# SYSTRAN/faster-whisper

Measured on AMD Instinct MI355X. Metric: audio-sec/sec (RTF) large-v3 fp16 beam=5 batch=16, higher is better.
Workload: dtype f16

## Files before the change

### faster_whisper_amd/_lib.py

```python
import ctypes as C
import os

import numpy as np

_HERE = os.path.dirname(os.path.abspath(__file__))
LIB_PATH = os.environ.get("FWAMD_LIB") or os.path.join(_HERE, "libfwamd.so")

FW_OK = 0
FW_EINVAL = -1
FW_ENODEV = -2
FW_ENOMEM = -3
FW_ERUNTIME = -4
FW_ENOSPC = -5

COMPUTE_FLOAT16 = 0
COMPUTE_INT8_FLOAT16 = 1
FW_DT_F32 = 0
FW_DT_F16 = 1
FW_MAX_ALIGN_HEADS = 64
FW_MAX_ALTERNATIVES = 8


class FwConfig(C.Structure):
    _fields_ = [
        ("n_mels", C.c_int32), ("n_audio_ctx", C.c_int32), ("d_model", C.c_int32), ("n_heads", C.c_int32),
        ("n_enc_layers", C.c_int32), ("n_dec_layers", C.c_int32), ("n_vocab", C.c_int32),
        ("n_text_ctx", C.c_int32), ("is_multilingual", C.c_int32),
        ("tok_eot", C.c_int32), ("tok_sot", C.c_int32), ("tok_lang_begin", C.c_int32), ("n_langs", C.c_int32),
        ("tok_translate", C.c_int32), ("tok_transcribe", C.c_int32), ("tok_sot_lm", C.c_int32),
        ("tok_sot_prev", C.c_int32), ("tok_no_speech", C.c_int32), ("tok_no_timestamps", C.c_int32),
        ("tok_timestamp_begin", C.c_int32),
        ("n_suppress_begin", C.c_int32), ("suppress_begin", C.c_int32 * 8),
        ("n_align_heads", C.c_int32), ("align_heads", C.c_int32 * (2 * FW_MAX_ALIGN_HEADS)),
    ]


class FwWeight(C.Structure):
    _fields_ = [("name", C.c_char_p), ("data", C.c_void_p), ("dtype", C.c_int32), ("ndim", C.c_int32),
                ("dims", C.c_int64 * 4)]


class FwGenOpts(C.Structure):
    _fields_ = [
        ("beam_size", C.c_int32), ("patience", C.c_float), ("num_hypotheses", C.c_int32),
        ("length_penalty", C.c_float), ("repetition_penalty", C.c_float), ("no_repeat_ngram_size", C.c_int32),
        ("max_length", C.c_int32), ("return_scores", C.c_int32), ("return_no_speech_prob", C.c_int32),
        ("max_initial_timestamp_index", C.c_int32), ("suppress_blank", C.c_int32),
        ("suppress_tokens", C.POINTER(C.c_int32)), ("n_suppress_tokens", C.c_int32),
        ("sampling_topk", C.c_int32), ("sampling_temperature", C.c_float), ("seed", C.c_uint64),
        ("min_new_tokens", C.c_int32),
    ]


class FwVadWeights(C.Structure):
    _fields_ = [
        ("stft_basis", C.c_void_p), ("conv_w", C.c_void_p * 4), ("conv_b", C.c_void_p * 4),
        ("lstm_w", C.c_void_p), ("lstm_r", C.c_void_p), ("lstm_b", C.c_void_p), ("dec_w", C.c_void_p),
        ("dec_b", C.c_float),
    ]


SYMBOLS = [
    "fw_last_error", "fw_abi_version", "fw_device_count",
    "fw_model_create", "fw_model_free", "fw_model_info", "fw_model_blob", "fw_model_create_from_blob_dev",
    "fw_model_set_decode_batch", "fw_model_decode_batch", "fw_model_join_decoder", "fw_model_decode_stats",
    "fw_model_set_merge_wait", "fw_model_set_decode_lanes", "fw_model_run_capacity", "fw_dec_big_min_rows", "fw_dec_big_min_rows_of", "fw_test_knob",
    "fw_test_idle_lead_chunks", "fw_test_run_capacity", "fw_test_dec_linear_plan", "fw_test_self_attn_form",
    "fw_test_gemm_plan",
    "fw_pack_blob_size", "fw_pack_blob_copy", "fw_pack_blob_free",
    "fw_logmel", "fw_logmel_full",
    "fw_encode", "fw_encode_pcm", "fw_encode_pcm_dev", "fw_tensor_shape", "fw_tensor_to_host",
    "fw_tensor_from_host", "fw_tensor_free",
    "fw_generate", "fw_generate_lp", "fw_generate_alt", "fw_detect_language", "fw_align", "fw_score",
    "fw_prof_enable", "fw_prof_reset", "fw_prof_count", "fw_prof_name", "fw_prof_get", "fw_synchronize",
    "fw_dev_alloc", "fw_dev_free", "fw_dev_upload",
    "fw_test_gemm", "fw_test_layernorm", "fw_test_attention", "fw_test_dec_linear", "fw_test_dec_logits", "fw_test_logits_rules",
    "fw_test_dec_self_attn", "fw_test_dec_cross_attn", "fw_test_dec_cross_probs", "fw_test_dec_softmax_pick", "fw_bench_gemm", "fw_bench_dec_linear", "fw_bench_attention",
    "fw_bench_gemm_epi", "fw_bench_dec_linear_epi",
    "fw_test_gemm_ex", "fw_test_cross_kv_frag_index", "fw_test_quant_rows", "fw_test_layernorm_frag",
    "fw_test_dec_beam_update", "fw_test_dec_embed", "fw_test_align_post",
    "fw_test_logits_rules_lp", "fw_test_dec_beam_update_lp",
    "fw_test_logits_rules_alt", "fw_test_dec_beam_update_alt", "fw_test_alt_gather",
    "fw_test_logits_rules_smp_tab", "fw_test_logits_rules_ex", "fw_test_score_rows", "fw_test_graph_captures", "fw_test_blob_check",
    "fw_vad_create", "fw_vad_forward", "fw_vad_free", "fw_vad_forward_dev", "fw_vad_forward_audio_dev",
    "fw_vad_forward_audio_batch_dev",
    "fw_flac_info", "fw_flac_decode",
    "fw_resample_filter", "fw_resample_dev", "fw_bench_resample",
]

_lib = None


class FwError(RuntimeError):
    pass


def load():
    global _lib
    if _lib is not None:
        return _lib
    if not os.path.exists(LIB_PATH):
        raise FwError(
            f"{LIB_PATH} not found: build it with `python -c 'import __graft_entry__ as g; g.build()'` "
            "(hipcc --offload-arch=gfx950). faster_whisper_amd has no CPU fallback.")
    lib = C.CDLL(LIB_PATH)
    vp, i32, i64, f32p = C.c_void_p, C.c_int32, C.c_int64, C.POINTER(C.c_float)
    i32p, i64p = C.POINTER(C.c_int32), C.POINTER(C.c_int64)
    lib.fw_last_error.restype = C.c_char_p
    lib.fw_abi_version.restype = i32
    lib.fw_device_count.restype = i32
    lib.fw_model_create.argtypes = [C.POINTER(FwConfig), C.POINTER(FwWeight), i32, i32, i32, i32, i32, C.POINTER(vp)]
    lib.fw_model_free.argtypes = [vp]
    lib.fw_model_free.restype = None
    lib.fw_model_info.argtypes = [vp, C.POINTER(FwConfig), i32p, i32p, i32p, i32p]
    lib.fw_model_blob.argtypes = [vp, C.POINTER(vp), i64p]
    lib.fw_model_create_from_blob_dev.argtypes = [C.POINTER(FwConfig), vp, i64, i32, i32, i32, i32, C.POINTER(vp)]
    lib.fw_model_set_decode_batch.argtypes = [vp, i32]
    lib.fw_model_decode_batch.argtypes = [vp]
    lib.fw_model_decode_batch.restype = i32
    lib.fw_model_run_capacity.argtypes = [vp]
    lib.fw_model_run_capacity.restype = i32
    lib.fw_dec_big_min_rows.restype = i32
    if hasattr(lib, "fw_dec_big_min_rows_of"):
        lib.fw_dec_big_min_rows_of.restype = i32
        lib.fw_dec_big_min_rows_of.argtypes = [i32, i32]
    if hasattr(lib, "fw_flac_info"):
        lib.fw_flac_info.argtypes = [vp, i64, i32p, i32p, i32p, i64p]
        lib.fw_flac_decode.argtypes = [vp, i64, vp, i64, i64p, i32p]
    if hasattr(lib, "fw_test_knob"):
        lib.fw_test_knob.argtypes = [i32, i32]
    if hasattr(lib, "fw_test_idle_lead_chunks"):
        lib.fw_test_idle_lead_chunks.argtypes = [i64, i32, i32, i64, i32]
        lib.fw_test_idle_lead_chunks.restype = i64
    if hasattr(lib, "fw_test_run_capacity"):
        lib.fw_test_run_capacity.argtypes = [i32, i32, i32, i64, i32, i32, i32, i32, i32, i64p, i64p, i64p]
        lib.fw_test_run_capacity.restype = i32
    if hasattr(lib, "fw_test_dec_linear_plan"):
        lib.fw_test_dec_linear_plan.argtypes = [i32, i32, i32, i32, i32, i32, i32, i32p]
        lib.fw_test_self_attn_form.argtypes = [i32] * 8
        lib.fw_test_self_attn_form.restype = i32
    if hasattr(lib, "fw_test_gemm_plan"):
        lib.fw_test_gemm_plan.argtypes = [i32, i32, i32, i32, i64, i64, i64, i64, i64, i32, i32, i32, i32, i32, i32p]
    lib.fw_model_join_decoder.argtypes = [vp, vp]
    lib.fw_model_set_merge_wait.argtypes = [vp, i32, i32]
    lib.fw_model_set_decode_lanes.argtypes = [vp, i32]
    lib.fw_model_decode_stats.argtypes = [vp, i64p, i64p, i64p, i32p]
    lib.fw_pack_blob_size.argtypes = [C.POINTER(FwConfig), C.POINTER(FwWeight), i32, i32, i64p, C.POINTER(vp)]
    lib.fw_pack_blob_copy.argtypes = [vp, vp, i64]
    lib.fw_pack_blob_free.argtypes = [vp]
    lib.fw_pack_blob_free.restype = None
    lib.fw_logmel.argtypes = [vp, vp, i64p, i32, vp, i32p]
    lib.fw_logmel_full.argtypes = [vp, vp, i64, vp, i64]
    lib.fw_encode.argtypes = [vp, vp, i32, C.POINTER(vp)]
    lib.fw_encode_pcm.argtypes = [vp, vp, i64p, i32, C.POINTER(vp)]
    lib.fw_encode_pcm_dev.argtypes = [vp, vp, i64p, i32, C.POINTER(vp)]
    lib.fw_tensor_shape.argtypes = [vp, i32p, i32p, i32p]
    lib.fw_tensor_to_host.argtypes = [vp, vp, vp]
    lib.fw_tensor_from_host.argtypes = [vp, vp, i32, C.POINTER(vp)]
    lib.fw_tensor_free.argtypes = [vp]
    lib.fw_tensor_free.restype = None
    lib.fw_generate.argtypes = [vp, vp, i32p, i32p, i32, C.POINTER(FwGenOpts), i32p, i32p, f32p, f32p]
    if hasattr(lib, "fw_generate_lp"):
        lib.fw_generate_lp.argtypes = [vp, vp, i32p, i32p, i32, C.POINTER(FwGenOpts), i32p, i32p, f32p, f32p, f32p, f32p]
    if hasattr(lib, "fw_generate_alt"):
        f32 = C.c_float
        lib.fw_generate_alt.argtypes = [vp, vp, i32p, i32p, i32, C.POINTER(FwGenOpts), i32, i32p, i32p, f32p, f32p, f32p,
                                        f32p, i32p, f32p, i32p, f32p]
        lib.fw_test_logits_rules_alt.argtypes = [vp, vp, i32, vp, i32, vp, C.POINTER(FwGenOpts), i32, vp, vp, vp, vp, vp,
                                                 vp, vp, i32, vp, vp]
        lib.fw_test_dec_beam_update_alt.argtypes = [vp, i32, i32, i32, i32, i32, i32, i32, i32, f32, i32, vp, vp, vp, vp,
                                                    vp, vp, vp, i32, f32, vp, vp, vp, vp, vp, vp, vp, vp, vp, vp, vp, vp,
                                                    vp, vp, vp]
        lib.fw_test_alt_gather.argtypes = [vp, vp, vp, i32, i32, i32, i32, i32, vp, i32, vp, vp, vp, vp, i32, vp, vp]
    lib.fw_detect_language.argtypes = [vp, vp, i32, i32p, f32p]
    lib.fw_align.argtypes = [vp, vp, i32p, i32, i32p, i32p, i32p, i32, i32, i32, i32p, i32p, f32p]
    lib.fw_prof_enable.argtypes = [vp, i32]
    lib.fw_prof_enable.restype = None
    lib.fw_prof_reset.argtypes = [vp]
    lib.fw_prof_reset.restype = None
    lib.fw_prof_count.restype = i32
    lib.fw_prof_name.argtypes = [i32]
    lib.fw_prof_name.restype = C.c_char_p
    lib.fw_prof_get.argtypes = [vp, i32, C.POINTER(C.c_double), i64p, C.POINTER(C.c_double), C.POINTER(C.c_double)]
    lib.fw_synchronize.argtypes = [vp]
    lib.fw_dev_alloc.argtypes = [vp, i64, C.POINTER(vp)]
    lib.fw_dev_free.argtypes = [vp, vp]
    lib.fw_dev_upload.argtypes = [vp, vp, vp, i64]
    lib.fw_test_gemm.argtypes = [vp, vp, vp, vp, vp, i32, i32, i32, i32, i32, vp]
    lib.fw_test_dec_linear.argtypes = [vp, vp, vp, vp, vp, vp, vp, i32, i32, i32, i32, i32, vp, vp]
    lib.fw_test_dec_logits.argtypes = [vp, vp, i32, vp]
    lib.fw_test_logits_rules.argtypes = [vp, vp, i32, vp, i32, vp, C.POINTER(FwGenOpts), i32, vp, vp]
    if hasattr(lib, "fw_test_dec_self_attn"):
        lib.fw_test_dec_self_attn.argtypes = [vp, vp, vp, vp, vp, i32, i32, i32, i32, i32, i32, i32, i32, i32, i32, i32, vp]
        lib.fw_test_dec_cross_attn.argtypes = [vp, vp, vp, vp, i32, i32, i32, i32, i32, i32, vp, vp, i32, C.c_float, vp]
        lib.fw_test_dec_cross_probs.argtypes = [vp, vp, vp, i32, i32, i32, vp, i32, i32, i32, i32, vp]
        lib.fw_test_dec_softmax_pick.argtypes = [vp, vp, i32, i32, i32, vp, i32, vp]
    lib.fw_bench_attention.argtypes = [vp, i32, i32, i32, i32, i32, f32p]
    lib.fw_bench_gemm.argtypes = [vp, i32, i32, i32, i32, i32, i32, i32, i32, f32p]
    lib.fw_bench_dec_linear.argtypes = [vp, i32, i32, i32, i32, i32, i32, f32p]
    if hasattr(lib, "fw_bench_gemm_epi"):
        lib.fw_bench_gemm_epi.argtypes = [vp, i32, i32, i32, i32, i32, i32, i32, i32, i32, i32, i32, f32p]
        lib.fw_bench_dec_linear_epi.argtypes = [vp, i32, i32, i32, i32, i32, i32, i32, i32, i32, f32p]
    lib.fw_test_layernorm.argtypes = [vp, vp, vp, vp, i32, i32, vp]
    lib.fw_test_attention.argtypes = [vp, vp, vp, vp, i32, i32, i32, vp]
    if hasattr(lib, "fw_test_gemm_ex"):
        lib.fw_test_gemm_ex.argtypes = [vp, vp, i64, i64, i64, vp, vp, vp, i64, i64, i64, vp, i64, i64, i64, i64, i64,
                                        i32, i32, i32, i32, i32, i32, i32, i32, i32, vp, vp]
        lib.fw_test_cross_kv_frag_index.argtypes = [i32, i32, i32, vp]
        lib.fw_test_quant_rows.argtypes = [vp, vp, i32, i32, i64, vp, vp, i32, vp, vp]
        lib.fw_test_layernorm_frag.argtypes = [vp, vp, vp, vp, i32, i32, i32, vp]
    if hasattr(lib, "fw_test_dec_beam_update"):
        f32 = C.c_float
        lib.fw_test_dec_beam_update.argtypes = [vp, i32, i32, i32, i32, i32, i32, i32, i32, f32, i32, vp, vp, vp, vp, vp,
                                                i32, f32, vp, vp, vp, vp, vp, vp, vp, vp, vp, vp, vp]
        lib.fw_test_dec_embed.argtypes = [vp, vp, i32, vp, i32, vp, i32, i32, i32, i32, i32, i32, f32, vp, vp]
        lib.fw_test_align_post.argtypes = [vp, vp, i32, i32, i32, i32, vp, vp, i32, vp]
    if hasattr(lib, "fw_test_dec_beam_update_lp"):
        f32 = C.c_float
        lib.fw_test_logits_rules_lp.argtypes = [vp, vp, i32, vp, i32, vp, C.POINTER(FwGenOpts), i32, vp, vp, vp]
        lib.fw_test_dec_beam_update_lp.argtypes = [vp, i32, i32, i32, i32, i32, i32, i32, i32, f32, i32, vp, vp, vp, vp, vp,
                                                   vp, vp, i32, f32, vp, vp, vp, vp, vp, vp, vp, vp, vp, vp, vp, vp, vp]
    if hasattr(lib, "fw_test_graph_captures"):
        lib.fw_test_logits_rules_smp_tab.argtypes = [vp, vp, i32, vp, i32, vp, C.POINTER(FwGenOpts), i32, vp, vp, vp, vp, vp, vp]
        lib.fw_test_graph_captures.argtypes = [vp, i64p]
    if hasattr(lib, "fw_test_logits_rules_ex"):
        lib.fw_test_logits_rules_ex.argtypes = [vp, vp, i32, vp, i32, vp, C.POINTER(FwGenOpts), i32, vp, vp, vp, vp, vp, vp, vp]
    if hasattr(lib, "fw_score"):
        lib.fw_score.argtypes = [vp, vp, i32p, i32p, i32p, i32p, i32, i32, C.POINTER(FwGenOpts), f32p, i32p, f32p]
        lib.fw_test_score_rows.argtypes = [vp, vp, i32, vp, vp, vp, C.POINTER(FwGenOpts), i32, vp, vp, vp]
    if hasattr(lib, "fw_test_blob_check"):
        lib.fw_test_blob_check.argtypes = [vp, i64]
    lib.fw_vad_create.argtypes = [C.POINTER(FwVadWeights), C.POINTER(vp)]
    lib.fw_vad_forward.argtypes = [vp, vp, i64, i32, vp, vp, vp]
    lib.fw_vad_free.argtypes = [vp]
    lib.fw_vad_forward_dev.argtypes = [vp, i32, vp, i64, vp, vp, vp]
    if hasattr(lib, "fw_vad_forward_audio_dev"):
        lib.fw_vad_forward_audio_dev.argtypes = [vp, i32, vp, i64, vp, vp, vp]
    if hasattr(lib, "fw_vad_forward_audio_batch_dev"):
        lib.fw_vad_forward_audio_batch_dev.argtypes = [vp, i32, vp, vp, i32, vp, vp, vp]
    lib.fw_vad_free.restype = None
    if hasattr(lib, "fw_resample_dev"):
        f64 = C.c_double
        lib.fw_resample_filter.argtypes = [i32, i32, i32, f64, vp, i64p, i32p, i32p]
        lib.fw_resample_dev.argtypes = [i32, vp, i64, i32, i32, i32, f64, i32, vp, i64]
        lib.fw_bench_resample.argtypes = [i32, vp, i64, i32, i32, i32, f64, i32, i32, f32p]
    _lib = lib
    return lib


def check(rc: int):
    if rc == FW_OK:
        return
    msg = load().fw_last_error().decode("utf-8", "replace")
    if rc in (FW_EINVAL, FW_ENOSPC):
        raise ValueError(msg)
    raise RuntimeError(f"libfwamd error {rc}: {msg}")


def ptr(a: np.ndarray):
    return a.ctypes.data_as(C.c_void_p)


def as_i32p(a: np.ndarray):
    return a.ctypes.data_as(C.POINTER(C.c_int32))


def as_i64p(a: np.ndarray):
    return a.ctypes.data_as(C.POINTER(C.c_int64))


def as_f32p(a: np.ndarray):
    return a.ctypes.data_as(C.POINTER(C.c_float))
```

### faster_whisper_amd/csrc/decoder.hip

```cpp
#include "engine.h"

#include <math.h>
#include <stdlib.h>
#include <string.h>

#include <algorithm>
#include <atomic>
#include <chrono>
#include <numeric>

#include "dec_kernels.h"
#include "kernels.h"

namespace fw {

using fwd::FIN_CAP;
using fwd::GenDev;

#define DEC_RUN_MAX_ROWS 1600

struct CrossPool {
  DevBufs bufs;
  half_t *ck = nullptr, *cvt = nullptr;
  int n_blocks = 0, EB = 0, kvp = 0;
// ... 40 lines not shown
  GrowBuf<int> alt_out_tok;
  GrowBuf<float> alt_out_lp;
  GrowBuf<fwd::AltHyp> alt_hyps;
  int *done = nullptr, *n_done = nullptr, *n_fin = nullptr, *fin_tok = nullptr, *fin_len = nullptr;
  float *fin_score = nullptr, *fin_cum = nullptr;
  int* d_step = nullptr;
  float* no_speech = nullptr;
  unsigned long long* sup_bits = nullptr;
  int* zero_done = nullptr;
  int *ptab = nullptr, *sot_tab = nullptr;
  half_t *nsp_x = nullptr, *nsp_xf = nullptr;
  fwd::SmpRow* smp_tab = nullptr;
  half_t *x_frag = nullptr, *att_frag = nullptr, *ffn_frag = nullptr;
  half_t* xn_frag = nullptr;
  int8_t* xq = nullptr;
  float* xs = nullptr;
  QuantRows ekq;
  std::vector<GraphSlot> graphs;
  uint64_t graph_clock = 0;
  bool graphs_enabled = true;
  ~GenWorkspace() {
    for (GraphSlot& s : graphs)
      if (s.exec) (void)hipGraphExecDestroy(s.exec);
  }
};

static std::atomic<uint64_t> g_tensor_id{1};
uint64_t next_tensor_id() { return g_tensor_id.fetch_add(1); }

static bool env_knob_on(std::atomic<int>& v, const char* env) {
  int x = v.load(std::memory_order_relaxed);
  if (x < 0) {
    const char* e = getenv(env);
    x = (e && atoi(e) == 0) ? 0 : 1;
    v.store(x);
  }
  return x != 0;
}

static int self_positions(const Model* m, int decode_batch, int nts) {
  const int NT = m->cfg.n_text_ctx;
  const int need = (int)(((int64_t)NT * m->max_batch + decode_batch - 1) / decode_batch);
  return std::min(NT, std::max(std::max(nts, need), 8));
}

int64_t gen_workspace_bytes(const Model* m, int lane_chunks, int nts) {
  const fw_config& c = m->cfg;
  const int64_t B = lane_chunks, R = B * m->max_beam, d = c.d_model, L = c.n_dec_layers, NT = c.n_text_ctx;
  const int64_t NTs = self_positions(m, lane_chunks, nts > 0 ? nts : (int)NT);
  int64_t n = 2 * (L * R * NTs * d) * 2;
  n += R * (int64_t)c.n_vocab * 4 + R * 12 * d * 2 * 2;
  n += R * FIN_CAP * NT * 4 + 3 * R * NT * 4;
  n += R * FIN_CAP * (NT + 1) * 4 + 2 * R * NT * 4 + R * 32 * 4;
  return n + (64 << 20);
}

int64_t cross_pool_bytes(const Model* m, int pool_chunks) {
  const fw_config& c = m->cfg;
  const int64_t kvp = ((c.n_audio_ctx + 31) / 32) * 32;
  return 2 * ((int64_t)c.n_dec_layers * pool_chunks * c.d_model * kvp) * 2;
}

static int pool_block_count(int pool_chunks, int max_batch) {
  return std::max(1, std::max(pool_chunks, max_batch) / max_batch);
}

int cross_pool_ensure(Model* m, int pool_chunks) {
  if (m->xpool) return FW_OK;
  const fw_config& c = m->cfg;
  std::unique_ptr<CrossPool> p(new CrossPool());
  p->EB = m->max_batch;
  p->n_blocks = pool_block_count(pool_chunks, m->max_batch);
  p->kvp = ((c.n_audio_ctx + 31) / 32) * 32;
  p->blocks.assign(p->n_blocks, CrossPool::Block());
  const size_t n = (size_t)c.n_dec_layers * p->n_slots() * c.d_model * p->kvp;
  int rc;
  if ((rc = p->bufs.alloc(&p->ck, n)) || (rc = p->bufs.alloc(&p->cvt, n))) return rc;
  const HipFail fail{FW_ENODEV, "cross-attention pool setup"};
  FW_HIP_AS(fail, hipMemset(p->ck, 0, n * sizeof(half_t)));
  FW_HIP_AS(fail, hipMemset(p->cvt, 0, n * sizeof(half_t)));
  FW_HIP_AS(fail, hipDeviceSynchronize());
  m->xpool = p.release();
  return FW_OK;
}

void cross_pool_free(Model* m) {
  delete m->xpool;
  m->xpool = nullptr;
}

static void pool_acquire(CrossPool* p, const std::vector<uint64_t>& ids, const std::vector<int>& ns, std::vector<int>& blk,
                         std::vector<char>& hit) {
  std::unique_lock<std::mutex> lk(p->mu);
  const int n = (int)ids.size();
  blk.assign(n, -1);
  hit.assign(n, 0);
  for (;;) {
    int n_free = 0;
    for (const CrossPool::Block& b : p->blocks) n_free += b.busy ? 0 : 1;
    if (n_free >= n) break;
    p->cv.wait(lk);
  }
  for (int i = 0; i < n; ++i)
    for (int k = 0; k < p->n_blocks; ++k) {
      CrossPool::Block& b = p->blocks[k];
      if (!b.busy && b.enc_id == ids[i] && b.n == ns[i] && ids[i] != 0) { b.busy = true; blk[i] = k; hit[i] = 1; break; }
    }
  for (int i = 0; i < n; ++i) {
    if (blk[i] >= 0) continue;
    int best = -1;
    for (int k = 0; k < p->n_blocks; ++k)
      if (!p->blocks[k].busy && (best < 0 || p->blocks[k].stamp < p->blocks[best].stamp)) best = k;
    CrossPool::Block& b = p->blocks[best];
    b.busy = true; b.enc_id = 0; b.n = 0;
    blk[i] = best;
  }
  for (int i = 0; i < n; ++i) p->blocks[blk[i]].stamp = ++p->clock;
}

static void pool_release(CrossPool* p, const std::vector<int>& blk) {
  {
    std::lock_guard<std::mutex> lk(p->mu);
    for (int k : blk)
      if (k >= 0) p->blocks[k].busy = false;
  }
  p->cv.notify_all();
}

struct PoolHold {
  CrossPool* p;
  std::vector<int> blk;
  hipStream_t st = nullptr;
  ~PoolHold() {
    if (!p) return;
    if (st && !blk.empty()) (void)hipStreamSynchronize(st);
    pool_release(p, blk);
  }
};

int gen_workspace_build(const Model* m, DecodeLane* lane, int lane_chunks, int self_ctx) {
  const fw_config& c = m->cfg;
  std::unique_ptr<GenWorkspace> ws(new GenWorkspace());
  GenWorkspace* g = ws.get();
  g->B = lane_chunks;
  g->EB = m->max_batch;
  g->K = m->max_beam;
  g->R = g->B * g->K;
  g->NT = c.n_text_ctx;
  g->NTs = self_positions(m, g->B, self_ctx > 0 ? self_ctx : c.n_text_ctx);
  g->self_cap = (int64_t)g->R * g->NTs;
  const size_t R = g->R, d = c.d_model, L = c.n_dec_layers, NT = g->NT;
  FW_CHECK_ARG(R <= 2048, "decode_batch * max_beam must be <= 2048 (got %zu)", R);
  FW_HIP(hipSetDevice(m->device));
  if (!lane->stream) FW_HIP(create_stream(&lane->stream, "DEC"));
  int rc;
#define A(p, n) do { if ((rc = g->bufs.alloc(&(p), (n)))) return rc; } while (0)
#define Z(p, n) do { if ((rc = g->bufs.zalloc(&(p), (n)))) return rc; } while (0)
  Z(g->slot_map, R);
  A(g->sk, L * (size_t)g->self_cap * d);
  A(g->sv, L * (size_t)g->self_cap * d);
  A(g->x, R * d); A(g->qkv, R * 3 * d); A(g->att, R * d); A(g->qc, R * d);
  A(g->ffn, R * 4 * d);
  A(g->logits, R * c.n_vocab);
  A(g->prompt_dev, NT * R); A(g->prompt_blk, NT * R);
  A(g->cur_tok, R);
  A(g->hist2, 2 * R * NT);
  A(g->cum2, 2 * R);
  A(g->kvidx2, 2 * R * NT);
  A(g->cand_val, R * 32);
  A(g->cand_tok, R * 32);
  A(g->cand_lp, R * 32);
  A(g->lphist2, 2 * R * NT);
  A(g->done, R); A(g->n_done, 1); A(g->n_fin, R);
  A(g->fin_tok, R * FIN_CAP * NT); A(g->fin_len, R * FIN_CAP);
  A(g->fin_score, R * FIN_CAP); A(g->fin_cum, R * FIN_CAP);
  A(g->fin_lp, R * FIN_CAP * (NT + 1));
  Z(g->d_step, 1);
  A(g->no_speech, R);
  A(g->sup_bits, (size_t)LP_SUP_WORDS);
  Z(g->zero_done, R);
  const size_t R16 = (R + 15) / 16 * 16;
  Z(g->ptab, R); Z(g->sot_tab, R);
  Z(g->nsp_x, R16 * d); Z(g->nsp_xf, R16 * d);
  Z(g->smp_tab, R);
  if (m->compute_type == FW_COMPUTE_INT8_FLOAT16) {
    Z(g->xq, R16 * 4 * d);
    Z(g->xs, R16);
    g->ekq.cap_rows = (int64_t)g->EB * c.n_audio_ctx;
    g->ekq.cap_elems = g->ekq.cap_rows * d;
    A(g->ekq.q, (size_t)g->ekq.cap_elems);
    A(g->ekq.scale, (size_t)g->ekq.cap_rows);
  } else {
    Z(g->x_frag, R16 * d); Z(g->att_frag, R16 * d); Z(g->ffn_frag, R16 * 4 * d); Z(g->xn_frag, R16 * d);
  }
#undef A
#undef Z
  FW_HIP(hipDeviceSynchronize());
  const char* ng = getenv("FWAMD_NO_GRAPH");
  g->graphs_enabled = !(ng && ng[0] == '1');
  lane->gen = ws.release();
  return FW_OK;
}

int gen_workspace_ensure(Model* m, DecodeLane* lane) {
  if (int rc = cross_pool_ensure(m, m->decode_batch)) return rc;
  if (lane->gen) return FW_OK;
  return gen_workspace_build(m, lane, lane_chunks_of(m), m->decode_self_ctx);
}

void gen_workspace_free(DecodeLane* lane) {
  delete lane->gen;
  lane->gen = nullptr;
}

DecodeLane::~DecodeLane() {
  if (stream) (void)hipStreamSynchronize(stream);
  gen_workspace_free(this);
  if (stream) (void)hipStreamDestroy(stream);
  if (spare) (void)hipStreamDestroy(spare);
}

static std::atomic<int> g_cross_kv_layered{-1};
void set_cross_kv_layered(int on) { g_cross_kv_layered.store(on ? 1 : 0); }
static bool cross_kv_strides(const Model* m, int64_t* ws, int64_t* bs) {
  const int L = m->cfg.n_dec_layers;
  if (L < 2) return false;
  const int64_t w1 = m->dec[1].ck.w - m->dec[0].ck.w, b1 = m->dec[1].ck.b - m->dec[0].ck.b;
  for (int l = 1; l < L; ++l) {
    if (m->dec[l].ck.w - m->dec[0].ck.w != l * w1 || m->dec[l].cv.w - m->dec[0].cv.w != l * w1) return false;
    if (m->dec[l].ck.b - m->dec[0].ck.b != l * b1 || m->dec[l].cv.b - m->dec[0].cv.b != l * b1) return false;
  }
  *ws = w1; *bs = b1;
  return w1 > 0;
}

static int ensure_cross_kv(Model* m, DecodeLane* lane, const Tensor* enc, int blk, bool hit) {
  if (hit) return FW_OK;
  GenWorkspace* g = lane->gen;
  CrossPool* pool = m->xpool;
  const int B = enc->B;
  const int b0 = blk * pool->EB;
  const fw_config& c = m->cfg;
  const int d = c.d_model, T = c.n_audio_ctx;
  const int64_t xs = (int64_t)T * d;
  hipStream_t st = lane->stream;
  int rc;
  ProfScope ps(lane->prof, PF_CROSS_KV_GEMM, 2.0 * c.n_dec_layers * B * (double)T * d * (2.0 * d), 0, st);
  const bool i8 = m->compute_type == FW_COMPUTE_INT8_FLOAT16;
  const int kvp = pool->kvp;
  const int64_t kvs = (int64_t)d * kvp;
  const int64_t cls = (int64_t)pool->n_slots() * kvs;
  LinCall k{.in = {enc->data, d, xs}, .C = pool->ck + (size_t)b0 * kvs, .ldc = d, .c_bs = kvs, .M = T, .batch = B,
            .head_rows = kvp, .st = st};
  LinCall v{.in = k.in, .C = pool->cvt + (size_t)b0 * kvs, .ldc = kvp, .c_bs = kvs, .M = T, .batch = B, .trans = true,
            .head_rows = kvp, .st = st};
  if (i8) {
    if ((rc = quantise_rows(m, enc->data, nullptr, (int64_t)B * T, d, st, g->ekq))) return rc;
    k.in = v.in = {.xq = &g->ekq};
  }
  int64_t ws = 0, bs = 0;
  if (!i8 && env_knob_on(g_cross_kv_layered, "FWAMD_CROSS_KV_LAYERED") && cross_kv_strides(m, &ws, &bs)) {
    k.n_layers = v.n_layers = c.n_dec_layers;
    k.w_ls = v.w_ls = ws; k.b_ls = v.b_ls = bs; k.c_ls = v.c_ls = cls;
    if ((rc = run_linear(m, m->dec[0].ck, k)) || (rc = run_linear(m, m->dec[0].cv, v))) return rc;
  } else for (int l = 0; l < c.n_dec_layers; ++l) {
    if (l) { k.C += cls; v.C += cls; }
    if ((rc = run_linear(m, m->dec[l].ck, k)) || (rc = run_linear(m, m->dec[l].cv, v))) return rc;
  }
  std::lock_guard<std::mutex> lk(pool->mu);
  pool->blocks[blk].enc_id = enc->id;
  pool->blocks[blk].n = B;
  return FW_OK;
}

struct StepCfg {
  int rows, kmul;
  int B;
  int pos_fixed;
  int P;
  const int* ptab = nullptr;
  const int* tok;
  bool need_logits;
  int nospeech_rowmul;
  bool beam_tail;
  const int* done;
  int kv_slot0 = 0;
  int blk_n = 0;
  int nospeech_off = 0;
  const int* sel_heads_dev = nullptr;
  const int* sel_layer_off = nullptr;
  float* probs = nullptr; int n_sel_total = 0, n_tok = 0, tok_idx = 0;
};

#define DG(call)                                                        \
  do {                                                                  \
    if ((call) != 0) {                                                  \
      set_error("decoder gemm: unsupported shape (%s)", #call);        \
      return FW_ERUNTIME;                                               \
    }                                                                   \
  } while (0)

static std::atomic<int> g_pos_blocks{-1};
void set_pos_blocks(int on) { g_pos_blocks.store(on ? 1 : 0); }
static int pos_block_size(const Model* m, const GenWorkspace* g, const GenDev& gp, int chunks) {
  if (!env_knob_on(g_pos_blocks, "FWAMD_POS_BLOCKS") || chunks < 1) return 1;
  if (!fwd::self_attn_block_ok(g->NT, gp.ctx, m->cfg.d_model, gp.R)) return 1;
  return std::max(1, std::min(16, g->R / chunks));
}

static int project_logits(Model* m, DecodeLane* lane, const half_t* x, const half_t* x_frag, int rows) {
  GenWorkspace* g = lane->gen;
  const fw_config& c = m->cfg;
  const int d = c.d_model;
  hipStream_t st = lane->stream;
  ProfScope ps(lane->prof, PF_DEC_LOGITS, 2.0 * rows * (double)c.n_vocab * d, 2.0 * c.n_vocab * d, st);
  if (m->compute_type == FW_COMPUTE_INT8_FLOAT16) {
    fwk::launch_quant_rows(st, x, d, m->dec_ln.g, m->dec_ln.b, g->xq, g->xs, rows, d, 1);
    DG(fwd::launch_dec_logits(st, true, g->xq, g->xs, m->logits.wq, m->logits.wscale, nullptr, nullptr, g->logits,
                              c.n_vocab, rows, c.n_vocab, d));
  } else if (m->ln_unfold >= 1) {
    fwk::launch_layernorm(st, x, m->dec_ln.g, m->dec_ln.b, g->xn_frag, rows, d, 1);
    DG(fwd::launch_dec_logits(st, false, g->xn_frag, nullptr, m->logits_p.w, nullptr, nullptr, nullptr, g->logits,
                              c.n_vocab, rows, c.n_vocab, d));
  } else {
    DG(fwd::launch_dec_logits(st, false, x_frag, nullptr, m->logits.w, nullptr, m->logits.s1, m->logits.cf, g->logits,
                              c.n_vocab, rows, c.n_vocab, d));
  }
  return FW_OK;
}

static int run_step(Model* m, DecodeLane* lane, const GenDev& gp, const StepCfg& s) {
  GenWorkspace* g = lane->gen;
  const fw_config& c = m->cfg;
  const int d = c.d_model, H = c.n_heads, T = c.n_audio_ctx, NT = g->NT;
  CrossPool* pool = m->xpool;
  const int kvp = pool->kvp;
  hipStream_t st = lane->stream;
  const int rows = s.rows;
  const bool i8 = m->compute_type == FW_COMPUTE_INT8_FLOAT16;
  {
    ProfScope ps(lane->prof, PF_DEC_MISC, 0, 0, st);
    fwd::launch_embed(st, s.tok, m->tok_emb, m->dec_pos, g->x, i8 ? nullptr : g->x_frag, rows, d, g->d_step,
                      s.pos_fixed, s.P, s.blk_n, s.ptab, s.kmul, gp.reach);
  }
  auto lin_q = [&](const half_t* xin, const LNW* ln, const LinearW& L, const half_t* res, half_t* outp, int act) -> int {
    fwk::launch_quant_rows(st, xin, L.K, ln ? ln->g : nullptr, ln ? ln->b : nullptr, g->xq, g->xs, rows, L.K, 1);
    return fwd::launch_dec_gemm_frag_i8(st, g->xq, g->xs, L.wq, L.wscale, L.b, res, L.N, outp, L.N, rows, L.N, L.K, act);
  };
  auto lin_f = [&](const half_t* xin_frag, const LinearW& L, const half_t* res, half_t* outp, half_t* outp_frag,
                   int act) -> int {
    return fwd::launch_dec_linear(st, fwd::DecLin{xin_frag, L.w, L.b, L.s1, L.cf, res, L.N, outp, L.N, outp_frag, rows,
                                                  L.N, L.K, act});
  };
  const int frag = i8 ? 0 : 1;
  const bool unf = !i8 && m->ln_unfold >= 2;
  auto lin_u = [&](const LNW& ln, const LinearW& L, half_t* outp, half_t* outp_frag, int act) -> int {
    fwk::launch_layernorm(st, g->x, ln.g, ln.b, g->xn_frag, rows, d, 1);
    return fwd::launch_dec_linear(st, fwd::DecLin{g->xn_frag, L.w, L.b, nullptr, nullptr, nullptr, L.N, outp, L.N,
                                                  outp_frag, rows, L.N, L.K, act});
  };
  for (int l = 0; l < c.n_dec_layers; ++l) {
    const DecLayerW& L = m->dec[l];
    half_t* kc = g->sk + (size_t)l * gp.cache_rows * gp.ctx * d;
    half_t* vc = g->sv + (size_t)l * gp.cache_rows * gp.ctx * d;
    const half_t* ck = pool->ck + (size_t)l * pool->n_slots() * d * kvp;
    const half_t* cvt = pool->cvt + (size_t)l * pool->n_slots() * d * kvp;
    {
      ProfScope ps(lane->prof, PF_DEC_GEMM_QKV, 2.0 * rows * 3.0 * d * d, 2.0 * 3.0 * d * d, st);
      if (i8) DG(lin_q(g->x, &L.ln1, L.qkv, nullptr, g->qkv, 0));
      else if (unf) DG(lin_u(L.ln1, L.qkv_p, g->qkv, nullptr, 0));
      else DG(lin_f(g->x_frag, L.qkv, nullptr, g->qkv, nullptr, 0));
    }
// ... 1217 lines not shown
```

### faster_whisper_amd/csrc/engine.h

```cpp
#pragma once
#include <hip/hip_runtime.h>
#include <math.h>
#include <stdint.h>
#include <string.h>
#include <algorithm>
#include <atomic>
#include <chrono>
#include <condition_variable>
#include <deque>
#include <memory>
#include <mutex>
#include <string>
#include <vector>

#include "../../include/fwamd.h"
#include "common.h"
#include "kernels.h"

namespace fw {

void set_error(const char* fmt, ...);
#define FW_HIP(call)                                                                   \
  do {                                                                                 \
    hipError_t e_ = (call);                                                            \
// ... 23 lines not shown
  half_t h = (half_t)f;
  uint16_t u;
  memcpy(&u, &h, 2);
  return u;
}
inline float f16_bits_to_f32(uint16_t u) {
  half_t h;
  memcpy(&h, &u, 2);
  return (float)h;
}

template <typename At>
inline float quant_row_i8(const float* row, int K, int8_t* q, At&& at) {
  float amax = 0.f;
  for (int k = 0; k < K; ++k) amax = std::max(amax, fabsf(row[k]));
  const float sc = amax > 0.f ? 127.0f / amax : 0.f;
  for (int k = 0; k < K; ++k) q[at(k)] = (int8_t)lrintf(row[k] * sc);
  return amax > 0.f ? amax / 127.0f : 1.0f;
}

inline size_t frag_pos(int64_t row, int64_t k, int64_t K, int KE) {
  const int OCT = KE / 4;
  return (size_t)((((row >> 4) * (K / KE) + k / KE) * 64 + ((k / OCT) & 3) * 16 + (row & 15)) * OCT + (k % OCT));
}

#define FW_BLOB_MAGIC "FWAMDBL1"
constexpr int kBlobGeneration = 6;
struct BlobHeader {
  char magic[8];
  int32_t version;
  int32_t n_tensors;
  int64_t total_bytes;
  int32_t compute_type;
  int32_t reserved;
  fw_config cfg;
};
struct BlobEntry {
  char name[64];
  int32_t dtype;
  int32_t ndim;
  int64_t dims[4];
  int64_t offset;
  int64_t nbytes;
};

struct LinearW {
  const half_t* w = nullptr;
  const half_t* b = nullptr;
  const int8_t* wq = nullptr;
  const float* wscale = nullptr;
  const float* s1 = nullptr;
  const float* cf = nullptr;
  int N = 0, K = 0;
};
struct LNW { const half_t* g = nullptr; const half_t* b = nullptr; };

struct EncLayerW { LNW ln1, ln2; LinearW qk, v, out, ffn1, ffn2; };
struct DecLayerW { LNW ln1, ln2, ln3; LinearW qkv, out, cq, ck, cv, cout, ffn1, ffn2; LinearW qkv_p, cq_p, ffn1_p; };

enum ProfFamily {
  PF_LOGMEL = 0, PF_ENC_GEMM, PF_ENC_ATTN, PF_ENC_LN, PF_CROSS_KV_GEMM,
  PF_DEC_GEMM_QKV, PF_DEC_GEMM_DXD, PF_DEC_GEMM_FFN1, PF_DEC_GEMM_FFN2,
  PF_DEC_SELF_ATTN, PF_DEC_CROSS_ATTN, PF_DEC_LOGITS, PF_DEC_SAMPLE, PF_DEC_MISC, PF_COUNT
};

struct ProfAcc {
  double ms = 0; int64_t launches = 0; double flops = 0; double bytes = 0;
};

struct Prof {
  std::mutex mu;
  bool on = false;
  ProfAcc acc[PF_COUNT];
  struct PendingEv { hipEvent_t a, b; int fam; };
  std::vector<PendingEv> pending;
  std::vector<hipEvent_t> ev_pool;
  ~Prof();
};

int dev_alloc(void** p, size_t bytes);
template <typename T>
inline int dev_alloc_t(T** p, size_t n) { return dev_alloc(reinterpret_cast<void**>(p), n * sizeof(T)); }
struct DevBufs {
  std::vector<void*> ptrs;
  DevBufs() = default;
  DevBufs(const DevBufs&) = delete;
  DevBufs& operator=(const DevBufs&) = delete;
  ~DevBufs() {
    for (void* p : ptrs) (void)hipFree(p);
  }
  template <typename T>
  int alloc(T** p, size_t n) {
    if (int rc = dev_alloc_t(p, n)) return rc;
    ptrs.push_back(*p);
    return FW_OK;
  }
  template <typename T>
  int zalloc(T** p, size_t n) {
    if (int rc = alloc(p, n)) return rc;
    FW_HIP(hipMemset(*p, 0, n * sizeof(T)));
    return FW_OK;
  }
};
template <typename T>
struct GrowBuf {
  T* p = nullptr;
  int64_t cap = 0;
  GrowBuf() = default;
  GrowBuf(const GrowBuf&) = delete;
  GrowBuf& operator=(const GrowBuf&) = delete;
  ~GrowBuf() { if (p) (void)hipFree(p); }
  int ensure(int64_t n) {
    if (n <= cap) return FW_OK;
    if (p) (void)hipFree(p);
    p = nullptr;
    cap = 0;
    if (int rc = dev_alloc_t(&p, (size_t)n)) return rc;
    cap = n;
    return FW_OK;
  }
};

struct QuantRows {
  int8_t* q = nullptr;
  float* scale = nullptr;
  int64_t cap_rows = 0, cap_elems = 0;
  int64_t rows = 0, ld = 0;
  bool fits(int64_t r, int64_t K) const { return r >= 0 && K >= 0 && r <= cap_rows && r * K <= cap_elems; }
};

struct Model;
struct EncPool {
  std::mutex mu;
  std::vector<half_t*> free;
  const size_t elems;
  bool closed = false;
  std::atomic<Model*> model;
  EncPool(Model* m, size_t elems_) : elems(elems_), model(m) {}
  int take(half_t** p);
  void give(half_t* p);
  void close();
};
struct Tensor {
  std::shared_ptr<EncPool> pool;
  half_t* data = nullptr;
  int B = 0, T = 0, D = 0;
  uint64_t id = 0;
};

struct GenWorkspace;
struct GenRequest;
struct CrossPool;

constexpr int kMaxDecodeLanes = 4;
struct DecodeLane {
  GenWorkspace* gen = nullptr;
  hipStream_t stream = nullptr;
  hipStream_t spare = nullptr;
  std::mutex mu;
  Prof prof;
  bool busy = false;
  ~DecodeLane();
};

struct DecodeGroup {
  std::mutex mu;
  std::condition_variable cv;
  std::deque<GenRequest*> queue;
  bool gathering = false;
  bool resizing = false;
  int active_runs = 0;
  std::atomic<int> lanes_enabled{kMaxDecodeLanes};
  std::atomic<int> encoding{0};
  std::chrono::steady_clock::time_point last_arrival{};
  std::mutex enc_mu;
  std::atomic<int> enc_pass_us{0};
  std::atomic<int> merge_wait_ms{-1};
  std::atomic<int> merge_fill_pct{90};
  std::atomic<int64_t> n_runs{0}, n_requests{0}, n_chunks{0};
  std::atomic<int> max_run_chunks{0};
  std::atomic<int64_t> graph_captures{0};
};

struct Weights {
  int c_pad = 0;
  LinearW conv1, conv2;
  const half_t* enc_pos = nullptr;
  std::vector<EncLayerW> enc;
  LNW enc_ln_post;
  const half_t* tok_emb = nullptr;
  const half_t* dec_pos = nullptr;
  std::vector<DecLayerW> dec;
  LinearW logits;
  LinearW logits_p;
  LNW dec_ln;
};
int check_blob_header(const BlobHeader& h, int64_t blob_bytes);
int bind_weights(const BlobHeader& h, const BlobEntry* entries, void* blob, Weights& W, bool* has_plain);

struct Model : Weights {
  fw_config cfg{};
  int compute_type = 0;
  int device = 0;
  int max_batch = 0, max_beam = 0;
  hipStream_t stream = nullptr;
  std::mutex mu;

  void* blob = nullptr;
  bool blob_owned = true;
  int64_t blob_bytes = 0;
  int ln_unfold = 0;
  bool has_plain = false;

  float* lm_consts = nullptr;
  float* lm_filtT = nullptr;
  int lm_mel_pad = 0;

  DevBufs bufs;
  GrowBuf<float> ws_pcm;
  int64_t* ws_offsets = nullptr;
  GrowBuf<float> ws_raw;
  int* ws_chunk_max = nullptr;
  int* ws_nframes = nullptr;
  float* ws_feat32 = nullptr;
  half_t* ws_mel_cl = nullptr;
  half_t* ws_conv1 = nullptr;
  half_t *ws_x = nullptr, *ws_x2 = nullptr, *ws_xn = nullptr;
  half_t* ws_qk = nullptr;
  half_t* ws_vt = nullptr;
  half_t* ws_att = nullptr;
  half_t* ws_ffn = nullptr;
  QuantRows ws_xq;
  int t_pad = 0;

  std::vector<std::unique_ptr<DecodeLane>> lanes;
  Model* decoder = nullptr;
  CrossPool* xpool = nullptr;
  int decode_batch = 0;
  int lane_batch = 0;
  int decode_self_ctx = 0;
  int dependents = 0;
  bool free_deferred = false;
  void* self = nullptr;
  Model* blob_owner = nullptr;
  DecodeGroup grp;

  std::shared_ptr<EncPool> enc_pool;

  Prof prof;
};

struct ProfScope {
  Prof* p; int fam; hipStream_t st; hipEvent_t a = nullptr, b = nullptr;
  ProfScope(Prof& p_, int fam_, double flops, double bytes, hipStream_t st_);
  ProfScope(Model* m, int fam_, double flops, double bytes) : ProfScope(m->prof, fam_, flops, bytes, m->stream) {}
  ~ProfScope();
};
void prof_collect(Prof& p);

hipError_t create_stream(hipStream_t* st, const char* role);
int64_t idle_lead_chunks(int64_t queued, int n_queued, int encoding, int64_t want, int max_batch, int lanes = 2);
struct RunCapacity {
  int64_t rows_per_chunk;
  int64_t rows, row_cap, self_cap;
  int ctx;
  bool rows_fit, cache_fits;
  int64_t want;
  int64_t run_cap;
  RunCapacity(int lane_chunks, int max_batch, int max_beam, int64_t self_cap, int B, bool sampling, int beam_size,
              int num_hypotheses, int ctx);
};

struct LinIn {
  const half_t* A = nullptr; int64_t lda = 0, a_bs = 0;
  const QuantRows* xq = nullptr;
};
struct LinCall {
  LinIn in;
  half_t* C = nullptr; int64_t ldc = 0, c_bs = 0;
  const half_t* res = nullptr; int64_t ldr = 0, r_bs = 0;
  int M = 0, batch = 1;
  int act = 0;
  bool trans = false;
  int head_rows = 0;
  int n_layers = 1; int64_t w_ls = 0, b_ls = 0, c_ls = 0;
  hipStream_t st = nullptr;
};
fwk::GemmParams gemm_params(const LinearW& L, const LinCall& c, int64_t ldw);
int run_linear(Model* m, const LinearW& L, const LinCall& c);
int quantise_rows(Model* m, const half_t* A, const LNW* ln, int64_t rows, int K, hipStream_t st, QuantRows& qr);
void set_cross_kv_layered(int on);
int run_encoder(Model* m, int B, half_t* out);

void set_pos_blocks(int on);
uint64_t next_tensor_id();
int gen_workspace_ensure(Model* dm, DecodeLane* lane);
int cross_pool_ensure(Model* dm, int pool_chunks);
int gen_workspace_build(const Model* dm, DecodeLane* lane, int lane_chunks, int self_ctx);
void gen_workspace_free(DecodeLane* lane);
int64_t gen_workspace_bytes(const Model* m, int lane_chunks, int self_ctx);
int64_t cross_pool_bytes(const Model* m, int pool_chunks);
void cross_pool_free(Model* m);
void launch_align_post(hipStream_t st, const float* probs, float* stats, int n_sel, int n_tok_cap, int T, int B,
                       const int* n_tok, const int* nfr, int width, float* mat);
inline Model* decoder_of(Model* m) { return m->decoder ? m->decoder : m; }
inline const Model* decoder_of(const Model* m) { return m->decoder ? m->decoder : m; }
inline Model* decoder_of(const Tensor& t) {
  Model* m = t.pool ? t.pool->model.load() : nullptr;
  return m ? decoder_of(m) : nullptr;
}
inline int lane_chunks_of(const Model* m) {
  const int b = m->lane_batch > 0 ? m->lane_batch : m->decode_batch;
  return b > m->max_batch ? b : m->max_batch;
}

}

struct fw_model { fw::Model impl; };
struct fw_tensor { fw::Tensor impl; };
```

### faster_whisper_amd/csrc/engine.hip

```cpp
#include "engine.h"

#include <math.h>
#include <stdarg.h>
#include <stdio.h>
#include <stdlib.h>
#include <string.h>

#include <algorithm>
#include <map>
#include <optional>
#include <type_traits>

#include "dec_kernels.h"
#include "kernels.h"

namespace fw {

static thread_local char g_err[1024] = "";
void set_error(const char* fmt, ...) {
  va_list ap;
  va_start(ap, fmt);
  vsnprintf(g_err, sizeof(g_err), fmt, ap);
  va_end(ap);
}
// ... 435 lines not shown
  template <typename T>
  int get(const std::string& name, int dtype, std::initializer_list<int64_t> dims, const T** out) const {
    auto it = by_name.find(name);
    FW_CHECK_ARG(it != by_name.end(), "weight blob lacks tensor '%s'", name.c_str());
    const BlobEntry& e = *it->second;
    const char* nm = name.c_str();
    FW_CHECK_ARG(e.dtype == dtype, "weight blob tensor '%s': dtype %d, expected %d", nm, e.dtype, dtype);
    FW_CHECK_ARG(e.ndim == (int)dims.size(), "weight blob tensor '%s': %d dims, expected %zu", nm, e.ndim, dims.size());
    int64_t bytes = dtype == 1 ? 2 : dtype == 2 ? 1 : 4;
    int i = 0;
    for (int64_t x : dims) {
      FW_CHECK_ARG(e.dims[i] == x, "weight blob tensor '%s': dim %d is %lld, expected %lld", nm, i, (long long)e.dims[i],
                   (long long)x);
      bytes *= x;
      ++i;
    }
    FW_CHECK_ARG(e.nbytes == bytes, "weight blob tensor '%s': %lld bytes, its shape has %lld", nm, (long long)e.nbytes,
                 (long long)bytes);
    FW_CHECK_ARG(e.offset >= 0 && e.offset % 256 == 0 && e.offset <= h.total_bytes - bytes,
                 "weight blob tensor '%s': offset %lld (%lld bytes) misaligned or outside the blob's %lld bytes", nm,
                 (long long)e.offset, (long long)bytes, (long long)h.total_bytes);
    *out = reinterpret_cast<const T*>(blob + e.offset);
    return FW_OK;
  }
  int plain(const std::string& name, std::initializer_list<int64_t> dims, const half_t** dst, WForm form = W_ROWS,
            const char* = nullptr) const {
    if (dims.size() != 2) return get(name, 1, dims, dst);
    return get(name, 1, {stored_rows(dims.begin()[0], form), dims.begin()[1]}, dst);
  }
  int conv(const std::string& base, int cout, int, int cin_pad, LinearW& L) const {
    if (int rc = get(base + ".wg", 1, {cout, 3 * cin_pad}, &L.w)) return rc;
    return get(base + ".b", 1, {cout}, &L.b);
  }
  int folded(const std::string& out, const std::string&, const std::string&, const std::string&, int N, int K,
             WForm form, LinearW& L) const {
    int rc;
    if ((rc = get(out + ".wf", 1, {stored_rows(N, form), K}, &L.w)) || (rc = get(out + ".s1", 0, {N}, &L.s1))) return rc;
    return get(out + ".cf", 0, {N}, &L.cf);
  }
  int quant(const std::string& out, const std::string&, int N, int K, WForm form, LinearW& L) const {
    if (int rc = get(out + ".wq", 2, {stored_rows(N, form), K}, &L.wq)) return rc;
    return get(out + ".ws", 0, {N}, &L.wscale);
  }
};

int bind_weights(const BlobHeader& h, const BlobEntry* entries, void* blob, Weights& W, bool* has_plain) {
  Binder b{h, reinterpret_cast<char*>(blob), {}};
  for (int i = 0; i < h.n_tensors; ++i)
    b.by_name[std::string(entries[i].name, strnlen(entries[i].name, sizeof(entries[i].name)))] = &entries[i];
  const bool i8 = h.compute_type == FW_COMPUTE_INT8_FLOAT16;
  *has_plain = !i8 && b.by_name.count("dec.logits.wp") != 0;
  return walk_weights(h.cfg, i8, *has_plain, W, b);
}

static void compute_mel_filters(int n_mels, std::vector<float>& filt ) {
  const int n_fft = 400, nb = 201;
  const double sr = 16000.0;
  std::vector<double> fftfreqs(nb);
  const double val = 1.0 / (n_fft * (1.0 / sr));
  for (int k = 0; k < nb; ++k) fftfreqs[k] = k * val;
  const double max_mel = 45.245640471924965;
  const int n = n_mels + 2;
  std::vector<double> mels(n), freqs(n);
  const double step = (max_mel - 0.0) / (n - 1);
  for (int i = 0; i < n; ++i) mels[i] = i * step + 0.0;
  mels[n - 1] = max_mel;
  const double f_sp = 200.0 / 3;
  const double min_log_hz = 1000.0, min_log_mel = (min_log_hz - 0.0) / f_sp;
  const double logstep = log(6.4) / 27.0;
  for (int i = 0; i < n; ++i) {
    freqs[i] = 0.0 + f_sp * mels[i];
    if (mels[i] >= min_log_mel) freqs[i] = min_log_hz * exp(logstep * (mels[i] - min_log_mel));
  }
  filt.assign((size_t)n_mels * nb, 0.f);
  for (int i = 0; i < n_mels; ++i) {
    const double fd0 = freqs[i + 1] - freqs[i], fd1 = freqs[i + 2] - freqs[i + 1];
    const double enorm = 2.0 / (freqs[i + 2] - freqs[i]);
    for (int k = 0; k < nb; ++k) {
      const double lower = -(freqs[i] - fftfreqs[k]) / fd0;
      const double upper = (freqs[i + 2] - fftfreqs[k]) / fd1;
      double wv = std::max(0.0, std::min(lower, upper));
      wv *= enorm;
      filt[(size_t)i * nb + k] = (float)wv;
    }
  }
}

static int setup_logmel_consts(Model* m) {
  std::vector<float> consts(800);
  for (int j = 0; j < 400; ++j) consts[j] = (float)cos(2.0 * M_PI * (double)j / 400.0);
  for (int n = 0; n < 400; ++n) consts[400 + n] = (float)(0.5 - 0.5 * cos(2.0 * M_PI * (double)n / 400.0));
  std::vector<float> filt;
  compute_mel_filters(m->cfg.n_mels, filt);
  m->lm_mel_pad = ((m->cfg.n_mels + 31) / 32) * 32;
  std::vector<float> filtT((size_t)224 * m->lm_mel_pad, 0.f);
  for (int i = 0; i < m->cfg.n_mels; ++i)
    for (int k = 0; k < 201; ++k) filtT[(size_t)k * m->lm_mel_pad + i] = filt[(size_t)i * 201 + k];
  int rc;
  if ((rc = m->bufs.alloc(&m->lm_consts, 800)) || (rc = m->bufs.alloc(&m->lm_filtT, filtT.size()))) return rc;
  FW_HIP(hipMemcpy(m->lm_consts, consts.data(), 800 * sizeof(float), hipMemcpyHostToDevice));
  FW_HIP(hipMemcpy(m->lm_filtT, filtT.data(), filtT.size() * sizeof(float), hipMemcpyHostToDevice));
  return FW_OK;
}

static std::mutex g_models_mu;
static std::vector<Model*> g_live_models;

static int alloc_workspaces(Model* m) {
  const fw_config& c = m->cfg;
  const size_t B = m->max_batch, d = c.d_model, T = c.n_audio_ctx;
  m->t_pad = ((c.n_audio_ctx + 63) / 64) * 64;
  DevBufs& db = m->bufs;
  const bool i8 = m->compute_type == FW_COMPUTE_INT8_FLOAT16;
  int rc;
  if ((rc = db.alloc(&m->ws_offsets, B + 1)) || (rc = db.alloc(&m->ws_chunk_max, B)) || (rc = db.alloc(&m->ws_nframes, B)) ||
      (rc = m->ws_raw.ensure((int64_t)B * c.n_mels * 3008)) || (rc = db.alloc(&m->ws_feat32, B * c.n_mels * 3000)) ||
      (rc = db.zalloc(&m->ws_mel_cl, B * 3002 * m->c_pad)) || (rc = db.zalloc(&m->ws_conv1, B * 3002 * d)) ||
      (rc = db.alloc(&m->ws_x, B * T * d)) || (rc = db.alloc(&m->ws_x2, B * T * d)) || (rc = db.alloc(&m->ws_xn, B * T * d)) ||
      (rc = db.alloc(&m->ws_qk, B * T * 2 * d)) || (rc = db.zalloc(&m->ws_vt, B * d * m->t_pad)) ||
      (rc = db.alloc(&m->ws_att, B * T * d)) || (rc = db.alloc(&m->ws_ffn, B * T * 4 * d)) ||
      (i8 && ((rc = db.alloc(&m->ws_xq.q, B * T * 4 * d)) || (rc = db.alloc(&m->ws_xq.scale, B * T)))))
    return rc;
  if (i8) { m->ws_xq.cap_rows = B * T; m->ws_xq.cap_elems = B * T * 4 * d; }
  return FW_OK;
}

static int model_from_blob(const void* blob_dev, int64_t blob_bytes, bool owned, int device, int max_batch,
                           int max_beam, fw_model** out) {
  FW_CHECK_ARG(max_batch >= 1 && max_batch <= 256, "max_batch must be in [1,256], got %d", max_batch);
  FW_CHECK_ARG(max_beam >= 1 && max_beam <= 16, "max_beam must be in [1,16], got %d", max_beam);
  FW_CHECK_ARG(max_batch * max_beam <= 2048, "max_batch * max_beam must be <= 2048 decoder rows, got %d", max_batch * max_beam);
  FW_CHECK_ARG(blob_bytes >= (int64_t)sizeof(BlobHeader), "weight blob too small");
  BlobHeader h;
  FW_HIP(hipMemcpy(&h, blob_dev, sizeof(h), hipMemcpyDeviceToHost));
  int rc = check_blob_header(h, blob_bytes);
  if (rc) return rc;
  std::vector<BlobEntry> entries(h.n_tensors);
  FW_HIP(hipMemcpy(entries.data(), reinterpret_cast<const char*>(blob_dev) + sizeof(h),
                   entries.size() * sizeof(BlobEntry), hipMemcpyDeviceToHost));
  fw_model* fm = new fw_model();
  Model* m = &fm->impl;
  m->lanes.reserve(kMaxDecodeLanes);
  m->lanes.emplace_back(new DecodeLane());
  m->cfg = h.cfg;
  m->compute_type = h.compute_type;
  m->device = device;
  m->max_batch = max_batch;
  m->max_beam = max_beam;
  m->blob = const_cast<void*>(blob_dev);
  m->blob_owned = owned;
  m->blob_bytes = blob_bytes;
  m->enc_pool = std::make_shared<EncPool>(m, (size_t)max_batch * h.cfg.n_audio_ctx * h.cfg.d_model);
  auto fail = [&](int code) { fw_model_free(fm); return code; };
  hipError_t he = create_stream(&m->stream, "ENC");
  if (he != hipSuccess) {
    set_error("hipStreamCreate failed: %s", hipGetErrorString(he));
    return fail(FW_ENODEV);
  }
  if ((rc = bind_weights(h, entries.data(), m->blob, *m, &m->has_plain))) return fail(rc);
  m->ln_unfold = env_ln_unfold();
  if (m->ln_unfold && m->compute_type != FW_COMPUTE_INT8_FLOAT16 && !m->has_plain) {
    set_error("FWAMD_LN_UNFOLD=%d needs a weight blob packed with FWAMD_LN_UNFOLD set (this one carries the folded forms only)",
              m->ln_unfold);
    return fail(FW_EINVAL);
  }
  if ((rc = setup_logmel_consts(m))) return fail(rc);
  if ((rc = alloc_workspaces(m))) return fail(rc);
  m->decode_batch = max_batch;
  he = hipDeviceSynchronize();
  if (he != hipSuccess) {
    set_error("device sync after model setup failed: %s", hipGetErrorString(he));
    return fail(FW_ENODEV);
  }
  {
    std::lock_guard<std::mutex> lk(g_models_mu);
    if (!owned)
      for (Model* o : g_live_models)
        if (o->blob == m->blob && o->blob_owned) { m->blob_owner = o; o->dependents += 1; break; }
    g_live_models.push_back(m);
  }
  m->self = fm;
  *out = fm;
  return FW_OK;
}

static void balanced_cu_mask(int n_cus, bool invert, uint32_t mask[8]) {
  const int k = n_cus / 32;
  for (int w = 0; w < 8; ++w) mask[w] = 0;
  for (int i = 0; i < 256; ++i) {
    const bool in = ((i % 8) + (i / 8)) % 8 < k;
    if (in != invert) mask[i >> 5] |= 1u << (i & 31);
  }
}

hipError_t create_stream(hipStream_t* st, const char* role) {
  char name[64];
  snprintf(name, sizeof(name), "FWAMD_%s_CUS", role);
  if (const char* c = getenv(name)) {
    const int v = atoi(c), n = v < 0 ? -v : v;
    if (n >= 32 && n <= 224 && n % 32 == 0) {
      uint32_t mask[8];
      balanced_cu_mask(n, v < 0, mask);
      return hipExtStreamCreateWithCUMask(st, 8, mask);
    }
  }
  snprintf(name, sizeof(name), "FWAMD_%s_STREAM_PRIO", role);
  const char* e = getenv(name);
  if (e && (!strcmp(e, "high") || !strcmp(e, "low"))) {
    int least = 0, greatest = 0;
    if (hipDeviceGetStreamPriorityRange(&least, &greatest) == hipSuccess && least != greatest)
      return hipStreamCreateWithPriority(st, hipStreamNonBlocking, e[0] == 'h' ? greatest : least);
  }
  return hipStreamCreateWithFlags(st, hipStreamNonBlocking);
}

fwk::GemmParams gemm_params(const LinearW& L, const LinCall& c, int64_t ldw) {
  fwk::GemmParams p{};
  if (const QuantRows* xq = c.in.xq) {
    p.A = reinterpret_cast<const half_t*>(xq->q); p.lda = xq->ld; p.a_bstride = c.M * xq->ld;
    p.W = reinterpret_cast<const half_t*>(L.wq);
    p.a_scale = xq->scale; p.as_bstride = c.M; p.w_scale = L.wscale;
  } else {
    p.A = c.in.A; p.lda = c.in.lda; p.a_bstride = c.in.a_bs;
    p.W = L.w;
  }
  p.ldw = ldw;
  p.bias = L.b;
  p.res = c.res; p.ldr = c.ldr; p.r_bstride = c.r_bs;
  p.C = c.C; p.ldc = c.ldc; p.c_bstride = c.c_bs;
  p.M = c.M; p.N = L.N; p.K = L.K;
  p.act = c.act;
  p.head_rows = c.head_rows;
  p.n_layers = c.n_layers; p.w_lstride = c.w_ls; p.bias_lstride = c.b_ls; p.c_lstride = c.c_ls;
  return p;
}

int run_linear(Model* m, const LinearW& L, const LinCall& c) {
  if (const QuantRows* xq = c.in.xq)
    FW_CHECK_ARG(xq->scale && xq->rows == (int64_t)c.batch * c.M && xq->ld == L.K,
                 "int8 gemm: the quantised input holds %lld rows of %lld, the call reads %lld rows of %d", (long long)xq->rows,
                 (long long)xq->ld, (long long)c.batch * c.M, L.K);
  if (fwk::launch_gemm(c.st ? c.st : m->stream, gemm_params(L, c, L.K), c.batch, c.trans) != 0) {
    set_error("%sgemm: unsupported shape M=%d N=%d K=%d lda=%lld layers=%d", c.in.xq ? "int8 " : "", c.M, L.N, L.K,
              (long long)c.in.lda, c.n_layers);
    return FW_ERUNTIME;
  }
  return FW_OK;
}

int quantise_rows(Model* m, const half_t* A, const LNW* ln, int64_t rows, int K, hipStream_t st, QuantRows& qr) {
  FW_CHECK_ARG(qr.fits(rows, K), "quantise_rows: %lld rows x %d = %lld elements, the buffer holds %lld rows, %lld elements",
               (long long)rows, K, (long long)(rows * K), (long long)qr.cap_rows, (long long)qr.cap_elems);
  fwk::launch_quant_rows(st ? st : m->stream, A, K, ln ? ln->g : nullptr, ln ? ln->b : nullptr, qr.q, qr.scale, (int)rows, K);
  qr.rows = rows; qr.ld = K;
  return FW_OK;
}

int run_encoder(Model* m, int B, half_t* out) {
  const fw_config& c = m->cfg;
  const int d = c.d_model, T = c.n_audio_ctx, H = c.n_heads;
  const int64_t xs = (int64_t)T * d, vts = (int64_t)d * m->t_pad;
  const bool i8 = m->compute_type == FW_COMPUTE_INT8_FLOAT16;
  auto gemm_flops = [&](double rows, double k) { return 2.0 * B * rows * d * k; };
  int rc;
  {
    ProfScope ps(m, PF_ENC_GEMM, gemm_flops(3000.0, 3.0 * c.n_mels), 0);
    if ((rc = run_linear(m, m->conv1, {.in = {m->ws_mel_cl, m->c_pad, (int64_t)3002 * m->c_pad}, .C = m->ws_conv1 + d,
                                       .ldc = d, .c_bs = (int64_t)3002 * d, .M = 3000, .batch = B, .act = 1})))
      return rc;
  }
  {
    ProfScope ps(m, PF_ENC_GEMM, gemm_flops(T, 3.0 * d), 0);
    if ((rc = run_linear(m, m->conv2, {.in = {m->ws_conv1, 2 * d, (int64_t)3002 * d}, .C = m->ws_x, .ldc = d, .c_bs = xs,
                                       .res = m->enc_pos, .ldr = d, .r_bs = 0, .M = T, .batch = B, .act = 1})))
      return rc;
  }
  half_t* x = m->ws_x;
  half_t* x2 = m->ws_x2;
  auto normed = [&](const half_t* a, const LNW& ln) -> const half_t* {
    if (i8) return a;
    ProfScope ps(m, PF_ENC_LN, 0, 4.0 * B * T * d);
    fwk::launch_layernorm(m->stream, a, ln.g, ln.b, m->ws_xn, B * T, d);
    return m->ws_xn;
  };
  auto input = [&](const half_t* a, int K, const LNW* ln, LinIn& in) -> int {
    if (!i8) { in = {a, K, (int64_t)T * K}; return FW_OK; }
    in = {.xq = &m->ws_xq};
    return quantise_rows(m, a, ln, (int64_t)B * T, K, m->stream, m->ws_xq);
  };
  for (int l = 0; l < c.n_enc_layers; ++l) {
    const EncLayerW& L = m->enc[l];
    LinIn in;
    const half_t* h = normed(x, L.ln1);
    {
      ProfScope ps(m, PF_ENC_GEMM, gemm_flops(T, 3.0 * d), 0);
      if ((rc = input(h, d, &L.ln1, in)) ||
          (rc = run_linear(m, L.qk, {.in = in, .C = m->ws_qk, .ldc = 2 * d, .c_bs = 2 * xs, .M = T, .batch = B})) ||
          (rc = run_linear(m, L.v, {.in = in, .C = m->ws_vt, .ldc = m->t_pad, .c_bs = vts, .M = T, .batch = B, .trans = true})))
        return rc;
    }
    {
      ProfScope ps(m, PF_ENC_ATTN, 4.0 * B * (double)T * T * d, 0);
      fwk::launch_attn_enc(m->stream, {.q = m->ws_qk, .k = m->ws_qk + d, .ld = 2 * d, .qk_bstride = 2 * xs, .vt = m->ws_vt,
                                       .ldvt = m->t_pad, .vt_bstride = vts, .out = m->ws_att, .ldo = d, .o_bstride = xs,
                                       .B = B, .H = H, .T = T});
    }
    std::optional<ProfScope> ps;
    ps.emplace(m, PF_ENC_GEMM, gemm_flops(T, i8 ? 9.0 * d : d), 0);
    if ((rc = input(m->ws_att, d, nullptr, in)) ||
        (rc = run_linear(m, L.out, {.in = in, .C = x2, .ldc = d, .c_bs = xs, .res = x, .ldr = d, .r_bs = xs, .M = T, .batch = B})))
      return rc;
    if (!i8) ps.reset();
    h = normed(x2, L.ln2);
    if (!i8) ps.emplace(m, PF_ENC_GEMM, gemm_flops(T, 8.0 * d), 0);
    if ((rc = input(h, d, &L.ln2, in)) ||
        (rc = run_linear(m, L.ffn1, {.in = in, .C = m->ws_ffn, .ldc = 4 * d, .c_bs = 4 * xs, .M = T, .batch = B, .act = 1})) ||
        (rc = input(m->ws_ffn, 4 * d, nullptr, in)) ||
        (rc = run_linear(m, L.ffn2, {.in = in, .C = x, .ldc = d, .c_bs = xs, .res = x2, .ldr = d, .r_bs = xs, .M = T, .batch = B})))
      return rc;
  }
  {
    ProfScope ps(m, PF_ENC_LN, 0, 4.0 * B * T * d);
    fwk::launch_layernorm(m->stream, x, m->enc_ln_post.g, m->enc_ln_post.b, out, B * T, d);
  }
  hipError_t he = hipGetLastError();
  if (he != hipSuccess) {
    set_error("encoder launch failed: %s", hipGetErrorString(he));
    return FW_ERUNTIME;
  }
  return FW_OK;
}

int EncPool::take(half_t** p) {
  {
    std::lock_guard<std::mutex> lk(mu);
    if (!free.empty()) {
      *p = free.back();
      free.pop_back();
      return FW_OK;
    }
  }
  return dev_alloc_t(p, elems);
}
void EncPool::give(half_t* p) {
  std::unique_lock<std::mutex> lk(mu);
  if (!closed) { free.push_back(p); return; }
  lk.unlock();
  (void)hipFree(p);
}
void EncPool::close() {
  std::vector<half_t*> rest;
  {
    std::lock_guard<std::mutex> lk(mu);
    closed = true;
    model.store(nullptr);
    rest.swap(free);
  }
  for (half_t* p : rest) (void)hipFree(p);
}

static int new_tensor(Model* m, int B, fw_tensor** out) {
  fw_tensor* t = new fw_tensor();
  t->impl.pool = m->enc_pool;
  t->impl.B = B;
  t->impl.T = m->cfg.n_audio_ctx;
  t->impl.D = m->cfg.d_model;
// ... 8 lines not shown

static int encode_to_tensor(Model* m, int B, const char* what, fw_tensor** out) {
  fw_tensor* t = nullptr;
  int rc = new_tensor(m, B, &t);
  if (rc) return rc;
  if ((rc = run_encoder(m, B, t->impl.data))) {
    fw_tensor_free(t);
    return rc;
  }
  hipError_t he = hipStreamSynchronize(m->stream);
  if (he != hipSuccess) {
    fw_tensor_free(t);
    set_error("%s failed: %s", what, hipGetErrorString(he));
    return FW_ERUNTIME;
  }
  prof_collect(m->prof);
  *out = t;
  return FW_OK;
}

static int check_offsets(const int64_t* offsets, int B, int64_t* total, int* max_frames) {
  FW_CHECK_ARG(offsets && offsets[0] == 0, "offsets[0] must be 0");
  int mf = 0;
  for (int b = 0; b < B; ++b) {
    const int64_t n = offsets[b + 1] - offsets[b];
    FW_CHECK_ARG(n >= 0 && n < (int64_t)1 << 30, "chunk %d has invalid length %lld", b, (long long)n);
    mf = std::max(mf, (int)((n + 160) / 160));
  }
  *total = offsets[B];
  *max_frames = mf;
  return FW_OK;
}

static int logmel_batch(Model* m, const float* pcm_dev, const int64_t* offsets_host, int B, bool want_f32,
                        bool want_cl) {
  int64_t total;
  int max_frames;
  int rc = check_offsets(offsets_host, B, &total, &max_frames);
  if (rc) return rc;
  const int stride = std::max(3008, (max_frames + 7) / 8 * 8);
  if ((rc = m->ws_raw.ensure((int64_t)B * m->cfg.n_mels * stride))) return rc;
  FW_HIP(hipMemcpyAsync(m->ws_offsets, offsets_host, (B + 1) * sizeof(int64_t), hipMemcpyHostToDevice, m->stream));
  {
    ProfScope ps(m, PF_LOGMEL, 0, (double)total * 4 + (double)B * m->cfg.n_mels * 3000 * (want_f32 ? 4 : 2));
    fwk::launch_logmel(m->stream, pcm_dev, m->ws_offsets, B, max_frames, m->lm_consts, m->lm_filtT, m->lm_mel_pad,
                       m->cfg.n_mels, m->ws_raw.p, (int64_t)m->cfg.n_mels * stride, stride, m->ws_chunk_max, 1, 3000,
                       want_f32 ? m->ws_feat32 : nullptr, want_cl ? m->ws_mel_cl : nullptr, m->c_pad, m->ws_nframes);
  }
  hipError_t he = hipGetLastError();
  if (he != hipSuccess) {
    set_error("logmel launch failed: %s", hipGetErrorString(he));
    return FW_ERUNTIME;
  }
  return FW_OK;
}

}

using namespace fw;

extern "C" {

const char* fw_last_error(void) { return g_err; }
int32_t fw_abi_version(void) { return FW_ABI_VERSION; }

int32_t fw_device_count(void) {
  int n = 0;
  if (hipGetDeviceCount(&n) != hipSuccess) return 0;
  return n;
}

int32_t fw_model_create(const fw_config* cfg, const fw_weight* weights, int32_t n_weights, int32_t compute_type,
                        int32_t device_index, int32_t max_batch, int32_t max_beam, fw_model** out) {
  FW_CHECK_ARG(cfg && weights && out, "null argument");
  FW_CHECK_ARG(compute_type == FW_COMPUTE_FLOAT16 || compute_type == FW_COMPUTE_INT8_FLOAT16,
               "unsupported compute_type %d", compute_type);
  int rc = check_config(cfg);
  if (rc) return rc;
  const int ndev = fw_device_count();
  if (ndev <= 0) {
    set_error("no HIP device visible: libfwamd has no CPU fallback");
    return FW_ENODEV;
  }
  FW_CHECK_ARG(device_index >= 0 && device_index < ndev, "device_index %d out of range (%d devices)", device_index,
               ndev);
  FW_HIP(hipSetDevice(device_index));
  std::vector<uint8_t> blob;
  if ((rc = pack_blob(cfg, weights, n_weights, compute_type, blob))) return rc;
  void* dblob = nullptr;
  if ((rc = dev_alloc(&dblob, blob.size()))) return rc;
  hipError_t he = hipMemcpy(dblob, blob.data(), blob.size(), hipMemcpyHostToDevice);
  if (he != hipSuccess) {
    (void)hipFree(dblob);
    set_error("weight upload failed: %s", hipGetErrorString(he));
    return FW_ENODEV;
  }
  rc = model_from_blob(dblob, (int64_t)blob.size(), true, device_index, max_batch, max_beam, out);
  return rc;
}

int32_t fw_pack_blob_size(const fw_config* cfg, const fw_weight* weights, int32_t n_weights, int32_t compute_type,
                          int64_t* size_out, void** handle_out) {
  FW_CHECK_ARG(cfg && weights && size_out && handle_out, "null argument");
  int rc = check_config(cfg);
  if (rc) return rc;
  auto* blob = new std::vector<uint8_t>();
  if ((rc = pack_blob(cfg, weights, n_weights, compute_type, *blob))) {
    delete blob;
    return rc;
  }
  *size_out = (int64_t)blob->size();
  *handle_out = blob;
  return FW_OK;
}
int32_t fw_pack_blob_copy(void* handle, void* dst, int64_t dst_bytes) {
  auto* blob = reinterpret_cast<std::vector<uint8_t>*>(handle);
  FW_CHECK_ARG(blob && dst && dst_bytes >= (int64_t)blob->size(), "bad blob copy arguments");
  memcpy(dst, blob->data(), blob->size());
  return FW_OK;
}
void fw_pack_blob_free(void* handle) { delete reinterpret_cast<std::vector<uint8_t>*>(handle); }

int32_t fw_model_create_from_blob_dev(const fw_config* cfg, const void* blob_dev, int64_t blob_bytes,
                                      int32_t compute_type, int32_t device_index, int32_t max_batch,
                                      int32_t max_beam, fw_model** out) {
  (void)cfg;
  (void)compute_type;
  FW_CHECK_ARG(blob_dev && out, "null argument");
  const int ndev = fw_device_count();
  if (ndev <= 0) {
    set_error("no HIP device visible: libfwamd has no CPU fallback");
    return FW_ENODEV;
  }
  FW_CHECK_ARG(device_index >= 0 && device_index < ndev, "device_index %d out of range", device_index);
  FW_HIP(hipSetDevice(device_index));
  return model_from_blob(blob_dev, blob_bytes, false, device_index, max_batch, max_beam, out);
}

void fw_model_free(fw_model* fm) {
  if (!fm) return;
  Model* m = &fm->impl;
  Model* release[2] = {nullptr, nullptr};
  {
    std::lock_guard<std::mutex> lk(g_models_mu);
    if (m->dependents > 0) {
      m->free_deferred = true;
      return;
    }
    g_live_models.erase(std::remove(g_live_models.begin(), g_live_models.end(), m), g_live_models.end());
    release[0] = m->blob_owner;
    release[1] = m->decoder;
  }
  (void)hipSetDevice(m->device);
  if (m->stream) (void)hipStreamSynchronize(m->stream);
  m->lanes.clear();
  cross_pool_free(m);
  m->enc_pool->close();
  if (m->blob && m->blob_owned) (void)hipFree(m->blob);
  if (m->stream) (void)hipStreamDestroy(m->stream);
  delete fm;
  for (Model* t : release) {
    if (!t) continue;
    bool free_now = false;
    {
      std::lock_guard<std::mutex> lk(g_models_mu);
      t->dependents -= 1;
      free_now = t->free_deferred && t->dependents == 0;
    }
    if (free_now) fw_model_free(static_cast<fw_model*>(t->self));
  }
}

int32_t fw_model_blob(const fw_model* fm, void** blob_dev, int64_t* blob_bytes) {
  FW_CHECK_ARG(fm && blob_dev && blob_bytes, "null argument");
  *blob_dev = fm->impl.blob;
  *blob_bytes = fm->impl.blob_bytes;
  return FW_OK;
}

int32_t fw_model_info(const fw_model* fm, fw_config* cfg_out, int32_t* compute_type, int32_t* device_index,
                      int32_t* max_batch, int32_t* max_beam) {
  FW_CHECK_ARG(fm, "null model");
  const Model* m = &fm->impl;
  if (cfg_out) *cfg_out = m->cfg;
  if (compute_type) *compute_type = m->compute_type;
  if (device_index) *device_index = m->device;
  if (max_batch) *max_batch = m->max_batch;
  if (max_beam) *max_beam = m->max_beam;
  return FW_OK;
}

#define DEC_GROUP_RUN_ROWS 1600
static int env_decode_lanes() {
  const char* e = getenv("FWAMD_DECODE_LANES");
  return e ? std::min(kMaxDecodeLanes, std::max(1, atoi(e))) : 2;
}

int32_t fw_model_set_decode_batch(fw_model* fm, int32_t decode_batch) {
  FW_CHECK_ARG(fm, "null model");
  Model* m = &fm->impl;
  FW_CHECK_ARG(!m->decoder, "this model has joined another model's decoder");
  FW_CHECK_ARG(decode_batch >= 1, "decode_batch must be positive");
  {
    std::lock_guard<std::mutex> gl(m->grp.mu);
    FW_CHECK_ARG(m->grp.active_runs == 0 && !m->grp.gathering && m->grp.queue.empty() && !m->grp.resizing,
                 "decode runs are queued or in flight: set the decode batch before the first generate call or after the last one returned");
    m->grp.resizing = true;
  }
  struct Done {
    DecodeGroup& g;
    ~Done() {
      { std::lock_guard<std::mutex> gl(g.mu); g.resizing = false; }
      g.cv.notify_all();
    }
  } done{m->grp};
  DecodeLane* lane0 = m->lanes[0].get();
  std::lock_guard<std::mutex> lk(lane0->mu);
  FW_HIP(hipSetDevice(m->device));
  int want = std::max(decode_batch, m->max_batch) / m->max_batch * m->max_batch;
  const int n_lanes = want >= 4 * m->max_batch ? env_decode_lanes() : 1;
  const int max_rows = n_lanes >= 2 ? DEC_GROUP_RUN_ROWS : 2048;
  auto lane_of = [&](int pool_chunks) {
    int lc = pool_chunks;
    while (lc > m->max_batch && (int64_t)lc * m->max_beam > max_rows) lc -= m->max_batch;
    return lc;
  };
  size_t free_b = 0, total_b = 0;
  FW_HIP(hipMemGetInfo(&free_b, &total_b));
  for (const auto& l : m->lanes)
    if (l->gen) free_b += (size_t)gen_workspace_bytes(m, lane_chunks_of(m), m->decode_self_ctx);
  if (m->xpool) free_b += (size_t)cross_pool_bytes(m, std::max(m->decode_batch, m->max_batch));
  const int64_t budget = (int64_t)(0.7 * (double)free_b);
  const int NT = m->cfg.n_text_ctx;
  const int ctx_steps[] = {NT, 320, 224, 160};
  int self_ctx = NT;
  for (;;) {
    bool fits = false;
    for (int cs : ctx_steps) {
      if (cs > NT) continue;
      if (cross_pool_bytes(m, want) + n_lanes * gen_workspace_bytes(m, lane_of(want), cs) <= budget) { self_ctx = cs; fits = true; break; }
    }
    if (fits || want <= m->max_batch) break;
    want -= m->max_batch;
  }
  const int lane_batch = lane_of(want);
  const bool lanes_ok = n_lanes == (int)m->lanes.size();
  if (lane0->gen && m->xpool && lanes_ok && want == m->decode_batch && lane_batch == lane_chunks_of(m) &&
      self_ctx == m->decode_self_ctx)
    return FW_OK;
  if (lane0->stream) FW_HIP(hipStreamSynchronize(lane0->stream));
  auto reset = [&] {
    m->lanes.resize(1);
    gen_workspace_free(lane0);
    cross_pool_free(m);
    m->decode_batch = m->max_batch; m->lane_batch = 0; m->decode_self_ctx = 0;
  };
  reset();
  std::vector<std::unique_ptr<DecodeLane>> further;
  int rc = cross_pool_ensure(m, want);
  if (!rc) rc = gen_workspace_build(m, lane0, lane_batch, self_ctx);
  for (int k = 1; !rc && k < n_lanes; ++k) {
    further.emplace_back(new DecodeLane());
    further.back()->prof.on = m->prof.on;
    const hipError_t he = create_stream(&further.back()->spare, "DEC");
    if (he != hipSuccess) set_error("hipStreamCreate failed: %s", hipGetErrorString(he));
    rc = he != hipSuccess ? FW_ENODEV : gen_workspace_build(m, further.back().get(), lane_batch, self_ctx);
  }
  if (rc) { reset(); return rc; }
  m->decode_batch = want; m->lane_batch = lane_batch; m->decode_self_ctx = self_ctx;
  for (auto& l : further) m->lanes.push_back(std::move(l));
  return FW_OK;
}

int32_t fw_model_set_decode_lanes(fw_model* fm, int32_t lanes) {
  FW_CHECK_ARG(fm, "null model");
  Model* dm = decoder_of(&fm->impl);
  int have;
  {
    std::lock_guard<std::mutex> gl(dm->grp.mu);
    have = std::max({2, env_decode_lanes(), (int)dm->lanes.size()});
  }
  FW_CHECK_ARG(lanes >= 1 && lanes <= have, "decode lanes: 1 .. %d", have);
  dm->grp.lanes_enabled.store(lanes);
  return FW_OK;
}

int32_t fw_model_set_merge_wait(fw_model* fm, int32_t wait_ms, int32_t fill_percent) {
  FW_CHECK_ARG(fm, "null model");
  FW_CHECK_ARG(wait_ms >= -1 && wait_ms <= 10000, "merge wait: -1 (one encoder pass), 0 (never) or milliseconds <= 10000");
  FW_CHECK_ARG(fill_percent >= 1 && fill_percent <= 100, "merge fill: 1 .. 100 percent of a run's chunk capacity");
  DecodeGroup& g = decoder_of(&fm->impl)->grp;
  g.merge_wait_ms.store(wait_ms);
  g.merge_fill_pct.store(fill_percent);
  return FW_OK;
}

int32_t fw_model_decode_batch(const fw_model* fm) {
  if (!fm) return 0;
  const Model* m = decoder_of(&fm->impl);
  return std::max(m->decode_batch, m->max_batch);
}

int32_t fw_model_run_capacity(const fw_model* fm) {
  if (!fm) return 0;
  return lane_chunks_of(decoder_of(&fm->impl));
}

int32_t fw_model_decode_stats(const fw_model* fm, int64_t* runs, int64_t* requests, int64_t* chunks,
                              int32_t* max_run_chunks) {
  FW_CHECK_ARG(fm, "null model");
  const Model* m = decoder_of(&fm->impl);
  if (runs) *runs = m->grp.n_runs.load();
  if (requests) *requests = m->grp.n_requests.load();
  if (chunks) *chunks = m->grp.n_chunks.load();
  if (max_run_chunks) *max_run_chunks = m->grp.max_run_chunks.load();
  return FW_OK;
}

int32_t fw_model_join_decoder(fw_model* fm, fw_model* decoder) {
  FW_CHECK_ARG(fm && decoder && fm != decoder, "need two distinct models");
  Model* m = &fm->impl;
  Model* d = &decoder->impl;
  FW_CHECK_ARG(!d->decoder, "the decoder model has itself joined another decoder");
  FW_CHECK_ARG(m->device == d->device && m->blob == d->blob && m->max_batch == d->max_batch && m->max_beam == d->max_beam,
               "models that share a decoder must share device, weight blob, max_batch and max_beam");
  FW_CHECK_ARG(!m->decoder, "this model has already joined a decoder");
  DecodeLane* lane = m->lanes[0].get();
  std::lock_guard<std::mutex> lk(lane->mu);
  FW_HIP(hipSetDevice(m->device));
  if (lane->stream) FW_HIP(hipStreamSynchronize(lane->stream));
  gen_workspace_free(lane);
  cross_pool_free(m);
  {
    std::lock_guard<std::mutex> lk2(g_models_mu);
    d->dependents += 1;
  }
  m->decoder = d;
  return FW_OK;
}

int32_t fw_logmel(fw_model* fm, const float* pcm, const int64_t* offsets, int32_t B, float* out,
                  int32_t* n_frames_out) {
  FW_CHECK_ARG(fm && offsets && out, "null argument");
  Model* m = &fm->impl;
  FW_CHECK_ARG(B >= 1 && B <= m->max_batch, "batch %d exceeds max_batch %d", B, m->max_batch);
  std::lock_guard<std::mutex> lk(m->mu);
  FW_HIP(hipSetDevice(m->device));
  int64_t total; int mf;
  int rc = check_offsets(offsets, B, &total, &mf);
  if (rc) return rc;
  FW_CHECK_ARG(total == 0 || pcm, "null pcm");
  if ((rc = m->ws_pcm.ensure(std::max<int64_t>(total, 1)))) return rc;
  if (total) FW_HIP(hipMemcpyAsync(m->ws_pcm.p, pcm, total * sizeof(float), hipMemcpyHostToDevice, m->stream));
  if ((rc = logmel_batch(m, m->ws_pcm.p, offsets, B, true, false))) return rc;
  FW_HIP(hipMemcpyAsync(out, m->ws_feat32, (size_t)B * m->cfg.n_mels * 3000 * sizeof(float), hipMemcpyDeviceToHost,
                        m->stream));
  if (n_frames_out)
    FW_HIP(hipMemcpyAsync(n_frames_out, m->ws_nframes, B * sizeof(int32_t), hipMemcpyDeviceToHost, m->stream));
  FW_HIP(hipStreamSynchronize(m->stream));
  return FW_OK;
}

int32_t fw_logmel_full(fw_model* fm, const float* pcm, int64_t n_samples, float* out, int64_t out_frames) {
  FW_CHECK_ARG(fm && out, "null argument");
  Model* m = &fm->impl;
  FW_CHECK_ARG(n_samples >= 0 && n_samples < (int64_t)1 << 30, "invalid n_samples");
  const int64_t nf = (n_samples + 160) / 160;
  FW_CHECK_ARG(out_frames == nf, "out_frames must be n_samples/160 + 1 = %lld, got %lld", (long long)nf,
               (long long)out_frames);
  std::lock_guard<std::mutex> lk(m->mu);
  FW_HIP(hipSetDevice(m->device));
  int rc;
  if ((rc = m->ws_pcm.ensure(std::max<int64_t>(n_samples, 1)))) return rc;
  if (n_samples) FW_HIP(hipMemcpyAsync(m->ws_pcm.p, pcm, n_samples * sizeof(float), hipMemcpyHostToDevice, m->stream));
  const int stride = (int)((nf + 7) / 8 * 8);
  if ((rc = m->ws_raw.ensure((int64_t)m->cfg.n_mels * std::max(stride, 3008)))) return rc;
  const int rstride = std::max(stride, 3008);
  int64_t offs[2] = {0, n_samples};
  FW_HIP(hipMemcpyAsync(m->ws_offsets, offs, 2 * sizeof(int64_t), hipMemcpyHostToDevice, m->stream));
  float* dout = nullptr;
  if ((rc = dev_alloc_t(&dout, (size_t)m->cfg.n_mels * nf))) return rc;
  {
    ProfScope ps(m, PF_LOGMEL, 0, (double)n_samples * 4 + (double)m->cfg.n_mels * nf * 4);
    fwk::launch_logmel(m->stream, m->ws_pcm.p, m->ws_offsets, 1, (int)nf, m->lm_consts, m->lm_filtT, m->lm_mel_pad,
                       m->cfg.n_mels, m->ws_raw.p, (int64_t)m->cfg.n_mels * rstride, rstride, m->ws_chunk_max, 0,
                       (int)nf, dout, nullptr, m->c_pad, nullptr);
  }
  hipError_t he = hipMemcpyAsync(out, dout, (size_t)m->cfg.n_mels * nf * sizeof(float), hipMemcpyDeviceToHost,
                                 m->stream);
  if (he == hipSuccess) he = hipStreamSynchronize(m->stream);
  (void)hipFree(dout);
  if (he != hipSuccess) {
    set_error("logmel_full failed: %s", hipGetErrorString(he));
    return FW_ERUNTIME;
  }
  return FW_OK;
}

namespace {
struct EncodingMark {
  fw::DecodeGroup& g;
  std::chrono::steady_clock::time_point t0;
  explicit EncodingMark(fw::Model* m) : g(fw::decoder_of(m)->grp) {
    g.encoding.fetch_add(1);
    g.enc_mu.lock();
    t0 = std::chrono::steady_clock::now();
  }
  ~EncodingMark() {
    const int us = (int)std::chrono::duration_cast<std::chrono::microseconds>(std::chrono::steady_clock::now() - t0).count();
    const int old = g.enc_pass_us.load();
    g.enc_pass_us.store(old ? (3 * old + us) / 4 : us);
    g.enc_mu.unlock();
    g.encoding.fetch_sub(1);
    g.cv.notify_all();
  }
};
}

int32_t fw_encode(fw_model* fm, const float* features, int32_t B, fw_tensor** out) {
  FW_CHECK_ARG(fm && features && out, "null argument");
  Model* m = &fm->impl;
  FW_CHECK_ARG(B >= 1 && B <= m->max_batch, "batch %d exceeds max_batch %d", B, m->max_batch);
  EncodingMark mark(m);
  std::lock_guard<std::mutex> lk(m->mu);
  FW_HIP(hipSetDevice(m->device));
  FW_HIP(hipMemcpyAsync(m->ws_feat32, features, (size_t)B * m->cfg.n_mels * 3000 * sizeof(float),
                        hipMemcpyHostToDevice, m->stream));
  fwk::launch_features_to_cl(m->stream, m->ws_feat32, B, m->cfg.n_mels, 3000, m->ws_mel_cl, m->c_pad);
  return encode_to_tensor(m, B, "encode", out);
}

static int encode_pcm_common(Model* m, const float* pcm_dev, const int64_t* offsets, int B, fw_tensor** out) {
  if (int rc = logmel_batch(m, pcm_dev, offsets, B, false, true)) return rc;
  return encode_to_tensor(m, B, "encode_pcm", out);
}

int32_t fw_encode_pcm(fw_model* fm, const float* pcm, const int64_t* offsets, int32_t B, fw_tensor** out) {
  FW_CHECK_ARG(fm && offsets && out, "null argument");
  Model* m = &fm->impl;
  FW_CHECK_ARG(B >= 1 && B <= m->max_batch, "batch %d exceeds max_batch %d", B, m->max_batch);
  EncodingMark mark(m);
  std::lock_guard<std::mutex> lk(m->mu);
  FW_HIP(hipSetDevice(m->device));
  int64_t total; int mf;
  int rc = check_offsets(offsets, B, &total, &mf);
  if (rc) return rc;
  FW_CHECK_ARG(total == 0 || pcm, "null pcm");
  if ((rc = m->ws_pcm.ensure(std::max<int64_t>(total, 1)))) return rc;
  if (total) FW_HIP(hipMemcpyAsync(m->ws_pcm.p, pcm, total * sizeof(float), hipMemcpyHostToDevice, m->stream));
  return encode_pcm_common(m, m->ws_pcm.p, offsets, B, out);
}

int32_t fw_encode_pcm_dev(fw_model* fm, const float* pcm_dev, const int64_t* offsets, int32_t B, fw_tensor** out) {
  FW_CHECK_ARG(fm && pcm_dev && offsets && out, "null argument");
  Model* m = &fm->impl;
  FW_CHECK_ARG(B >= 1 && B <= m->max_batch, "batch %d exceeds max_batch %d", B, m->max_batch);
  EncodingMark mark(m);
  std::lock_guard<std::mutex> lk(m->mu);
  FW_HIP(hipSetDevice(m->device));
  return encode_pcm_common(m, pcm_dev, offsets, B, out);
}

int32_t fw_tensor_shape(const fw_tensor* t, int32_t* B, int32_t* T, int32_t* D) {
  FW_CHECK_ARG(t, "null tensor");
  if (B) *B = t->impl.B;
  if (T) *T = t->impl.T;
  if (D) *D = t->impl.D;
  return FW_OK;
}

int32_t fw_tensor_to_host(fw_model* fm, const fw_tensor* t, float* out) {
  FW_CHECK_ARG(fm && t && out, "null argument");
  Model* m = &fm->impl;
  std::lock_guard<std::mutex> lk(m->mu);
  FW_HIP(hipSetDevice(m->device));
  const size_t n = (size_t)t->impl.B * t->impl.T * t->impl.D;
  DevBufs db;
  float* tmp = nullptr;
  if (int rc = db.alloc(&tmp, n)) return rc;
  fwk::launch_f16_to_f32(m->stream, t->impl.data, tmp, (int64_t)n);
  hipError_t he = hipMemcpyAsync(out, tmp, n * sizeof(float), hipMemcpyDeviceToHost, m->stream);
  if (he == hipSuccess) he = hipStreamSynchronize(m->stream);
  if (he != hipSuccess) {
    set_error("tensor_to_host failed: %s", hipGetErrorString(he));
    return FW_ERUNTIME;
  }
  return FW_OK;
}

int32_t fw_tensor_from_host(fw_model* fm, const float* data, int32_t B, fw_tensor** out) {
  FW_CHECK_ARG(fm && data && out, "null argument");
  Model* m = &fm->impl;
  FW_CHECK_ARG(B >= 1 && B <= m->max_batch, "batch %d exceeds max_batch %d", B, m->max_batch);
  std::lock_guard<std::mutex> lk(m->mu);
  FW_HIP(hipSetDevice(m->device));
  fw_tensor* t = nullptr;
  int rc = new_tensor(m, B, &t);
  if (rc) return rc;
  const size_t n = (size_t)B * t->impl.T * t->impl.D;
  DevBufs db;
  float* tmp = nullptr;
  if ((rc = db.alloc(&tmp, n))) { fw_tensor_free(t); return rc; }
  hipError_t he = hipMemcpyAsync(tmp, data, n * sizeof(float), hipMemcpyHostToDevice, m->stream);
  fwk::launch_f32_to_f16(m->stream, tmp, t->impl.data, (int64_t)n);
  if (he == hipSuccess) he = hipStreamSynchronize(m->stream);
  if (he != hipSuccess) {
    fw_tensor_free(t);
    set_error("tensor_from_host failed: %s", hipGetErrorString(he));
    return FW_ERUNTIME;
  }
  *out = t;
  return FW_OK;
}

void fw_tensor_free(fw_tensor* t) {
  if (!t) return;
  if (t->impl.data) t->impl.pool->give(t->impl.data);
  delete t;
}

void fw_prof_enable(fw_model* fm, int32_t on) {
  if (!fm) return;
  for_each_prof(&fm->impl, [&](Prof& p) { p.on = on != 0; });
}
void fw_prof_reset(fw_model* fm) {
  if (!fm) return;
  for_each_prof(&fm->impl, [](Prof& p) {
    prof_collect(p);
    std::lock_guard<std::mutex> lk(p.mu);
    for (auto& a : p.acc) a = ProfAcc();
  });
}
int32_t fw_prof_count(void) { return PF_COUNT; }
const char* fw_prof_name(int32_t i) { return (i >= 0 && i < PF_COUNT) ? kProfNames[i] : ""; }
int32_t fw_prof_get(fw_model* fm, int32_t i, double* ms, int64_t* launches, double* flops, double* bytes) {
  FW_CHECK_ARG(fm && i >= 0 && i < PF_COUNT, "bad profile index");
  ProfAcc p;
  for_each_prof(&fm->impl, [&](Prof& r) {
    prof_collect(r);
    std::lock_guard<std::mutex> lk(r.mu);
    const ProfAcc& a = r.acc[i];
    p.ms += a.ms; p.launches += a.launches; p.flops += a.flops; p.bytes += a.bytes;
  });
  if (ms) *ms = p.ms;
  if (launches) *launches = p.launches;
  if (flops) *flops = p.flops;
  if (bytes) *bytes = p.bytes;
  return FW_OK;
}
int32_t fw_synchronize(fw_model* fm) {
  FW_CHECK_ARG(fm, "null model");
  FW_HIP(hipSetDevice(fm->impl.device));
  FW_HIP(hipStreamSynchronize(fm->impl.stream));
  for (const auto& l : fm->impl.lanes)
    if (l->stream) FW_HIP(hipStreamSynchronize(l->stream));
  return FW_OK;
}
int32_t fw_dev_alloc(fw_model* fm, int64_t bytes, void** out_dev) {
  FW_CHECK_ARG(fm && out_dev && bytes >= 0, "bad argument");
  FW_HIP(hipSetDevice(fm->impl.device));
  return dev_alloc(out_dev, (size_t)bytes);
}
int32_t fw_dev_free(fw_model* fm, void* dev) {
  FW_CHECK_ARG(fm, "null model");
  FW_HIP(hipSetDevice(fm->impl.device));
  if (dev) FW_HIP(hipFree(dev));
  return FW_OK;
}
int32_t fw_dev_upload(fw_model* fm, void* dst_dev, const void* src_host, int64_t bytes) {
  FW_CHECK_ARG(fm && dst_dev && src_host && bytes >= 0, "bad argument");
  FW_HIP(hipSetDevice(fm->impl.device));
  FW_HIP(hipMemcpy(dst_dev, src_host, (size_t)bytes, hipMemcpyHostToDevice));
  return FW_OK;
}

}
```

### faster_whisper_amd/csrc/hooks.hip

```cpp
#include "engine.h"

#include <math.h>
#include <string.h>

#include <algorithm>

#include "dec_kernels.h"
#include "kernels.h"

using namespace fw;
using fwd::FIN_CAP;
using fwd::GenDev;

namespace {

struct HookBufs : DevBufs {
  template <typename T>
  int upload(T** dst, const T* src, size_t n) {
    int rc = alloc(dst, n);
    if (rc) return rc;
    FW_HIP(hipMemcpy(*dst, src, n * sizeof(T), hipMemcpyHostToDevice));
    return FW_OK;
  }
  int upload_f16(half_t** dst, const float* src, size_t n) {
    std::vector<half_t> tmp(n);
    for (size_t i = 0; i < n; ++i) tmp[i] = (half_t)src[i];
    return upload(dst, tmp.data(), n);
  }
  int zero(void* ptr, size_t bytes, hipStream_t st) {
    FW_HIP(hipMemsetAsync(ptr, 0, bytes, st));
    return FW_OK;
  }
};

template <typename T>
int download(T* dst, const T* src, size_t n) {
  FW_HIP(hipMemcpy(dst, src, n * sizeof(T), hipMemcpyDeviceToHost));
  return FW_OK;
}
int download_f16(hipStream_t st, float* dst, const half_t* src, size_t n) {
  std::vector<half_t> tmp(n);
  FW_HIP(hipStreamSynchronize(st));
  FW_HIP(hipMemcpy(tmp.data(), src, n * 2, hipMemcpyDeviceToHost));
  for (size_t i = 0; i < n; ++i) dst[i] = (float)tmp[i];
  return FW_OK;
}

int download_f16_frag(hipStream_t st, float* dst, const half_t* src, int rows, int d) {
  std::vector<float> f((size_t)((rows + 15) / 16 * 16) * d);
  int rc = download_f16(st, f.data(), src, f.size());
  if (rc) return rc;
  for (int r = 0; r < rows; ++r)
    for (int k = 0; k < d; ++k) dst[(size_t)r * d + k] = f[frag_pos(r, k, d, 32)];
  return FW_OK;
}

inline size_t cross_kv_frag_pos(bool vt, int kvp, int mm, int n) {
  const int c = n & 63, r = mm & 31;
  const size_t head = (size_t)(n >> 6) * kvp * 64;
  return vt ? head + ((size_t)((mm >> 5) * 4 + (c >> 4)) * 64 + ((mm >> 3) & 3) * 16 + (c & 15)) * 8 + (mm & 7)
            : head + ((size_t)((mm >> 5) * 4 + 2 * ((r >> 2) & 1) + (c >> 5)) * 64 + ((c >> 3) & 3) * 16 + (((r >> 3) << 2) | (r & 3))) * 8 + (c & 7);
}

template <typename At>
int upload_quant_w(HookBufs& db, const float* W, int N, int K, At&& at, int8_t** d_wq, float** d_ws) {
  std::vector<int8_t> wq((size_t)N * K);
  std::vector<float> ws(N), row(K);
  for (int n = 0; n < N; ++n) {
    for (int k = 0; k < K; ++k) row[k] = f16_bits_to_f32(f32_to_f16_bits(W[(size_t)n * K + k]));
    ws[n] = quant_row_i8(row.data(), K, wq.data(), [&](int k) { return at(n, k); });
  }
  int rc = db.upload(d_wq, wq.data(), wq.size());
  return rc ? rc : db.upload(d_ws, ws.data(), ws.size());
}

int fill_lcg(half_t* dst, size_t n, std::vector<uint16_t>& stage, uint32_t seed, float scale) {
  if (stage.size() < n) stage.resize(n);
  for (size_t i = 0; i < n; ++i) {
    seed = seed * 1664525u + 1013904223u;
    stage[i] = f32_to_f16_bits(((int)(seed >> 16) % 2001 - 1000) * scale);
  }
  FW_HIP(hipMemcpy(dst, stage.data(), n * 2, hipMemcpyHostToDevice));
  return FW_OK;
}

constexpr int LAUNCH_REFUSED = 1;
template <typename F>
int time_launches(hipStream_t st, int warmup, int iters, F&& launch, float* ms_total) {
  struct Events {
    hipEvent_t a = nullptr, b = nullptr;
    ~Events() {
      if (a) (void)hipEventDestroy(a);
      if (b) (void)hipEventDestroy(b);
    }
  } ev;
  FW_HIP(hipEventCreate(&ev.a));
  FW_HIP(hipEventCreate(&ev.b));
  int lr = 0;
  for (int i = 0; i < warmup && lr == 0; ++i) lr = launch(i);
  FW_HIP(hipEventRecord(ev.a, st));
  for (int i = 0; i < iters && lr == 0; ++i) lr = launch(i);
  FW_HIP(hipEventRecord(ev.b, st));
  FW_HIP(hipEventSynchronize(ev.b));
  if (lr != 0) return LAUNCH_REFUSED;
  FW_HIP(hipEventElapsedTime(ms_total, ev.a, ev.b));
  return FW_OK;
}

int test_layernorm_impl(fw_model* fm, const float* x, const float* g, const float* b, int32_t rows, int32_t d, int32_t frag,
                        float* out) {
  FW_CHECK_ARG(fm && x && g && b && out && rows >= 1, "null argument");
  FW_CHECK_ARG(d % 128 == 0 && d >= 128 && d <= 1536, "d must be a multiple of 128 and <= 1536");
  Model* m = &fm->impl;
  std::lock_guard<std::mutex> lk(m->mu);
  FW_HIP(hipSetDevice(m->device));
  HookBufs db;
  half_t *dx, *dg, *dlb, *dy;
  const size_t ny = (size_t)(frag ? (rows + 15) / 16 * 16 : rows) * d;
  int rc;
  if ((rc = db.upload_f16(&dx, x, (size_t)rows * d)) || (rc = db.upload_f16(&dg, g, d)) || (rc = db.upload_f16(&dlb, b, d)) ||
      (rc = db.alloc(&dy, ny)) || (rc = db.zero(dy, ny * sizeof(half_t), m->stream)))
    return rc;
  fwk::launch_layernorm(m->stream, dx, dg, dlb, dy, rows, d, frag ? 1 : 0);
  return frag ? download_f16_frag(m->stream, out, dy, rows, d) : download_f16(m->stream, out, dy, (size_t)rows * d);
}

}

extern "C" {

int32_t fw_test_gemm(fw_model* fm, const float* A, const float* W, const float* bias, const float* residual,
                     int32_t M, int32_t N, int32_t K, int32_t act_gelu, int32_t use_int8, float* out) {
  FW_CHECK_ARG(fm && A && W && out, "null argument");
  Model* m = &fm->impl;
  std::lock_guard<std::mutex> lk(m->mu);
  FW_HIP(hipSetDevice(m->device));
  const bool frag_kv = !use_int8 && (act_gelu == 8 || act_gelu == 9);
  FW_CHECK_ARG(!use_int8 || m->compute_type == FW_COMPUTE_INT8_FLOAT16, "int8 gemm test needs an int8_float16 model");
  if (frag_kv && (N % 64 || residual)) { set_error("fragment-major gemm test: N %% 64 == 0, no residual"); return FW_EINVAL; }
  HookBufs db;
  half_t *dA, *dW, *dB = nullptr, *dR = nullptr, *dC;
  int rc;
  if ((rc = db.upload_f16(&dA, A, (size_t)M * K)) || (rc = db.upload_f16(&dW, W, (size_t)N * K)) ||
      (bias && (rc = db.upload_f16(&dB, bias, N))) || (residual && (rc = db.upload_f16(&dR, residual, (size_t)M * N))) ||
      (rc = db.alloc(&dC, (size_t)M * N)))
    return rc;
  LinearW L{dW, dB, nullptr, nullptr, nullptr, nullptr, N, K};
  LinIn in{dA, K, 0};
  if (use_int8) {
    int8_t* dWq;
    float* dWs;
    if ((rc = upload_quant_w(db, W, N, K, [&](int n, int k) { return (size_t)n * K + k; }, &dWq, &dWs)) ||
        (rc = quantise_rows(m, dA, nullptr, M, K, nullptr, m->ws_xq)))
      return rc;
    L.wq = dWq; L.wscale = dWs;
    in = {.xq = &m->ws_xq};
  }
  if (frag_kv) {
    const bool vt = act_gelu == 9;
    const int kvp = (M + 31) / 32 * 32, H = N / 64;
    std::vector<float> hf((size_t)H * kvp * 64);
    half_t* dF;
    if ((rc = db.alloc(&dF, hf.size())) || (rc = db.zero(dF, hf.size() * sizeof(half_t), m->stream))) return rc;
    if ((rc = run_linear(m, L, {.in = in, .C = dF, .ldc = vt ? kvp : N, .M = M, .trans = vt, .head_rows = kvp})) ||
        (rc = download_f16(m->stream, hf.data(), dF, hf.size())))
      return rc;
    for (int mm = 0; mm < kvp; ++mm)
      for (int n = 0; n < N; ++n) {
        const size_t off = cross_kv_frag_pos(vt, kvp, mm, n);
        if (mm < M) out[(size_t)mm * N + n] = hf[off];
        else if (hf[off] != 0.f) { set_error("fragment-major epilogue wrote the padded key %d", mm); return FW_ERUNTIME; }
      }
    return FW_OK;
  }
  const bool trans = act_gelu >= 2;
  rc = run_linear(m, L, {.in = in, .C = dC, .ldc = trans ? M : N, .res = trans ? nullptr : dR, .ldr = trans ? 0 : N, .M = M,
                         .act = trans ? act_gelu - 2 : act_gelu, .trans = trans});
  return rc ? rc : download_f16(m->stream, out, dC, (size_t)M * N);
}

int32_t fw_test_dec_linear(fw_model* fm, const float* x, const float* W, const float* bias, const float* ln_g,
                           const float* ln_b, const float* res, int32_t R, int32_t N, int32_t K, int32_t act,
                           int32_t form, float* out, float* out_from_frag) {
  FW_CHECK_ARG(fm && x && W && out && out_from_frag, "null argument");
  FW_CHECK_ARG(R >= 1 && N % 32 == 0 && K % 64 == 0, "need R >= 1, N %% 32 == 0, K %% 64 == 0");
  FW_CHECK_ARG((ln_g == nullptr) == (ln_b == nullptr), "ln_g and ln_b go together");
  Model* m = &fm->impl;
  std::lock_guard<std::mutex> lk(m->mu);
  FW_HIP(hipSetDevice(m->device));
  const bool i8 = form == 1;
  if (i8 && (m->compute_type != FW_COMPUTE_INT8_FLOAT16 || ln_g)) {
    set_error("int8 decoder-linear test needs an int8_float16 model and no LayerNorm");
    return FW_EINVAL;
  }
  hipStream_t st = m->stream;
  const int R16 = (R + 15) / 16 * 16;
  auto h = [](float v) { return f16_bits_to_f32(f32_to_f16_bits(v)); };
  HookBufs db;
  half_t *d_res = nullptr, *d_bias = nullptr, *d_out;
  int rc;
  if ((res && (rc = db.upload_f16(&d_res, res, (size_t)R * N))) || (rc = db.alloc(&d_out, (size_t)R * N))) return rc;
  if (i8) {
    int8_t *d_wq, *d_xq;
    float *d_ws, *d_xs;
    half_t* d_x;
    if ((rc = upload_quant_w(db, W, N, K, [&](int n, int k) { return frag_pos(n, k, K, 64); }, &d_wq, &d_ws)) ||
        (rc = db.upload_f16(&d_x, x, (size_t)R * K)) || (bias && (rc = db.upload_f16(&d_bias, bias, N))) ||
        (rc = db.alloc(&d_xq, (size_t)R16 * K)) || (rc = db.alloc(&d_xs, (size_t)R16)) || (rc = db.zero(d_xq, (size_t)R16 * K, st)))
      return rc;
    fwk::launch_quant_rows(st, d_x, K, nullptr, nullptr, d_xq, d_xs, R, K, 1);
    if (fwd::launch_dec_gemm_frag_i8(st, d_xq, d_xs, d_wq, d_ws, d_bias, d_res, N, d_out, N, R, N, K, act) != 0) {
      set_error("int8 decoder linear: unsupported shape R=%d N=%d K=%d", R, N, K);
      return FW_ERUNTIME;
    }
    if ((rc = download_f16(st, out, d_out, (size_t)R * N))) return rc;
    memcpy(out_from_frag, out, (size_t)R * N * sizeof(float));
    return FW_OK;
  }
  std::vector<uint16_t> wf((size_t)N * K), xf((size_t)R16 * K, 0);
  std::vector<float> s1(N, 0.f), cf(N, 0.f);
  for (int n = 0; n < N; ++n) {
    double a1 = 0.0, ac = 0.0;
    for (int k = 0; k < K; ++k) {
      const float wv = h(W[(size_t)n * K + k]);
      const uint16_t wg = ln_g ? f32_to_f16_bits(wv * h(ln_g[k])) : f32_to_f16_bits(wv);
      wf[frag_pos(n, k, K, 32)] = wg;
      a1 += (double)f16_bits_to_f32(wg);
      if (ln_g) ac += (double)wv * (double)h(ln_b[k]);
    }
    if (bias) ac += (double)h(bias[n]);
    s1[n] = (float)a1;
    cf[n] = (float)ac;
  }
  for (int r = 0; r < R; ++r)
    for (int k = 0; k < K; ++k) xf[frag_pos(r, k, K, 32)] = f32_to_f16_bits(x[(size_t)r * K + k]);
  uint16_t *d_wf, *d_xf;
  half_t* d_of;
  float *d_s1 = nullptr, *d_cf = nullptr;
  if ((rc = db.upload(&d_wf, wf.data(), wf.size())) || (rc = db.upload(&d_xf, xf.data(), xf.size())) ||
      (rc = db.alloc(&d_of, (size_t)R16 * N)) || (rc = db.zero(d_of, (size_t)R16 * N * 2, st)))
    return rc;
  if (ln_g) {
    if ((rc = db.upload(&d_s1, s1.data(), (size_t)N)) || (rc = db.upload(&d_cf, cf.data(), (size_t)N))) return rc;
  } else if (bias) {
    if ((rc = db.upload_f16(&d_bias, bias, N))) return rc;
  }
  const fwd::DecLin lin{(const half_t*)d_xf, (const half_t*)d_wf, d_bias, d_s1, d_cf, d_res, N, d_out, N, d_of, R, N, K, act};
  if (fwd::launch_dec_linear(st, lin, form) != 0) {
    set_error("decoder linear: unsupported shape R=%d N=%d K=%d (form %d)", R, N, K, form);
    return FW_ERUNTIME;
  }
  if ((rc = download_f16(st, out, d_out, (size_t)R * N))) return rc;
  return download_f16_frag(st, out_from_frag, d_of, R, N);
}

int32_t fw_dec_big_min_rows(void) { return fwd::dec_big_min_rows(); }
int32_t fw_dec_big_min_rows_of(int32_t role, int32_t compute_type) { return fwd::dec_big_min_rows_of(role, compute_type); }

int32_t fw_test_knob(int32_t id, int32_t value) {
  FW_CHECK_ARG(id == 1 || id == 2 || id == 4 || id == 5 || id == 6 || id == 7, "unknown knob %d", id);
  if (id == 6) { set_cross_kv_layered(value); return FW_OK; }
  if (id == 7) { fwd::set_cross_attn_regs(value); return FW_OK; }
  if (id == 1) fwk::g_gemm_order.store(value);
  else if (id == 5) fwk::g_gemm_vt_stage.store(value);
  else if (id == 2) fwd::set_self_attn_form(value);
  else set_pos_blocks(value);
  return FW_OK;
}

int64_t fw_test_idle_lead_chunks(int64_t queued, int32_t n_queued, int32_t encoding, int64_t want, int32_t max_batch) {
  return idle_lead_chunks(queued, n_queued, encoding, want, max_batch);
}

int32_t fw_test_run_capacity(int32_t lane_chunks, int32_t max_batch, int32_t max_beam, int64_t self_cap, int32_t B,
                             int32_t sampling, int32_t beam_size, int32_t num_hypotheses, int32_t ctx,
                             int64_t* rows_per_chunk, int64_t* want, int64_t* run_cap) {
  const RunCapacity cap(lane_chunks, max_batch, max_beam, self_cap, B, sampling != 0, beam_size, num_hypotheses, ctx);
  *rows_per_chunk = cap.rows_per_chunk;
  *want = cap.want;
  *run_cap = cap.run_cap;
  return cap.rows_fit && cap.cache_fits ? 1 : 0;
}

int32_t fw_test_dec_linear_plan(int32_t R, int32_t N, int32_t K, int32_t ldo, int32_t ldr, int32_t compute_type,
                                int32_t form, int32_t out[6]) {
  const fwd::DecLinPlan p = fwd::dec_linear_plan(R, N, K, ldo, ldr, compute_type, form);
  const int32_t f[6] = {p.family, p.cfg, p.row_tiles, p.col_tiles, p.chunk, p.waves};
  memcpy(out, f, sizeof(f));
  return FW_OK;
}

int32_t fw_test_gemm_plan(int32_t M, int32_t N, int32_t K, int32_t batch, int64_t lda, int64_t ldw, int64_t a_bstride,
                          int64_t ldc, int64_t c_bstride, int32_t trans, int32_t int8, int32_t head_rows, int32_t n_layers,
                          int32_t has_res, int32_t out[9]) {
  static const float some_scale = 1.f;
  static const half_t some_res = 0;
  fwk::GemmParams p{};
  p.lda = lda; p.a_bstride = a_bstride; p.ldw = ldw; p.ldc = ldc; p.c_bstride = c_bstride;
  p.M = M; p.N = N; p.K = K;
  p.head_rows = head_rows; p.n_layers = n_layers;
  p.a_scale = int8 ? &some_scale : nullptr;
  p.w_scale = int8 == 1 ? &some_scale : nullptr;
  p.res = has_res ? &some_res : nullptr;
  const fwk::GemmPlan pl = fwk::gemm_plan(p, batch, trans != 0);
  const int32_t f[9] = {pl.kernel, pl.p.nMt, pl.p.nNt, pl.p.nNt_layer, pl.p.n_mp, pl.p.blk_n, pl.p.blk_m, pl.p.vt_stage, pl.grid};
  memcpy(out, f, sizeof(f));
  return FW_OK;
}

int32_t fw_test_self_attn_form(int32_t n_ctx, int32_t cache_ctx, int32_t d, int32_t R_total, int32_t kmul, int32_t H,
                               int32_t chunks, int32_t knob) {
  return fwd::self_attn_form(n_ctx, cache_ctx, d, R_total, kmul, H, chunks, knob);
}

int32_t fw_test_blob_check(const void* blob_host, int64_t bytes) {
  FW_CHECK_ARG(blob_host && bytes >= (int64_t)sizeof(BlobHeader), "weight blob too small");
  BlobHeader h;
  memcpy(&h, blob_host, sizeof(h));
  if (int rc = check_blob_header(h, bytes)) return rc;
  std::vector<BlobEntry> entries(h.n_tensors);
  memcpy(entries.data(), reinterpret_cast<const char*>(blob_host) + sizeof(h), entries.size() * sizeof(BlobEntry));
  Weights unused;
  bool has_plain;
  return bind_weights(h, entries.data(), const_cast<void*>(blob_host), unused, &has_plain);
}

int32_t fw_test_dec_logits(fw_model* fm, const float* x, int32_t R, float* out) {
  FW_CHECK_ARG(fm && x && out && R >= 1, "bad argument");
  Model* m = &fm->impl;
  std::lock_guard<std::mutex> lk(m->mu);
  FW_HIP(hipSetDevice(m->device));
  hipStream_t st = m->stream;
  const int d = m->cfg.d_model, V = m->cfg.n_vocab, R16 = (R + 15) / 16 * 16;
  const bool i8 = m->compute_type == FW_COMPUTE_INT8_FLOAT16;
  std::vector<half_t> xh((size_t)R16 * d, (half_t)0.f);
  for (int r = 0; r < R; ++r)
    for (int k = 0; k < d; ++k) xh[i8 ? (size_t)r * d + k : frag_pos(r, k, d, 32)] = (half_t)x[(size_t)r * d + k];
  HookBufs db;
  half_t* d_x;
  float* d_out;
  int rc, lr;
  if ((rc = db.upload(&d_x, xh.data(), xh.size())) || (rc = db.alloc(&d_out, (size_t)R * V))) return rc;
  if (i8) {
    int8_t* d_xq;
    float* d_xs;
    if ((rc = db.alloc(&d_xq, (size_t)R16 * d)) || (rc = db.alloc(&d_xs, (size_t)R16)) || (rc = db.zero(d_xq, (size_t)R16 * d, st)))
      return rc;
    fwk::launch_quant_rows(st, d_x, d, m->dec_ln.g, m->dec_ln.b, d_xq, d_xs, R, d, 1);
    lr = fwd::launch_dec_logits(st, true, d_xq, d_xs, m->logits.wq, m->logits.wscale, nullptr, nullptr, d_out, V, R, V, d);
  } else {
    lr = fwd::launch_dec_logits(st, false, d_x, nullptr, m->logits.w, nullptr, m->logits.s1, m->logits.cf, d_out, V, R, V,
                                d);
  }
  FW_HIP(hipStreamSynchronize(st));
  if (lr != 0) {
    set_error("logits projection test failed: unsupported shape");
    return FW_ERUNTIME;
  }
  return download(out, d_out, (size_t)R * V);
}

int32_t fw_bench_dec_linear(fw_model* fm, int32_t R, int32_t N, int32_t K, int32_t lnf, int32_t variant, int32_t iters,
                            float* us_out) {
  FW_CHECK_ARG(fm && us_out && R > 0 && N > 0 && K > 0 && iters > 0, "bad argument");
  Model* m = &fm->impl;
  std::lock_guard<std::mutex> lk(m->mu);
  FW_HIP(hipSetDevice(m->device));
  hipStream_t st = m->stream;
  const size_t wn = (size_t)N * K;
  const int copies = (int)std::max<size_t>(2, ((size_t)640 << 20) / (wn * 2));
  const size_t rp = ((size_t)R + 15) / 16 * 16;
  HookBufs db;
  half_t *dW, *dX, *dO, *dB;
  float *dS, *dC;
  std::vector<uint16_t> stage;
  int rc;
  if ((rc = db.alloc(&dW, wn * copies)) || (rc = db.alloc(&dX, rp * K)) || (rc = db.alloc(&dO, rp * N)) ||
      (rc = db.alloc(&dB, (size_t)N)) || (rc = db.alloc(&dS, (size_t)N)) || (rc = db.alloc(&dC, (size_t)N)) ||
      (rc = fill_lcg(dW, wn, stage, 2463534242u, 1e-3f)) || (rc = fill_lcg(dX, rp * K, stage, 2463534242u, 1e-3f)) ||
      (rc = db.zero(dB, (size_t)N * 2, st)) || (rc = db.zero(dS, (size_t)N * 4, st)) || (rc = db.zero(dC, (size_t)N * 4, st)))
    return rc;
  for (int c = 1; c < copies; ++c) FW_HIP(hipMemcpy(dW + (size_t)c * wn, dW, wn * 2, hipMemcpyDeviceToDevice));
  float ms = 0.f;
  rc = time_launches(st, 4, iters, [&](int i) {
    return fwd::launch_dec_gemm_frag_variant(st, variant, lnf != 0, dX, dW + (size_t)(i % copies) * wn, dB, dS, dC, dO, R, N, K);
  }, &ms);
  if (rc == LAUNCH_REFUSED) { set_error("fw_bench_dec_linear: unsupported shape / variant"); return FW_EINVAL; }
  if (rc) return rc;
  *us_out = ms * 1000.f / (float)iters;
  return FW_OK;
}

int32_t fw_bench_gemm(fw_model* fm, int32_t M, int32_t N, int32_t K, int32_t batch, int32_t a_pad, int32_t w_pad,
                      int32_t trans, int32_t iters, float* ms_out) {
  FW_CHECK_ARG(fm && ms_out && M > 0 && N > 0 && K > 0 && batch > 0 && iters > 0, "bad argument");
  Model* m = &fm->impl;
  std::lock_guard<std::mutex> lk(m->mu);
  FW_HIP(hipSetDevice(m->device));
  const bool i8 = m->compute_type == FW_COMPUTE_INT8_FLOAT16;
  const int64_t lda = K + a_pad, ldw = K + w_pad;
  const int64_t ldct = (M + 63) / 64 * 64;
  const size_t na = (size_t)batch * M * lda, nw = (size_t)N * ldw,
               nc = trans ? (size_t)batch * N * ldct : (size_t)batch * M * N;
  const size_t ha = i8 ? (na + 1) / 2 : na, hw = i8 ? (nw + 1) / 2 : nw;
  HookBufs db;
  half_t *dA, *dW, *dC;
  float *dsa = nullptr, *dsw = nullptr;
  std::vector<uint16_t> stage;
  int rc;
  if ((rc = db.alloc(&dA, ha)) || (rc = db.alloc(&dW, hw)) || (rc = db.alloc(&dC, nc)) ||
      (rc = fill_lcg(dA, ha, stage, 12345u, 1e-3f)) || (rc = fill_lcg(dW, hw, stage, 12345u, 1e-3f)))
    return rc;
  if (i8 && ((rc = db.alloc(&dsa, (size_t)batch * M)) || (rc = db.alloc(&dsw, (size_t)N)) ||
             (rc = db.zero(dsa, (size_t)batch * M * 4, m->stream)) || (rc = db.zero(dsw, (size_t)N * 4, m->stream))))
    return rc;
  QuantRows xq;
  xq.q = reinterpret_cast<int8_t*>(dA); xq.scale = dsa; xq.ld = lda;
  const LinearW L{dW, nullptr, reinterpret_cast<const int8_t*>(dW), dsw, nullptr, nullptr, N, K};
  LinCall call{.C = dC, .ldc = trans ? ldct : N, .c_bs = trans ? (int64_t)N * ldct : (int64_t)M * N, .M = M};
  if (i8) call.in = {.xq = &xq};
  else call.in = {dA, lda, (int64_t)M * lda};
  const fwk::GemmParams p = gemm_params(L, call, ldw);
  float ms = 0.f;
  rc = time_launches(m->stream, 1, iters, [&](int) { return fwk::launch_gemm(m->stream, p, batch, trans != 0); }, &ms);
  if (rc == LAUNCH_REFUSED) { set_error("gemm bench failed: unsupported shape"); return FW_ERUNTIME; }
  if (rc) return rc;
  *ms_out = ms / (float)iters;
  return FW_OK;
}

int32_t fw_bench_gemm_epi(fw_model* fm, int32_t M, int32_t N, int32_t K, int32_t batch, int32_t lda_in, int32_t trans,
                          int32_t bias, int32_t act, int32_t res, int32_t n_layers, int32_t iters, float* ms_out) {
  FW_CHECK_ARG(fm && ms_out && M > 0 && N > 0 && K > 0 && batch > 0 && iters > 0 && n_layers >= 1, "bad argument");
  FW_CHECK_ARG(res >= 0 && res <= 2 && !(res && (trans || n_layers > 1)), "residual: row-major single-layer output only");
  Model* m = &fm->impl;
  FW_CHECK_ARG(m->compute_type != FW_COMPUTE_INT8_FLOAT16, "float16 models only");
  std::lock_guard<std::mutex> lk(m->mu);
  FW_HIP(hipSetDevice(m->device));
  const int64_t lda = lda_in > 0 ? lda_in : K;
  const bool layered = n_layers > 1;
  const int64_t kvp = (M + 31) / 32 * 32;
  const int64_t ldct = layered ? kvp : (M + 63) / 64 * 64;
  const int64_t c_bs = layered ? (int64_t)N * kvp : (trans ? (int64_t)N * ldct : (int64_t)M * N);
  const int64_t c_ls = c_bs * batch;
  const size_t na = (size_t)batch * ((size_t)M * lda + K), nw = (size_t)N * K * n_layers, nc = (size_t)c_ls * n_layers;
  const size_t nr1 = res == 1 ? (size_t)batch * M * N : (size_t)M * N;
  const int copies = res == 1 ? (int)std::max<size_t>(2, ((size_t)640 << 20) / (nr1 * 2)) : 1;
  HookBufs db;
  half_t *dA, *dW, *dC, *dB, *dR = nullptr;
  std::vector<uint16_t> stage;
  int rc;
  if ((rc = db.alloc(&dA, na)) || (rc = db.alloc(&dW, nw)) || (rc = db.alloc(&dC, nc)) || (rc = db.alloc(&dB, (size_t)N * n_layers)) ||
      (res && (rc = db.alloc(&dR, nr1 * copies))) || (rc = fill_lcg(dA, na, stage, 12345u, 1e-3f)) ||
      (rc = fill_lcg(dW, nw, stage, 12345u, 1e-3f)) || (rc = fill_lcg(dB, (size_t)N * n_layers, stage, 777u, 1e-3f)) ||
      (res && (rc = fill_lcg(dR, nr1, stage, 4242u, 1e-3f))) || (rc = db.zero(dC, nc * 2, m->stream)))
    return rc;
  for (int c = 1; res && c < copies; ++c) FW_HIP(hipMemcpy(dR + (size_t)c * nr1, dR, nr1 * 2, hipMemcpyDeviceToDevice));
  const LinearW L{dW, bias ? dB : nullptr, nullptr, nullptr, nullptr, nullptr, N, K};
  LinCall call{.in = {dA, lda, (int64_t)M * lda}, .C = dC, .ldc = trans ? ldct : N, .c_bs = c_bs, .ldr = N,
               .r_bs = res == 1 ? (int64_t)M * N : 0, .M = M, .act = act};
  if (layered) {
    call.head_rows = (int)kvp;
    call.n_layers = n_layers; call.w_ls = (int64_t)N * K; call.b_ls = N; call.c_ls = c_ls;
  }
  float ms = 0.f;
  rc = time_launches(m->stream, 1, iters, [&](int i) {
    call.res = res ? dR + (size_t)(i % copies) * nr1 : nullptr;
    return fwk::launch_gemm(m->stream, gemm_params(L, call, K), batch, trans != 0);
  }, &ms);
  if (rc == LAUNCH_REFUSED) { set_error("gemm epilogue bench failed: unsupported shape"); return FW_ERUNTIME; }
  if (rc) return rc;
  *ms_out = ms / (float)iters;
  return FW_OK;
}

int32_t fw_bench_dec_linear_epi(fw_model* fm, int32_t R, int32_t N, int32_t K, int32_t lnf, int32_t variant, int32_t act,
                                int32_t res, int32_t outs, int32_t iters, float* us_out) {
  FW_CHECK_ARG(fm && us_out && R > 0 && N > 0 && K > 0 && iters > 0, "bad argument");
  FW_CHECK_ARG((outs & 3) != 0 && (!res || (outs & 1)), "needs an output; the residual is the row-major output in place");
  FW_CHECK_ARG(variant == 0 || variant == 5 || (variant >= 10 && variant <= 12), "unknown variant %d", variant);
  Model* m = &fm->impl;
  std::lock_guard<std::mutex> lk(m->mu);
  FW_HIP(hipSetDevice(m->device));
  hipStream_t st = m->stream;
  const size_t wn = (size_t)N * K;
  const int copies = (int)std::max<size_t>(2, ((size_t)640 << 20) / (wn * 2));
  const size_t rp = ((size_t)R + 15) / 16 * 16, on = rp * N;
  const int ocopies = (int)std::max<size_t>(2, ((size_t)640 << 20) / (on * 2));
  HookBufs db;
  half_t *dW, *dX, *dO, *dF, *dB;
  float *dS, *dC;
  std::vector<uint16_t> stage;
  int rc;
  if ((rc = db.alloc(&dW, wn * copies)) || (rc = db.alloc(&dX, rp * K)) || (rc = db.alloc(&dO, on * ocopies)) ||
      (rc = db.alloc(&dF, on)) || (rc = db.alloc(&dB, (size_t)N)) || (rc = db.alloc(&dS, (size_t)N)) || (rc = db.alloc(&dC, (size_t)N)) ||
      (rc = fill_lcg(dW, wn, stage, 2463534242u, 1e-3f)) || (rc = fill_lcg(dX, rp * K, stage, 2463534242u, 1e-3f)) ||
      (rc = db.zero(dO, on * ocopies * 2, st)) || (rc = db.zero(dB, (size_t)N * 2, st)) || (rc = db.zero(dS, (size_t)N * 4, st)) ||
      (rc = db.zero(dC, (size_t)N * 4, st)))
    return rc;
  for (int c = 1; c < copies; ++c) FW_HIP(hipMemcpy(dW + (size_t)c * wn, dW, wn * 2, hipMemcpyDeviceToDevice));
  float ms = 0.f;
  rc = time_launches(st, 4, iters, [&](int i) {
    const half_t* w = dW + (size_t)(i % copies) * wn;
    half_t* o = dO + (size_t)(i % ocopies) * on;
    half_t* op = (outs & 1) ? o : nullptr;
    half_t* of = (outs & 2) ? dF : nullptr;
    const half_t* r = res ? o : nullptr;
    const half_t* b = lnf ? nullptr : dB;
    const float *s1 = lnf ? dS : nullptr, *cf = lnf ? dC : nullptr;
    return fwd::launch_dec_linear(st, fwd::DecLin{dX, w, b, s1, cf, r, N, op, N, of, R, N, K, act}, variant);
  }, &ms);
  if (rc == LAUNCH_REFUSED) { set_error("fw_bench_dec_linear_epi: unsupported shape / variant"); return FW_EINVAL; }
  if (rc) return rc;
  *us_out = ms * 1000.f / (float)iters;
  return FW_OK;
}

int32_t fw_test_layernorm(fw_model* fm, const float* x, const float* g, const float* b, int32_t rows, int32_t d,
                          float* out) {
  return test_layernorm_impl(fm, x, g, b, rows, d, 0, out);
}
int32_t fw_test_layernorm_frag(fw_model* fm, const float* x, const float* g, const float* b, int32_t rows, int32_t d,
                               int32_t frag, float* out) {
  return test_layernorm_impl(fm, x, g, b, rows, d, frag, out);
}

int32_t fw_test_quant_rows(fw_model* fm, const float* x, int32_t rows, int32_t d, int64_t ldx, const float* ln_g,
                           const float* ln_b, int32_t frag, int8_t* xq, float* scale) {
  FW_CHECK_ARG(fm && x && xq && scale && rows >= 1 && rows <= (1 << 20), "bad argument");
  FW_CHECK_ARG((ln_g == nullptr) == (ln_b == nullptr), "ln_g and ln_b go together");
  FW_CHECK_ARG(d >= 64 && d % 64 == 0 && d <= (ln_g ? 1536 : 5120), "d %% 64 == 0, d <= 1536 with LayerNorm, <= 5120 without");
  FW_CHECK_ARG(ldx >= d && ldx % 8 == 0 && ldx <= (1 << 20), "ldx >= d, ldx %% 8 == 0");
  Model* m = &fm->impl;
  std::lock_guard<std::mutex> lk(m->mu);
  FW_HIP(hipSetDevice(m->device));
  const int R16 = (rows + 15) / 16 * 16;
  std::vector<int8_t> hq((size_t)R16 * d);
  HookBufs db;
  half_t *dx, *dg = nullptr, *dlb = nullptr;
  int8_t* dq;
  float* ds;
  int rc;
  if ((rc = db.upload_f16(&dx, x, (size_t)(rows - 1) * ldx + d)) || (ln_g && (rc = db.upload_f16(&dg, ln_g, d))) ||
      (ln_b && (rc = db.upload_f16(&dlb, ln_b, d))) || (rc = db.alloc(&dq, hq.size())) || (rc = db.alloc(&ds, (size_t)R16)) ||
      (rc = db.zero(dq, hq.size(), m->stream)))
    return rc;
  fwk::launch_quant_rows(m->stream, dx, ldx, dg, dlb, dq, ds, rows, d, frag ? 1 : 0);
  FW_HIP(hipStreamSynchronize(m->stream));
  if ((rc = download(hq.data(), dq, hq.size())) || (rc = download(scale, ds, (size_t)rows))) return rc;
  for (int r = 0; r < rows; ++r)
    for (int k = 0; k < d; ++k) xq[(size_t)r * d + k] = hq[frag ? frag_pos(r, k, d, 64) : (size_t)r * d + k];
  return FW_OK;
}

int32_t fw_test_cross_kv_frag_index(int32_t vt, int32_t kvp, int32_t N, int64_t* idx) {
  FW_CHECK_ARG(idx && kvp >= 32 && kvp % 32 == 0 && N >= 64 && N % 64 == 0, "need kvp %% 32 == 0, N %% 64 == 0");
  for (int mm = 0; mm < kvp; ++mm)
    for (int n = 0; n < N; ++n) idx[(size_t)mm * N + n] = (int64_t)cross_kv_frag_pos(vt != 0, kvp, mm, n);
  return FW_OK;
}

int32_t fw_test_gemm_ex(fw_model* fm, const float* A, int64_t a_elems, int64_t lda, int64_t a_bstride, const float* W,
                        const float* bias, const float* res, int64_t r_elems, int64_t ldr, int64_t r_bstride, float* C,
                        int64_t c_elems, int64_t c_off, int64_t ldc, int64_t c_bstride, int64_t c_lstride, int32_t M,
                        int32_t N, int32_t K, int32_t batch, int32_t n_layers, int32_t act, int32_t trans,
                        int32_t head_rows, int32_t use_int8, const float* ln_g, const float* ln_b) {
  FW_CHECK_ARG(fm && A && W && C, "null argument");
  const int64_t dim_max = 1 << 20, cnt_max = 1 << 12, str_max = (int64_t)1 << 40;
  FW_CHECK_ARG(M >= 1 && N >= 1 && K >= 1 && M <= dim_max && N <= dim_max && K <= dim_max, "bad M / N / K");
  FW_CHECK_ARG(batch >= 1 && n_layers >= 1 && batch <= cnt_max && n_layers <= cnt_max, "bad batch / n_layers");
  for (int64_t v : {a_elems, lda, a_bstride, r_elems, ldr, r_bstride, c_elems, c_off, ldc, c_bstride, c_lstride})
    FW_CHECK_ARG(v >= 0 && v <= str_max, "negative or oversized count / stride");
  FW_CHECK_ARG(act == 0 || act == 1, "act is 0 or 1");
  FW_CHECK_ARG((ln_g == nullptr) == (ln_b == nullptr) && (!ln_g || use_int8), "ln_g / ln_b: both, and only with use_int8");
  const bool rowmajor = !trans && head_rows == 0;
  FW_CHECK_ARG(!res || (rowmajor && n_layers == 1), "a residual needs the row-major single-layer form");
  FW_CHECK_ARG(n_layers == 1 || (!use_int8 && act == 0), "the layered launch is fp16 without activation");
  FW_CHECK_ARG(head_rows == 0 || (head_rows > 0 && head_rows % 32 == 0 && head_rows >= M && N % 64 == 0),
               "fragment-major output: head_rows %% 32 == 0, head_rows >= M, N %% 64 == 0");
  FW_CHECK_ARG(c_off % 8 == 0 && c_lstride % 8 == 0, "c_off and c_lstride must be multiples of 8");
  if (use_int8) FW_CHECK_ARG(lda == K && a_bstride == (int64_t)M * K, "int8: A is contiguous [batch * M][K]");
  const int64_t a_last = (int64_t)(batch - 1) * a_bstride + (int64_t)(M - 1) * lda + (K - 1);
  FW_CHECK_ARG(a_last < a_elems, "the launch reads A[%lld], a_elems = %lld", (long long)a_last, (long long)a_elems);
  if (res) {
    const int64_t r_last = (int64_t)(batch - 1) * r_bstride + (int64_t)(M - 1) * ldr + (N - 1);
    FW_CHECK_ARG(r_last < r_elems, "the launch reads res[%lld], r_elems = %lld", (long long)r_last, (long long)r_elems);
  }
  const int64_t chunk_last = head_rows > 0 ? (int64_t)(N / 64 - 1) * head_rows * 64 + (int64_t)((M - 1) / 32 + 1) * 2048 - 1
                             : trans       ? (int64_t)(N - 1) * ldc + (M - 1)
                                           : (int64_t)(M - 1) * ldc + (N - 1);
  const int64_t c_last = c_off + (int64_t)(n_layers - 1) * c_lstride + (int64_t)(batch - 1) * c_bstride + chunk_last;
  FW_CHECK_ARG(c_last < c_elems, "the launch writes C[%lld], c_elems = %lld", (long long)c_last, (long long)c_elems);

  Model* m = &fm->impl;
  std::lock_guard<std::mutex> lk(m->mu);
  FW_CHECK_ARG(!use_int8 || (m->compute_type == FW_COMPUTE_INT8_FLOAT16 && !(ln_g && K > 1536)),
               "int8 gemm test needs an int8_float16 model, K <= 1536 with LayerNorm");
  FW_HIP(hipSetDevice(m->device));
  HookBufs db;
  half_t *dA, *dW, *dB = nullptr, *dR = nullptr, *dC, *dG = nullptr, *dLb = nullptr;
  int rc;
  if ((rc = db.upload_f16(&dA, A, (size_t)a_elems)) || (rc = db.upload_f16(&dW, W, (size_t)n_layers * N * K)) ||
      (bias && (rc = db.upload_f16(&dB, bias, (size_t)n_layers * N))) || (res && (rc = db.upload_f16(&dR, res, (size_t)r_elems))) ||
      (rc = db.upload_f16(&dC, C, (size_t)c_elems)) ||
      (ln_g && ((rc = db.upload_f16(&dG, ln_g, K)) || (rc = db.upload_f16(&dLb, ln_b, K)))))
    return rc;
  LinearW L{dW, dB, nullptr, nullptr, nullptr, nullptr, N, K};
  LinCall call{.in = {dA, lda, a_bstride}, .C = dC + c_off, .ldc = ldc, .c_bs = c_bstride, .res = dR, .ldr = ldr,
               .r_bs = r_bstride, .M = M, .batch = batch, .act = act, .trans = trans != 0, .head_rows = head_rows,
               .n_layers = n_layers, .w_ls = (int64_t)N * K, .b_ls = bias ? N : 0, .c_ls = c_lstride};
  if (use_int8) {
    int8_t* dWq;
    float* dWs;
    const LNW ln{dG, dLb};
    if ((rc = upload_quant_w(db, W, N, K, [&](int n, int k) { return (size_t)n * K + k; }, &dWq, &dWs)) ||
        (rc = quantise_rows(m, dA, ln_g ? &ln : nullptr, (int64_t)batch * M, K, nullptr, m->ws_xq)))
      return rc;
    L.wq = dWq; L.wscale = dWs;
    call.in = {.xq = &m->ws_xq};
  }
  rc = run_linear(m, L, call);
  return rc ? rc : download_f16(m->stream, C, dC, (size_t)c_elems);
}

int32_t fw_test_attention(fw_model* fm, const float* q, const float* k, const float* v, int32_t B, int32_t H,
                          int32_t T, float* out) {
  FW_CHECK_ARG(fm && q && k && v && out, "null argument");
  Model* m = &fm->impl;
  std::lock_guard<std::mutex> lk(m->mu);
  FW_HIP(hipSetDevice(m->device));
  const int d = H * 64, tp = (T + 63) / 64 * 64;
  const size_t n = (size_t)B * T * d;
  std::vector<float> vt((size_t)B * d * tp, 0.f);
  for (int b = 0; b < B; ++b)
    for (int t = 0; t < T; ++t)
      for (int c = 0; c < d; ++c) vt[((size_t)b * d + c) * tp + t] = v[((size_t)b * T + t) * d + c];
  HookBufs db;
  half_t *dq, *dk, *dvt, *dout;
  int rc;
  if ((rc = db.upload_f16(&dq, q, n)) || (rc = db.upload_f16(&dk, k, n)) || (rc = db.upload_f16(&dvt, vt.data(), vt.size())) ||
      (rc = db.alloc(&dout, n)))
    return rc;
  fwk::launch_attn_enc(m->stream, {.q = dq, .k = dk, .ld = d, .qk_bstride = (int64_t)T * d, .vt = dvt, .ldvt = tp,
                                   .vt_bstride = (int64_t)d * tp, .out = dout, .ldo = d, .o_bstride = (int64_t)T * d,
                                   .B = B, .H = H, .T = T});
  return download_f16(m->stream, out, dout, n);
}

int32_t fw_bench_attention(fw_model* fm, int32_t B, int32_t H, int32_t T, int32_t variant, int32_t iters, float* ms_out) {
  FW_CHECK_ARG(fm && ms_out && B > 0 && H > 0 && T > 0 && iters > 0, "bad argument");
  Model* m = &fm->impl;
  std::lock_guard<std::mutex> lk(m->mu);
  FW_HIP(hipSetDevice(m->device));
  const int d = H * 64, tp = (T + 63) / 64 * 64;
  const size_t nqk = (size_t)B * T * 2 * d, nvt = (size_t)B * d * tp, no = (size_t)B * T * d;
  HookBufs db;
  half_t *dqk, *dvt, *dout;
  std::vector<uint16_t> stage;
  int rc;
  if ((rc = db.alloc(&dqk, nqk)) || (rc = db.alloc(&dvt, nvt)) || (rc = db.alloc(&dout, no)) ||
      (rc = fill_lcg(dqk, nqk, stage, 777u, 2e-3f)) || (rc = fill_lcg(dvt, nvt, stage, 777u, 2e-3f)))
    return rc;
  float ms = 0.f;
  const fwk::AttnEnc att{.q = dqk, .k = dqk + d, .ld = 2 * d, .qk_bstride = (int64_t)T * 2 * d, .vt = dvt, .ldvt = tp,
                         .vt_bstride = (int64_t)d * tp, .out = dout, .ldo = d, .o_bstride = (int64_t)T * d,
                         .B = B, .H = H, .T = T, .order = variant};
  rc = time_launches(m->stream, 1, iters, [&](int) { fwk::launch_attn_enc(m->stream, att); return 0; }, &ms);
  if (rc) return rc;
  *ms_out = ms / (float)iters;
  return FW_OK;
}

int32_t fw_test_dec_self_attn(fw_model* fm, const float* qkv, float* kcache, float* vcache, const uint8_t* kvidx,
                              int32_t n_chunks, int32_t kmul, int32_t Kbeam, int32_t H, int32_t n_ctx, int32_t cache_ctx,
                              int32_t pos_fixed, int32_t P, int32_t step, int32_t blk_n, int32_t frag, float* out) {
  FW_CHECK_ARG(fm && qkv && kcache && vcache && kvidx && out, "null argument");
  FW_CHECK_ARG(n_chunks >= 1 && H >= 1 && kmul >= 1 && kmul <= 16 && Kbeam >= 1 && Kbeam <= 255, "bad geometry");
  FW_CHECK_ARG(n_ctx >= 1 && n_ctx <= 448 && cache_ctx >= 1 && cache_ctx <= n_ctx, "need 1 <= cache_ctx <= n_ctx <= 448");
  FW_CHECK_ARG(blk_n >= 0 && (blk_n == 0 ? kmul <= Kbeam : (kmul == blk_n && pos_fixed >= 0)),
               "blk_n = 0: kmul <= Kbeam; blk_n > 0: kmul == blk_n and pos_fixed >= 0");
  const int pos0 = pos_fixed >= 0 ? pos_fixed : P - 1 + step;
  const int pos_last = pos0 + (blk_n > 0 ? blk_n - 1 : 0);
  FW_CHECK_ARG(pos0 >= 0 && pos_last < cache_ctx, "positions %d..%d outside the cache (%d)", pos0, pos_last, cache_ctx);
  const int d = H * 64, R = n_chunks * kmul, R16 = (R + 15) / 16 * 16, R_total = n_chunks * Kbeam;
  FW_CHECK_ARG(blk_n == 0 || fwd::self_attn_block_ok(n_ctx, cache_ctx, d, R_total), "position blocks need n_ctx %% 4 == 0");
  const size_t n_tab = (size_t)2 * R_total * n_ctx, n_cache = (size_t)R_total * H * cache_ctx * 64;
  for (size_t i = 0; i < n_tab; ++i)
    FW_CHECK_ARG(kvidx[i] < Kbeam, "kvidx[%zu] = %d is not a beam of %d", i, (int)kvidx[i], Kbeam);
  Model* m = &fm->impl;
  std::lock_guard<std::mutex> lk(m->mu);
  FW_HIP(hipSetDevice(m->device));
  hipStream_t st = m->stream;
  HookBufs db;
  half_t *d_qkv, *d_kc, *d_vc, *d_out;
  uint8_t* d_idx;
  int* d_step;
  int rc;
  if ((rc = db.upload_f16(&d_qkv, qkv, (size_t)R * 3 * d)) || (rc = db.upload_f16(&d_kc, kcache, n_cache)) ||
      (rc = db.upload_f16(&d_vc, vcache, n_cache)) || (rc = db.alloc(&d_out, (size_t)R16 * d)) ||
      (rc = db.upload(&d_idx, kvidx, n_tab)) || (rc = db.upload(&d_step, &step, 1)) ||
      (rc = db.zero(d_out, (size_t)R16 * d * 2, st)))
    return rc;
  fwd::launch_self_attn(st, d_qkv, d, d_kc, d_vc, n_ctx, cache_ctx, H, d_idx, Kbeam, kmul, d_out, R, d_step, pos_fixed, P,
                        R_total, frag ? 1 : 0, blk_n);
  FW_HIP(hipGetLastError());
  if ((rc = download_f16(st, kcache, d_kc, n_cache)) || (rc = download_f16(st, vcache, d_vc, n_cache))) return rc;
  return frag ? download_f16_frag(st, out, d_out, R, d) : download_f16(st, out, d_out, (size_t)R * d);
}

int32_t fw_test_dec_cross_attn(fw_model* fm, const float* q, const float* k, const float* v, int32_t n_enc, int32_t T,
                               int32_t H, int32_t B, int32_t kmul, int32_t kv_div, const int32_t* slot_map,
                               const int32_t* done, int32_t frag, float k_pad, float* out) {
  FW_CHECK_ARG(fm && q && k && v && slot_map && out, "null argument");
  FW_CHECK_ARG(n_enc >= 1 && T >= 1 && H >= 1 && B >= 1 && kmul >= 1 && kmul <= 16 && kv_div >= 1, "bad geometry");
  const int n_map = (B + kv_div - 1) / kv_div;
  for (int i = 0; i < n_map; ++i)
    FW_CHECK_ARG(slot_map[i] >= 0 && slot_map[i] < n_enc, "slot_map[%d] = %d outside [0, %d)", i, slot_map[i], n_enc);
  const int d = H * 64, kvp = (T + 31) / 32 * 32, R = B * kmul, R16 = (R + 15) / 16 * 16;
  const size_t blk = (size_t)d * kvp;
  std::vector<float> kf((size_t)n_enc * blk), vf((size_t)n_enc * blk, 0.f);
  for (int e = 0; e < n_enc; ++e)
    for (int t = 0; t < kvp; ++t)
      for (int n = 0; n < d; ++n) {
        const size_t src = ((size_t)e * T + t) * d + n;
        kf[e * blk + cross_kv_frag_pos(false, kvp, t, n)] = t < T ? k[src] : k_pad;
        if (t < T) vf[e * blk + cross_kv_frag_pos(true, kvp, t, n)] = v[src];
      }
  std::vector<float> of((size_t)R16 * d, 0.f);
  for (int r = 0; r < R; ++r)
    for (int n = 0; n < d; ++n) of[frag ? frag_pos(r, n, d, 32) : (size_t)r * d + n] = out[(size_t)r * d + n];
  Model* m = &fm->impl;
  std::lock_guard<std::mutex> lk(m->mu);
  FW_HIP(hipSetDevice(m->device));
  HookBufs db;
  half_t *d_q, *d_k, *d_vt, *d_out;
  int *d_map, *d_done = nullptr;
  int rc;
  if ((rc = db.upload_f16(&d_q, q, (size_t)R * d)) || (rc = db.upload_f16(&d_k, kf.data(), kf.size())) ||
      (rc = db.upload_f16(&d_vt, vf.data(), vf.size())) || (rc = db.upload_f16(&d_out, of.data(), of.size())) ||
      (rc = db.upload(&d_map, slot_map, (size_t)n_map)) || (done && (rc = db.upload(&d_done, done, (size_t)B))))
    return rc;
  fwd::launch_cross_attn(m->stream, d_q, d, d_k, d_vt, T, kvp, kmul, d_out, B, H, d_done, kv_div, frag ? 1 : 0, d_map);
  FW_HIP(hipGetLastError());
  return frag ? download_f16_frag(m->stream, out, d_out, R, d) : download_f16(m->stream, out, d_out, (size_t)R * d);
}

int32_t fw_test_dec_cross_probs(fw_model* fm, const float* q, const float* k, int32_t B, int32_t T, int32_t H,
                                const int32_t* heads, int32_t n_sel, int32_t n_tok, int32_t tok_idx, int32_t blk_n,
                                float* probs) {
  FW_CHECK_ARG(fm && q && k && heads && probs, "null argument");
  const int blk = blk_n > 0 ? blk_n : 1;
  FW_CHECK_ARG(B >= 1 && T >= 1 && H >= 1 && n_sel >= 1 && blk_n >= 0 && blk <= 16, "bad geometry");
  FW_CHECK_ARG(tok_idx >= 0 && tok_idx + blk <= n_tok, "tokens %d..%d outside [0, %d)", tok_idx, tok_idx + blk - 1, n_tok);
  for (int i = 0; i < n_sel; ++i) FW_CHECK_ARG(heads[i] >= 0 && heads[i] < H, "heads[%d] = %d outside [0, %d)", i, heads[i], H);
  const int d = H * 64, kvp = (T + 31) / 32 * 32;
  const size_t blkk = (size_t)d * kvp, n_probs = (size_t)B * n_sel * n_tok * T;
  std::vector<float> kf((size_t)B * blkk, 0.f);
  for (int b = 0; b < B; ++b)
    for (int t = 0; t < T; ++t)
      for (int n = 0; n < d; ++n) kf[b * blkk + cross_kv_frag_pos(false, kvp, t, n)] = k[((size_t)b * T + t) * d + n];
  Model* m = &fm->impl;
  std::lock_guard<std::mutex> lk(m->mu);
  FW_HIP(hipSetDevice(m->device));
  HookBufs db;
  half_t *d_q, *d_k;
  int* d_heads;
  float* d_p;
  int rc;
  if ((rc = db.upload_f16(&d_q, q, (size_t)B * blk * d)) || (rc = db.upload_f16(&d_k, kf.data(), kf.size())) ||
      (rc = db.upload(&d_heads, heads, (size_t)n_sel)) || (rc = db.upload(&d_p, probs, n_probs)))
    return rc;
  fwd::launch_cross_probs(m->stream, d_q, d, d_k, T, kvp, d_heads, n_sel, n_sel, d_p, n_tok, tok_idx, B, blk_n);
  FW_HIP(hipGetLastError());
  FW_HIP(hipStreamSynchronize(m->stream));
  return download(probs, d_p, n_probs);
}

int32_t fw_test_dec_softmax_pick(fw_model* fm, const float* logits, int32_t rows, int32_t V, int32_t row_mul,
                                 const int32_t* target, int32_t nospeech, float* out) {
  FW_CHECK_ARG(fm && logits && target && out, "null argument");
  FW_CHECK_ARG(rows >= 1 && V >= 1 && row_mul >= 1, "bad geometry");
  FW_CHECK_ARG(!nospeech || (target[0] >= 0 && target[0] < V), "no-speech id %d outside [0, %d)", target[0], V);
  Model* m = &fm->impl;
  std::lock_guard<std::mutex> lk(m->mu);
  FW_HIP(hipSetDevice(m->device));
  HookBufs db;
  const size_t n_lg = (size_t)rows * row_mul * V;
  float *d_lg, *d_out;
  int* d_t;
  int rc;
  if ((rc = db.upload(&d_lg, logits, n_lg)) || (rc = db.alloc(&d_out, (size_t)rows)) || (rc = db.alloc(&d_t, (size_t)rows))) return rc;
  FW_HIP(hipMemcpy(d_t, target, (size_t)(nospeech ? 1 : rows) * sizeof(int), hipMemcpyHostToDevice));
  if (nospeech) fwd::launch_nospeech(m->stream, d_lg, V, row_mul, target[0], d_out, rows);
  else fwd::launch_token_prob(m->stream, d_lg, V, d_t, d_out, 1, 0, rows, row_mul);
  FW_HIP(hipGetLastError());
  FW_HIP(hipStreamSynchronize(m->stream));
  return download(out, d_out, (size_t)rows);
}

struct RulesEx { const int32_t* done; float* logits_io; int32_t n_alt = 0; int32_t* alt_tok = nullptr; float* alt_lp = nullptr; };
static int32_t logits_rules_hook(fw_model* fm, const float* logits, int32_t R, const int32_t* hist, int32_t n,
                                 const float* cum, const fw_gen_opts* o, int32_t with_timestamps, float* cand_val,
                                 int32_t* cand_tok, float* cand_lp, const fwd::SmpRow* smp = nullptr,
                                 const RulesEx* ex = nullptr) {
  FW_CHECK_ARG(fm && logits && cum && o && cand_val && cand_tok && R >= 1 && n >= 0, "bad arguments");
  Model* m = &fm->impl;
  const fw_config& c = m->cfg;
  const int K = o->beam_size;
  const bool sampling = K == 1 && o->sampling_topk != 1;
  FW_CHECK_ARG(K >= 1 && K <= 16 && R % K == 0 && n < c.n_text_ctx && (n == 0 || hist), "bad geometry");
  FW_CHECK_ARG(c.n_vocab <= LP_SUP_WORDS * 64, "vocabulary too large for the rules kernel");
  for (size_t i = 0; i < (size_t)R * n; ++i)
    FW_CHECK_ARG(hist[i] >= 0 && hist[i] < c.n_vocab, "hist[%d][%d] = %d outside [0, %d)", (int)(i / n), (int)(i % n),
                 hist[i], c.n_vocab);
  if (ex && ex->done)
    for (int b = 0; b < R / K; ++b) FW_CHECK_ARG(ex->done[b] == 0 || ex->done[b] == 1, "done[%d] = %d is not 0 / 1", b, ex->done[b]);
  const int n_alt = ex ? ex->n_alt : 0;
  FW_CHECK_ARG(n_alt >= 0 && n_alt <= FW_MAX_ALTERNATIVES, "n_alt %d not in [0, %d]", n_alt, FW_MAX_ALTERNATIVES);
  FW_HIP(hipSetDevice(m->device));
  GenDev gp;
  memset(&gp, 0, sizeof(gp));
  gp.B = R / K; gp.K = K; gp.R = R; gp.V = c.n_vocab; gp.n_text_ctx = c.n_text_ctx;
  gp.n_alt = n_alt;
  gp.sample = sampling ? 1 : 0;
  gp.inv_temp = 1.0f;
  gp.with_ts = with_timestamps ? 1 : 0;
  gp.suppress_blank = o->suppress_blank ? 1 : 0;
  gp.min_new = o->min_new_tokens;
  gp.mits = fwd::initial_timestamp_limit(o->max_initial_timestamp_index, c.n_vocab, c.tok_timestamp_begin);
  gp.ngram = o->no_repeat_ngram_size;
  gp.rep_pen = o->repetition_penalty;
  gp.eot = c.tok_eot; gp.no_ts = c.tok_no_timestamps; gp.ts_begin = c.tok_timestamp_begin;
  gp.n_sup_begin = c.n_suppress_begin;
  for (int i = 0; i < c.n_suppress_begin; ++i) gp.sup_begin[i] = c.suppress_begin[i];
  std::vector<unsigned long long> mask(LP_SUP_WORDS, 0ull);
  for (int i = 0; i < o->n_suppress_tokens; ++i) {
    const int t = o->suppress_tokens[i];
    if (t >= 0 && t < c.n_vocab) mask[t >> 6] |= 1ull << (t & 63);
  }
  const size_t NT = (size_t)c.n_text_ctx;
  std::vector<int> h2(2 * (size_t)R * NT, 0);
  std::vector<float> c2(2 * (size_t)R, 0.f);
  const int cur = n & 1;
  for (int r = 0; r < R; ++r) {
    for (int i = 0; i < n; ++i) h2[((size_t)cur * R + r) * NT + i] = hist[(size_t)r * n + i];
    c2[(size_t)cur * R + r] = cum[r];
  }
  std::vector<int> dn((size_t)R, 0);
  if (ex && ex->done) std::copy(ex->done, ex->done + R / K, dn.begin());
  const size_t NC = (size_t)R * 32;
  std::vector<float> hv(NC, 0.f), hl(cand_lp ? NC : 0, 0.f);
  std::vector<int> ht(NC, 0);
  if (ex) {
    std::copy(cand_val, cand_val + NC, hv.begin());
    std::copy(cand_tok, cand_tok + NC, ht.begin());
    if (cand_lp) std::copy(cand_lp, cand_lp + NC, hl.begin());
  }
  HookBufs db;
  float *d_lg, *d_cum, *d_cv, *d_cl = nullptr;
  int *d_hist, *d_step, *d_done, *d_ct;
  unsigned long long* d_bits;
  int rc;
  if ((rc = db.upload(&d_lg, logits, (size_t)R * c.n_vocab)) || (rc = db.upload(&d_cum, c2.data(), c2.size())) ||
      (rc = db.upload(&d_hist, h2.data(), h2.size())) || (rc = db.upload(&d_step, &n, 1)) ||
      (rc = db.upload(&d_bits, mask.data(), mask.size())) || (rc = db.upload(&d_done, dn.data(), dn.size())) ||
      (rc = db.upload(&d_cv, hv.data(), NC)) || (rc = db.upload(&d_ct, ht.data(), NC)))
    return rc;
  if (cand_lp && (rc = db.upload(&d_cl, hl.data(), NC))) return rc;
  fwd::SmpRow* d_smp = nullptr;
  if (sampling) {
    std::vector<fwd::SmpRow> tab((size_t)R);
    for (int r = 0; r < R; ++r)
      tab[r] = smp ? smp[r]
                   : fwd::SmpRow{1.0f / o->sampling_temperature, (unsigned)(o->seed & 0xffffffffu), (unsigned)(o->seed >> 32), 0};
    if ((rc = db.upload(&d_smp, tab.data(), tab.size()))) return rc;
  }
  int* d_at = nullptr;
  float* d_al = nullptr;
  const size_t n_slab = (size_t)R * n_alt;
  if (n_alt > 0) {
    if ((rc = db.alloc(&d_at, (size_t)(n + 1) * n_slab)) || (rc = db.alloc(&d_al, (size_t)(n + 1) * n_slab))) return rc;
    FW_HIP(hipMemcpy(d_at + (size_t)n * n_slab, ex->alt_tok, n_slab * sizeof(int), hipMemcpyHostToDevice));
    FW_HIP(hipMemcpy(d_al + (size_t)n * n_slab, ex->alt_lp, n_slab * sizeof(float), hipMemcpyHostToDevice));
  }
  fwd::launch_logits_process(nullptr, gp, d_lg, d_bits, d_hist, d_cum, d_step, d_done, d_cv, d_ct, d_cl, d_smp, d_at, d_al);
  FW_HIP(hipGetLastError());
  FW_HIP(hipDeviceSynchronize());
  if ((rc = download(hv.data(), d_cv, NC)) || (rc = download(ht.data(), d_ct, NC))) return rc;
  if (n_alt > 0 && ((rc = download(ex->alt_tok, d_at + (size_t)n * n_slab, n_slab)) ||
                    (rc = download(ex->alt_lp, d_al + (size_t)n * n_slab, n_slab))))
    return rc;
  if (cand_lp && (rc = download(hl.data(), d_cl, NC))) return rc;
  if (ex && ex->logits_io && (rc = download(ex->logits_io, d_lg, (size_t)R * c.n_vocab))) return rc;
  const int C = ex ? 32 : sampling ? 1 : 2 * K;
  for (int r = 0; r < R; ++r)
    for (int j = 0; j < C; ++j) {
      cand_val[(size_t)r * C + j] = hv[(size_t)r * 32 + j];
      cand_tok[(size_t)r * C + j] = ht[(size_t)r * 32 + j];
      if (cand_lp) cand_lp[(size_t)r * C + j] = hl[(size_t)r * 32 + j];
    }
  return FW_OK;
}

int32_t fw_test_logits_rules(fw_model* fm, const float* logits, int32_t R, const int32_t* hist, int32_t n,
                             const float* cum, const fw_gen_opts* o, int32_t with_timestamps, float* cand_val,
                             int32_t* cand_tok) {
  return logits_rules_hook(fm, logits, R, hist, n, cum, o, with_timestamps, cand_val, cand_tok, nullptr);
}

int32_t fw_test_logits_rules_lp(fw_model* fm, const float* logits, int32_t R, const int32_t* hist, int32_t n,
                                const float* cum, const fw_gen_opts* o, int32_t with_timestamps, float* cand_val,
                                int32_t* cand_tok, float* cand_lp) {
  FW_CHECK_ARG(cand_lp, "null argument");
  return logits_rules_hook(fm, logits, R, hist, n, cum, o, with_timestamps, cand_val, cand_tok, cand_lp);
}

static int32_t smp_table(int32_t R, const float* inv_temp, const uint64_t* seed, const int32_t* row0,
                         std::vector<fwd::SmpRow>& tab) {
  tab.resize((size_t)R);
  for (int r = 0; r < R; ++r) {
    FW_CHECK_ARG(row0[r] >= 0 && row0[r] <= r && inv_temp[r] > 0.f, "row %d: row0 must lie in [0, row], inv_temp must be positive", r);
    tab[r] = {inv_temp[r], (unsigned)(seed[r] & 0xffffffffu), (unsigned)(seed[r] >> 32), row0[r]};
  }
  return FW_OK;
}

int32_t fw_test_logits_rules_smp_tab(fw_model* fm, const float* logits, int32_t R, const int32_t* hist, int32_t n,
                                     const float* cum, const fw_gen_opts* o, int32_t with_timestamps,
                                     const float* inv_temp, const uint64_t* seed, const int32_t* row0, float* cand_val,
                                     int32_t* cand_tok, float* cand_lp) {
  FW_CHECK_ARG(o && inv_temp && seed && row0 && cand_lp && R >= 1, "null argument");
  FW_CHECK_ARG(o->beam_size == 1 && o->sampling_topk == 0, "the options must select sampling (beam_size 1, sampling_topk 0)");
  std::vector<fwd::SmpRow> tab;
  if (int rc = smp_table(R, inv_temp, seed, row0, tab)) return rc;
  return logits_rules_hook(fm, logits, R, hist, n, cum, o, with_timestamps, cand_val, cand_tok, cand_lp, tab.data());
}

int32_t fw_test_logits_rules_ex(fw_model* fm, float* logits, int32_t R, const int32_t* hist, int32_t n, const float* cum,
                                const fw_gen_opts* o, int32_t with_timestamps, const int32_t* done, const float* inv_temp,
                                const uint64_t* seed, const int32_t* row0, float* cand_val, int32_t* cand_tok,
                                float* cand_lp) {
  FW_CHECK_ARG(o && cand_lp && R >= 1, "null argument");
  const bool tab_given = inv_temp || seed || row0;
  FW_CHECK_ARG(!tab_given || (inv_temp && seed && row0), "the sampling table needs inv_temp, seed and row0 together");
  std::vector<fwd::SmpRow> tab;
  if (tab_given) {
    FW_CHECK_ARG(o->beam_size == 1 && o->sampling_topk == 0, "the options must select sampling (beam_size 1, sampling_topk 0)");
    if (int rc = smp_table(R, inv_temp, seed, row0, tab)) return rc;
  }
// ... 346 lines not shown
```

Baseline: 3163.

## Share group-owned encode and decode-lane streams across model replicas

Stream ownership moves from individual models and lanes to the decoder group. The group holds one shared encoder stream plus one stream per decode lane, and each replica binds a stream lazily per role. The aim is to stop encoder passes from landing on a hardware queue that a decode lane also uses, so encode and decode can overlap instead of serialising. An env/knob can restore per-replica encoder streams, and a trace-analysis script for queue overlap is added. The risk is that encoders from several replicas now serialise on a single shared stream.

```diff
diff --git a/faster_whisper_amd/_lib.py b/faster_whisper_amd/_lib.py
--- a/faster_whisper_amd/_lib.py
+++ b/faster_whisper_amd/_lib.py
@@ -66,7 +66,7 @@
     "fw_model_set_decode_batch", "fw_model_decode_batch", "fw_model_join_decoder", "fw_model_decode_stats",
     "fw_model_set_merge_wait", "fw_model_set_decode_lanes", "fw_model_run_capacity", "fw_dec_big_min_rows", "fw_dec_big_min_rows_of", "fw_test_knob",
     "fw_test_idle_lead_chunks", "fw_test_run_capacity", "fw_test_dec_linear_plan", "fw_test_self_attn_form",
-    "fw_test_gemm_plan",
+    "fw_test_gemm_plan", "fw_test_stream_plan",
     "fw_pack_blob_size", "fw_pack_blob_copy", "fw_pack_blob_free",
     "fw_logmel", "fw_logmel_full",
     "fw_encode", "fw_encode_pcm", "fw_encode_pcm_dev", "fw_tensor_shape", "fw_tensor_to_host",
@@ -141,6 +141,8 @@
         lib.fw_test_self_attn_form.restype = i32
     if hasattr(lib, "fw_test_gemm_plan"):
         lib.fw_test_gemm_plan.argtypes = [i32, i32, i32, i32, i64, i64, i64, i64, i64, i32, i32, i32, i32, i32, i32p]
+    if hasattr(lib, "fw_test_stream_plan"):
+        lib.fw_test_stream_plan.argtypes = [vp, i32, i32, i64p]
     lib.fw_model_join_decoder.argtypes = [vp, vp]
     lib.fw_model_set_merge_wait.argtypes = [vp, i32, i32]
     lib.fw_model_set_decode_lanes.argtypes = [vp, i32]
diff --git a/faster_whisper_amd/csrc/decoder.hip b/faster_whisper_amd/csrc/decoder.hip
--- a/faster_whisper_amd/csrc/decoder.hip
+++ b/faster_whisper_amd/csrc/decoder.hip
@@ -216,7 +216,7 @@
   const size_t R = g->R, d = c.d_model, L = c.n_dec_layers, NT = g->NT;
   FW_CHECK_ARG(R <= 2048, "decode_batch * max_beam must be <= 2048 (got %zu)", R);
   FW_HIP(hipSetDevice(m->device));
-  if (!lane->stream) FW_HIP(create_stream(&lane->stream, "DEC"));
+  FW_CHECK_ARG(lane->stream, "decode lane without a stream: the group's streams come first (group_streams_ensure)");
   int rc;
 #define A(p, n) do { if ((rc = g->bufs.alloc(&(p), (n)))) return rc; } while (0)
 #define Z(p, n) do { if ((rc = g->bufs.zalloc(&(p), (n)))) return rc; } while (0)
@@ -269,6 +269,13 @@
 int gen_workspace_ensure(Model* m, DecodeLane* lane) {
   if (int rc = cross_pool_ensure(m, m->decode_batch)) return rc;
   if (lane->gen) return FW_OK;
+  if (!lane->stream) {
+    int idx = 0;
+    while (idx < (int)m->lanes.size() && m->lanes[idx].get() != lane) ++idx;
+    FW_CHECK_ARG(idx < (int)m->lanes.size(), "the lane is not one of the model's");
+    if (int rc = group_streams_ensure(m, idx + 1)) return rc;
+    lane->stream = m->grp.lane_stream[idx];
+  }
   return gen_workspace_build(m, lane, lane_chunks_of(m), m->decode_self_ctx);
 }
 
@@ -280,8 +287,6 @@
 DecodeLane::~DecodeLane() {
   if (stream) (void)hipStreamSynchronize(stream);
   gen_workspace_free(this);
-  if (stream) (void)hipStreamDestroy(stream);
-  if (spare) (void)hipStreamDestroy(spare);
 }
 
 static std::atomic<int> g_cross_kv_layered{-1};
diff --git a/faster_whisper_amd/csrc/engine.h b/faster_whisper_amd/csrc/engine.h
--- a/faster_whisper_amd/csrc/engine.h
+++ b/faster_whisper_amd/csrc/engine.h
@@ -199,11 +199,19 @@
 struct GenRequest;
 struct CrossPool;
 
+enum StreamRole { SR_ENCODE = 0,
+                  SR_PRIVATE = 1 };
+enum StreamKind { SK_GROUP_ENC = 0, SK_REPLICA = 1, SK_LANE = 2, SK_COUNT };
+inline StreamKind stream_kind_for(StreamRole role, bool enc_per_replica) {
+  return role == SR_ENCODE && !enc_per_replica ? SK_GROUP_ENC : SK_REPLICA;
+}
+bool enc_stream_per_replica();
+void set_enc_stream_per_replica(int on);
+
 constexpr int kMaxDecodeLanes = 4;
 struct DecodeLane {
   GenWorkspace* gen = nullptr;
   hipStream_t stream = nullptr;
-  hipStream_t spare = nullptr;
   std::mutex mu;
   Prof prof;
   bool busy = false;
@@ -227,6 +235,10 @@
   std::atomic<int64_t> n_runs{0}, n_requests{0}, n_chunks{0};
   std::atomic<int> max_run_chunks{0};
   std::atomic<int64_t> graph_captures{0};
+  std::mutex streams_mu;
+  hipStream_t enc_stream = nullptr;
+  hipStream_t lane_stream[kMaxDecodeLanes] = {};
+  std::atomic<int> last_encode_kind{-1};
 };
 
 struct Weights {
@@ -251,6 +263,7 @@
   int device = 0;
   int max_batch = 0, max_beam = 0;
   hipStream_t stream = nullptr;
+  hipStream_t own_stream = nullptr;
   std::mutex mu;
 
   void* blob = nullptr;
@@ -305,7 +318,11 @@
 };
 void prof_collect(Prof& p);
 
-hipError_t create_stream(hipStream_t* st, const char* role);
+hipError_t create_stream(hipStream_t* st, const char* role, StreamKind kind);
+int64_t streams_created(int kind);
+int group_streams_ensure(Model* dm, int n_lanes);
+int bind_stream(Model* m, StreamRole role);
+hipStream_t replica_stream(Model* m);
 int64_t idle_lead_chunks(int64_t queued, int n_queued, int encoding, int64_t want, int max_batch, int lanes = 2);
 struct RunCapacity {
   int64_t rows_per_chunk;
diff --git a/faster_whisper_amd/csrc/engine.hip b/faster_whisper_amd/csrc/engine.hip
--- a/faster_whisper_amd/csrc/engine.hip
+++ b/faster_whisper_amd/csrc/engine.hip
@@ -611,11 +611,6 @@
   m->blob_bytes = blob_bytes;
   m->enc_pool = std::make_shared<EncPool>(m, (size_t)max_batch * h.cfg.n_audio_ctx * h.cfg.d_model);
   auto fail = [&](int code) { fw_model_free(fm); return code; };
-  hipError_t he = create_stream(&m->stream, "ENC");
-  if (he != hipSuccess) {
-    set_error("hipStreamCreate failed: %s", hipGetErrorString(he));
-    return fail(FW_ENODEV);
-  }
   if ((rc = bind_weights(h, entries.data(), m->blob, *m, &m->has_plain))) return fail(rc);
   m->ln_unfold = env_ln_unfold();
   if (m->ln_unfold && m->compute_type != FW_COMPUTE_INT8_FLOAT16 && !m->has_plain) {
@@ -626,7 +621,7 @@
   if ((rc = setup_logmel_consts(m))) return fail(rc);
   if ((rc = alloc_workspaces(m))) return fail(rc);
   m->decode_batch = max_batch;
-  he = hipDeviceSynchronize();
+  const hipError_t he = hipDeviceSynchronize();
   if (he != hipSuccess) {
     set_error("device sync after model setup failed: %s", hipGetErrorString(he));
     return fail(FW_ENODEV);
@@ -652,7 +647,15 @@
   }
 }
 
-hipError_t create_stream(hipStream_t* st, const char* role) {
+static std::atomic<int64_t> g_streams_created[SK_COUNT];
+int64_t streams_created(int kind) { return kind >= 0 && kind < SK_COUNT ? g_streams_created[kind].load() : 0; }
+static hipError_t create_stream_of_role(hipStream_t* st, const char* role);
+hipError_t create_stream(hipStream_t* st, const char* role, StreamKind kind) {
+  const hipError_t he = create_stream_of_role(st, role);
+  if (he == hipSuccess) g_streams_created[kind].fetch_add(1);
+  return he;
+}
+static hipError_t create_stream_of_role(hipStream_t* st, const char* role) {
   char name[64];
   snprintf(name, sizeof(name), "FWAMD_%s_CUS", role);
   if (const char* c = getenv(name)) {
@@ -671,6 +674,48 @@
       return hipStreamCreateWithPriority(st, hipStreamNonBlocking, e[0] == 'h' ? greatest : least);
   }
   return hipStreamCreateWithFlags(st, hipStreamNonBlocking);
+}
+
+static std::atomic<int> g_enc_per_replica{-1};
+void set_enc_stream_per_replica(int on) { g_enc_per_replica.store(on ? 1 : 0); }
+bool enc_stream_per_replica() {
+  int v = g_enc_per_replica.load();
+  if (v < 0) {
+    const char* e = getenv("FWAMD_ENC_STREAM_PER_REPLICA");
+    v = e && e[0] == '1' ? 1 : 0;
+    g_enc_per_replica.store(v);
+  }
+  return v != 0;
+}
+
+int group_streams_ensure(Model* dm, int n_lanes) {
+  DecodeGroup& g = dm->grp;
+  std::lock_guard<std::mutex> lk(g.streams_mu);
+  FW_CHECK_ARG(n_lanes >= 0 && n_lanes <= kMaxDecodeLanes, "decode lanes: at most %d", kMaxDecodeLanes);
+  FW_HIP(hipSetDevice(dm->device));
+  if (!g.enc_stream) FW_HIP(create_stream(&g.enc_stream, "ENC", SK_GROUP_ENC));
+  for (int i = 0; i < n_lanes; ++i)
+    if (!g.lane_stream[i]) FW_HIP(create_stream(&g.lane_stream[i], "DEC", SK_LANE));
+  return FW_OK;
+}
+
+int bind_stream(Model* m, StreamRole role) {
+  const StreamKind kind = stream_kind_for(role, enc_stream_per_replica());
+  if (kind == SK_GROUP_ENC) {
+    Model* dm = decoder_of(m);
+    if (int rc = group_streams_ensure(dm, 1)) return rc;
+    m->stream = dm->grp.enc_stream;
+  } else {
+    if (!m->own_stream) FW_HIP(create_stream(&m->own_stream, "ENC", SK_REPLICA));
+    m->stream = m->own_stream;
+  }
+  if (role == SR_ENCODE) decoder_of(m)->grp.last_encode_kind.store(kind);
+  return FW_OK;
+}
+
+hipStream_t replica_stream(Model* m) {
+  if (bind_stream(m, SR_PRIVATE) != FW_OK) m->stream = nullptr;
+  return m->stream;
 }
 
 fwk::GemmParams gemm_params(const LinearW& L, const LinCall& c, int64_t ldw) {
@@ -985,12 +1030,18 @@
     release[1] = m->decoder;
   }
   (void)hipSetDevice(m->device);
-  if (m->stream) (void)hipStreamSynchronize(m->stream);
+  if (m->own_stream) (void)hipStreamSynchronize(m->own_stream);
   m->lanes.clear();
   cross_pool_free(m);
   m->enc_pool->close();
   if (m->blob && m->blob_owned) (void)hipFree(m->blob);
-  if (m->stream) (void)hipStreamDestroy(m->stream);
+  if (m->own_stream) (void)hipStreamDestroy(m->own_stream);
+  if (m->grp.enc_stream) {
+    (void)hipStreamSynchronize(m->grp.enc_stream);
+    (void)hipStreamDestroy(m->grp.enc_stream);
+  }
+  for (hipStream_t s : m->grp.lane_stream)
+    if (s) (void)hipStreamDestroy(s);
   delete fm;
   for (Model* t : release) {
     if (!t) continue;
@@ -1090,14 +1141,15 @@
   };
   reset();
   std::vector<std::unique_ptr<DecodeLane>> further;
-  int rc = cross_pool_ensure(m, want);
+  int rc = group_streams_ensure(m, n_lanes);
+  if (!rc) lane0->stream = m->grp.lane_stream[0];
+  if (!rc) rc = cross_pool_ensure(m, want);
   if (!rc) rc = gen_workspace_build(m, lane0, lane_batch, self_ctx);
   for (int k = 1; !rc && k < n_lanes; ++k) {
     further.emplace_back(new DecodeLane());
     further.back()->prof.on = m->prof.on;
-    const hipError_t he = create_stream(&further.back()->spare, "DEC");
-    if (he != hipSuccess) set_error("hipStreamCreate failed: %s", hipGetErrorString(he));
-    rc = he != hipSuccess ? FW_ENODEV : gen_workspace_build(m, further.back().get(), lane_batch, self_ctx);
+    further.back()->stream = m->grp.lane_stream[k];
+    rc = gen_workspace_build(m, further.back().get(), lane_batch, self_ctx);
   }
   if (rc) { reset(); return rc; }
   m->decode_batch = want; m->lane_batch = lane_batch; m->decode_self_ctx = self_ctx;
@@ -1183,6 +1235,7 @@
   int rc = check_offsets(offsets, B, &total, &mf);
   if (rc) return rc;
   FW_CHECK_ARG(total == 0 || pcm, "null pcm");
+  if ((rc = bind_stream(m, SR_PRIVATE))) return rc;
   if ((rc = m->ws_pcm.ensure(std::max<int64_t>(total, 1)))) return rc;
   if (total) FW_HIP(hipMemcpyAsync(m->ws_pcm.p, pcm, total * sizeof(float), hipMemcpyHostToDevice, m->stream));
   if ((rc = logmel_batch(m, m->ws_pcm.p, offsets, B, true, false))) return rc;
@@ -1204,6 +1257,7 @@
   std::lock_guard<std::mutex> lk(m->mu);
   FW_HIP(hipSetDevice(m->device));
   int rc;
+  if ((rc = bind_stream(m, SR_PRIVATE))) return rc;
   if ((rc = m->ws_pcm.ensure(std::max<int64_t>(n_samples, 1)))) return rc;
   if (n_samples) FW_HIP(hipMemcpyAsync(m->ws_pcm.p, pcm, n_samples * sizeof(float), hipMemcpyHostToDevice, m->stream));
   const int stride = (int)((nf + 7) / 8 * 8);
@@ -1257,6 +1311,7 @@
   EncodingMark mark(m);
   std::lock_guard<std::mutex> lk(m->mu);
   FW_HIP(hipSetDevice(m->device));
+  if (int rc = bind_stream(m, SR_ENCODE)) return rc;
   FW_HIP(hipMemcpyAsync(m->ws_feat32, features, (size_t)B * m->cfg.n_mels * 3000 * sizeof(float),
                         hipMemcpyHostToDevice, m->stream));
   fwk::launch_features_to_cl(m->stream, m->ws_feat32, B, m->cfg.n_mels, 3000, m->ws_mel_cl, m->c_pad);
@@ -1279,6 +1334,7 @@
   int rc = check_offsets(offsets, B, &total, &mf);
   if (rc) return rc;
   FW_CHECK_ARG(total == 0 || pcm, "null pcm");
+  if ((rc = bind_stream(m, SR_ENCODE))) return rc;
   if ((rc = m->ws_pcm.ensure(std::max<int64_t>(total, 1)))) return rc;
   if (total) FW_HIP(hipMemcpyAsync(m->ws_pcm.p, pcm, total * sizeof(float), hipMemcpyHostToDevice, m->stream));
   return encode_pcm_common(m, m->ws_pcm.p, offsets, B, out);
@@ -1291,6 +1347,7 @@
   EncodingMark mark(m);
   std::lock_guard<std::mutex> lk(m->mu);
   FW_HIP(hipSetDevice(m->device));
+  if (int rc = bind_stream(m, SR_ENCODE)) return rc;
   return encode_pcm_common(m, pcm_dev, offsets, B, out);
 }
 
@@ -1311,6 +1368,7 @@
   DevBufs db;
   float* tmp = nullptr;
   if (int rc = db.alloc(&tmp, n)) return rc;
+  if (int rc = bind_stream(m, SR_PRIVATE)) return rc;
   fwk::launch_f16_to_f32(m->stream, t->impl.data, tmp, (int64_t)n);
   hipError_t he = hipMemcpyAsync(out, tmp, n * sizeof(float), hipMemcpyDeviceToHost, m->stream);
   if (he == hipSuccess) he = hipStreamSynchronize(m->stream);
@@ -1333,7 +1391,7 @@
   const size_t n = (size_t)B * t->impl.T * t->impl.D;
   DevBufs db;
   float* tmp = nullptr;
-  if ((rc = db.alloc(&tmp, n))) { fw_tensor_free(t); return rc; }
+  if ((rc = db.alloc(&tmp, n)) || (rc = bind_stream(m, SR_PRIVATE))) { fw_tensor_free(t); return rc; }
   hipError_t he = hipMemcpyAsync(tmp, data, n * sizeof(float), hipMemcpyHostToDevice, m->stream);
   fwk::launch_f32_to_f16(m->stream, tmp, t->impl.data, (int64_t)n);
   if (he == hipSuccess) he = hipStreamSynchronize(m->stream);
@@ -1384,7 +1442,8 @@
 int32_t fw_synchronize(fw_model* fm) {
   FW_CHECK_ARG(fm, "null model");
   FW_HIP(hipSetDevice(fm->impl.device));
-  FW_HIP(hipStreamSynchronize(fm->impl.stream));
+  if (fm->impl.own_stream) FW_HIP(hipStreamSynchronize(fm->impl.own_stream));
+  if (hipStream_t es = decoder_of(&fm->impl)->grp.enc_stream) FW_HIP(hipStreamSynchronize(es));
   for (const auto& l : fm->impl.lanes)
     if (l->stream) FW_HIP(hipStreamSynchronize(l->stream));
   return FW_OK;
diff --git a/faster_whisper_amd/csrc/hooks.hip b/faster_whisper_amd/csrc/hooks.hip
--- a/faster_whisper_amd/csrc/hooks.hip
+++ b/faster_whisper_amd/csrc/hooks.hip
@@ -119,10 +119,10 @@
   const size_t ny = (size_t)(frag ? (rows + 15) / 16 * 16 : rows) * d;
   int rc;
   if ((rc = db.upload_f16(&dx, x, (size_t)rows * d)) || (rc = db.upload_f16(&dg, g, d)) || (rc = db.upload_f16(&dlb, b, d)) ||
-      (rc = db.alloc(&dy, ny)) || (rc = db.zero(dy, ny * sizeof(half_t), m->stream)))
-    return rc;
-  fwk::launch_layernorm(m->stream, dx, dg, dlb, dy, rows, d, frag ? 1 : 0);
-  return frag ? download_f16_frag(m->stream, out, dy, rows, d) : download_f16(m->stream, out, dy, (size_t)rows * d);
+      (rc = db.alloc(&dy, ny)) || (rc = db.zero(dy, ny * sizeof(half_t), replica_stream(m))))
+    return rc;
+  fwk::launch_layernorm(replica_stream(m), dx, dg, dlb, dy, rows, d, frag ? 1 : 0);
+  return frag ? download_f16_frag(replica_stream(m), out, dy, rows, d) : download_f16(replica_stream(m), out, dy, (size_t)rows * d);
 }
 
 }
@@ -135,7 +135,8 @@
   Model* m = &fm->impl;
   std::lock_guard<std::mutex> lk(m->mu);
   FW_HIP(hipSetDevice(m->device));
-  const bool frag_kv = !use_int8 && (act_gelu == 8 || act_gelu == 9);
+  (void)replica_stream(m);
+  const bool frag_kv =!use_int8 && (act_gelu == 8 || act_gelu == 9);
   FW_CHECK_ARG(!use_int8 || m->compute_type == FW_COMPUTE_INT8_FLOAT16, "int8 gemm test needs an int8_float16 model");
   if (frag_kv && (N % 64 || residual)) { set_error("fragment-major gemm test: N %% 64 == 0, no residual"); return FW_EINVAL; }
   HookBufs db;
@@ -161,9 +162,9 @@
     const int kvp = (M + 31) / 32 * 32, H = N / 64;
     std::vector<float> hf((size_t)H * kvp * 64);
     half_t* dF;
-    if ((rc = db.alloc(&dF, hf.size())) || (rc = db.zero(dF, hf.size() * sizeof(half_t), m->stream))) return rc;
+    if ((rc = db.alloc(&dF, hf.size())) || (rc = db.zero(dF, hf.size() * sizeof(half_t), replica_stream(m)))) return rc;
     if ((rc = run_linear(m, L, {.in = in, .C = dF, .ldc = vt ? kvp : N, .M = M, .trans = vt, .head_rows = kvp})) ||
-        (rc = download_f16(m->stream, hf.data(), dF, hf.size())))
+        (rc = download_f16(replica_stream(m), hf.data(), dF, hf.size())))
       return rc;
     for (int mm = 0; mm < kvp; ++mm)
       for (int n = 0; n < N; ++n) {
@@ -176,7 +177,7 @@
   const bool trans = act_gelu >= 2;
   rc = run_linear(m, L, {.in = in, .C = dC, .ldc = trans ? M : N, .res = trans ? nullptr : dR, .ldr = trans ? 0 : N, .M = M,
                          .act = trans ? act_gelu - 2 : act_gelu, .trans = trans});
-  return rc ? rc : download_f16(m->stream, out, dC, (size_t)M * N);
+  return rc ? rc : download_f16(replica_stream(m), out, dC, (size_t)M * N);
 }
 
 int32_t fw_test_dec_linear(fw_model* fm, const float* x, const float* W, const float* bias, const float* ln_g,
@@ -193,7 +194,7 @@
     set_error("int8 decoder-linear test needs an int8_float16 model and no LayerNorm");
     return FW_EINVAL;
   }
-  hipStream_t st = m->stream;
+  hipStream_t st = replica_stream(m);
   const int R16 = (R + 15) / 16 * 16;
   auto h = [](float v) { return f16_bits_to_f32(f32_to_f16_bits(v)); };
   HookBufs db;
@@ -258,13 +259,29 @@
 int32_t fw_dec_big_min_rows_of(int32_t role, int32_t compute_type) { return fwd::dec_big_min_rows_of(role, compute_type); }
 
 int32_t fw_test_knob(int32_t id, int32_t value) {
-  FW_CHECK_ARG(id == 1 || id == 2 || id == 4 || id == 5 || id == 6 || id == 7, "unknown knob %d", id);
+  FW_CHECK_ARG(id == 1 || id == 2 || id == 4 || id == 5 || id == 6 || id == 7 || id == 8, "unknown knob %d", id);
+  if (id == 8) { set_enc_stream_per_replica(value); return FW_OK; }
   if (id == 6) { set_cross_kv_layered(value); return FW_OK; }
   if (id == 7) { fwd::set_cross_attn_regs(value); return FW_OK; }
   if (id == 1) fwk::g_gemm_order.store(value);
   else if (id == 5) fwk::g_gemm_vt_stage.store(value);
   else if (id == 2) fwd::set_self_attn_form(value);
   else set_pos_blocks(value);
+  return FW_OK;
+}
+
+int32_t fw_test_stream_plan(const fw_model* fm, int32_t role, int32_t enc_per_replica, int64_t out[7]) {
+  FW_CHECK_ARG(out && (role == SR_ENCODE || role == SR_PRIVATE), "stream plan: role 0 (encode) or 1 (private), out[7]");
+  for (int i = 0; i < 7; ++i) out[i] = -1;
+  out[0] = stream_kind_for((StreamRole)role, enc_per_replica < 0 ? enc_stream_per_replica() : enc_per_replica != 0);
+  for (int k = 0; k < SK_COUNT; ++k) out[1 + k] = streams_created(k);
+  if (fm) {
+    const Model* m = &fm->impl;
+    const DecodeGroup& g = decoder_of(m)->grp;
+    out[4] = g.last_encode_kind.load();
+    out[5] = g.enc_stream ? 1 : 0;
+    out[6] = m->own_stream ? 1 : 0;
+  }
   return FW_OK;
 }
 
@@ -330,7 +347,7 @@
   Model* m = &fm->impl;
   std::lock_guard<std::mutex> lk(m->mu);
   FW_HIP(hipSetDevice(m->device));
-  hipStream_t st = m->stream;
+  hipStream_t st = replica_stream(m);
   const int d = m->cfg.d_model, V = m->cfg.n_vocab, R16 = (R + 15) / 16 * 16;
   const bool i8 = m->compute_type == FW_COMPUTE_INT8_FLOAT16;
   std::vector<half_t> xh((size_t)R16 * d, (half_t)0.f);
@@ -366,7 +383,7 @@
   Model* m = &fm->impl;
   std::lock_guard<std::mutex> lk(m->mu);
   FW_HIP(hipSetDevice(m->device));
-  hipStream_t st = m->stream;
+  hipStream_t st = replica_stream(m);
   const size_t wn = (size_t)N * K;
   const int copies = (int)std::max<size_t>(2, ((size_t)640 << 20) / (wn * 2));
   const size_t rp = ((size_t)R + 15) / 16 * 16;
@@ -412,7 +429,7 @@
       (rc = fill_lcg(dA, ha, stage, 12345u, 1e-3f)) || (rc = fill_lcg(dW, hw, stage, 12345u, 1e-3f)))
     return rc;
   if (i8 && ((rc = db.alloc(&dsa, (size_t)batch * M)) || (rc = db.alloc(&dsw, (size_t)N)) ||
-             (rc = db.zero(dsa, (size_t)batch * M * 4, m->stream)) || (rc = db.zero(dsw, (size_t)N * 4, m->stream))))
+             (rc = db.zero(dsa, (size_t)batch * M * 4, replica_stream(m))) || (rc = db.zero(dsw, (size_t)N * 4, replica_stream(m)))))
     return rc;
   QuantRows xq;
   xq.q = reinterpret_cast<int8_t*>(dA); xq.scale = dsa; xq.ld = lda;
@@ -422,7 +439,7 @@
   else call.in = {dA, lda, (int64_t)M * lda};
   const fwk::GemmParams p = gemm_params(L, call, ldw);
   float ms = 0.f;
-  rc = time_launches(m->stream, 1, iters, [&](int) { return fwk::launch_gemm(m->stream, p, batch, trans != 0); }, &ms);
+  rc = time_launches(replica_stream(m), 1, iters, [&](int) { return fwk::launch_gemm(replica_stream(m), p, batch, trans != 0); }, &ms);
   if (rc == LAUNCH_REFUSED) { set_error("gemm bench failed: unsupported shape"); return FW_ERUNTIME; }
   if (rc) return rc;
   *ms_out = ms / (float)iters;
@@ -453,7 +470,7 @@
   if ((rc = db.alloc(&dA, na)) || (rc = db.alloc(&dW, nw)) || (rc = db.alloc(&dC, nc)) || (rc = db.alloc(&dB, (size_t)N * n_layers)) ||
       (res && (rc = db.alloc(&dR, nr1 * copies))) || (rc = fill_lcg(dA, na, stage, 12345u, 1e-3f)) ||
       (rc = fill_lcg(dW, nw, stage, 12345u, 1e-3f)) || (rc = fill_lcg(dB, (size_t)N * n_layers, stage, 777u, 1e-3f)) ||
-      (res && (rc = fill_lcg(dR, nr1, stage, 4242u, 1e-3f))) || (rc = db.zero(dC, nc * 2, m->stream)))
+      (res && (rc = fill_lcg(dR, nr1, stage, 4242u, 1e-3f))) || (rc = db.zero(dC, nc * 2, replica_stream(m))))
     return rc;
   for (int c = 1; res && c < copies; ++c) FW_HIP(hipMemcpy(dR + (size_t)c * nr1, dR, nr1 * 2, hipMemcpyDeviceToDevice));
   const LinearW L{dW, bias ? dB : nullptr, nullptr, nullptr, nullptr, nullptr, N, K};
@@ -464,9 +481,9 @@
     call.n_layers = n_layers; call.w_ls = (int64_t)N * K; call.b_ls = N; call.c_ls = c_ls;
   }
   float ms = 0.f;
-  rc = time_launches(m->stream, 1, iters, [&](int i) {
+  rc = time_launches(replica_stream(m), 1, iters, [&](int i) {
     call.res = res ? dR + (size_t)(i % copies) * nr1 : nullptr;
-    return fwk::launch_gemm(m->stream, gemm_params(L, call, K), batch, trans != 0);
+    return fwk::launch_gemm(replica_stream(m), gemm_params(L, call, K), batch, trans != 0);
   }, &ms);
   if (rc == LAUNCH_REFUSED) { set_error("gemm epilogue bench failed: unsupported shape"); return FW_ERUNTIME; }
   if (rc) return rc;
@@ -482,7 +499,7 @@
   Model* m = &fm->impl;
   std::lock_guard<std::mutex> lk(m->mu);
   FW_HIP(hipSetDevice(m->device));
-  hipStream_t st = m->stream;
+  hipStream_t st = replica_stream(m);
   const size_t wn = (size_t)N * K;
   const int copies = (int)std::max<size_t>(2, ((size_t)640 << 20) / (wn * 2));
   const size_t rp = ((size_t)R + 15) / 16 * 16, on = rp * N;
@@ -543,10 +560,10 @@
   int rc;
   if ((rc = db.upload_f16(&dx, x, (size_t)(rows - 1) * ldx + d)) || (ln_g && (rc = db.upload_f16(&dg, ln_g, d))) ||
       (ln_b && (rc = db.upload_f16(&dlb, ln_b, d))) || (rc = db.alloc(&dq, hq.size())) || (rc = db.alloc(&ds, (size_t)R16)) ||
-      (rc = db.zero(dq, hq.size(), m->stream)))
-    return rc;
-  fwk::launch_quant_rows(m->stream, dx, ldx, dg, dlb, dq, ds, rows, d, frag ? 1 : 0);
-  FW_HIP(hipStreamSynchronize(m->stream));
+      (rc = db.zero(dq, hq.size(), replica_stream(m))))
+    return rc;
+  fwk::launch_quant_rows(replica_stream(m), dx, ldx, dg, dlb, dq, ds, rows, d, frag ? 1 : 0);
+  FW_HIP(hipStreamSynchronize(replica_stream(m)));
   if ((rc = download(hq.data(), dq, hq.size())) || (rc = download(scale, ds, (size_t)rows))) return rc;
   for (int r = 0; r < rows; ++r)
     for (int k = 0; k < d; ++k) xq[(size_t)r * d + k] = hq[frag ? frag_pos(r, k, d, 64) : (size_t)r * d + k];
@@ -597,6 +614,7 @@
   FW_CHECK_ARG(!use_int8 || (m->compute_type == FW_COMPUTE_INT8_FLOAT16 && !(ln_g && K > 1536)),
                "int8 gemm test needs an int8_float16 model, K <= 1536 with LayerNorm");
   FW_HIP(hipSetDevice(m->device));
+  (void)replica_stream(m);
   HookBufs db;
   half_t *dA, *dW, *dB = nullptr, *dR = nullptr, *dC, *dG = nullptr, *dLb = nullptr;
   int rc;
@@ -620,7 +638,7 @@
     call.in = {.xq = &m->ws_xq};
   }
   rc = run_linear(m, L, call);
-  return rc ? rc : download_f16(m->stream, C, dC, (size_t)c_elems);
+  return rc ? rc : download_f16(replica_stream(m), C, dC, (size_t)c_elems);
 }
 
 int32_t fw_test_attention(fw_model* fm, const float* q, const float* k, const float* v, int32_t B, int32_t H,
@@ -641,10 +659,10 @@
   if ((rc = db.upload_f16(&dq, q, n)) || (rc = db.upload_f16(&dk, k, n)) || (rc = db.upload_f16(&dvt, vt.data(), vt.size())) ||
       (rc = db.alloc(&dout, n)))
     return rc;
-  fwk::launch_attn_enc(m->stream, {.q = dq, .k = dk, .ld = d, .qk_bstride = (int64_t)T * d, .vt = dvt, .ldvt = tp,
+  fwk::launch_attn_enc(replica_stream(m), {.q = dq, .k = dk, .ld = d, .qk_bstride = (int64_t)T * d, .vt = dvt, .ldvt = tp,
                                    .vt_bstride = (int64_t)d * tp, .out = dout, .ldo = d, .o_bstride = (int64_t)T * d,
                                    .B = B, .H = H, .T = T});
-  return download_f16(m->stream, out, dout, n);
+  return download_f16(replica_stream(m), out, dout, n);
 }
 
 int32_t fw_bench_attention(fw_model* fm, int32_t B, int32_t H, int32_t T, int32_t variant, int32_t iters, float* ms_out) {
@@ -665,7 +683,7 @@
   const fwk::AttnEnc att{.q = dqk, .k = dqk + d, .ld = 2 * d, .qk_bstride = (int64_t)T * 2 * d, .vt = dvt, .ldvt = tp,
                          .vt_bstride = (int64_t)d * tp, .out = dout, .ldo = d, .o_bstride = (int64_t)T * d,
                          .B = B, .H = H, .T = T, .order = variant};
-  rc = time_launches(m->stream, 1, iters, [&](int) { fwk::launch_attn_enc(m->stream, att); return 0; }, &ms);
+  rc = time_launches(replica_stream(m), 1, iters, [&](int) { fwk::launch_attn_enc(replica_stream(m), att); return 0; }, &ms);
   if (rc) return rc;
   *ms_out = ms / (float)iters;
   return FW_OK;
@@ -690,7 +708,7 @@
   Model* m = &fm->impl;
   std::lock_guard<std::mutex> lk(m->mu);
   FW_HIP(hipSetDevice(m->device));
-  hipStream_t st = m->stream;
+  hipStream_t st = replica_stream(m);
   HookBufs db;
   half_t *d_qkv, *d_kc, *d_vc, *d_out;
   uint8_t* d_idx;
@@ -740,9 +758,9 @@
       (rc = db.upload_f16(&d_vt, vf.data(), vf.size())) || (rc = db.upload_f16(&d_out, of.data(), of.size())) ||
       (rc = db.upload(&d_map, slot_map, (size_t)n_map)) || (done && (rc = db.upload(&d_done, done, (size_t)B))))
     return rc;
-  fwd::launch_cross_attn(m->stream, d_q, d, d_k, d_vt, T, kvp, kmul, d_out, B, H, d_done, kv_div, frag ? 1 : 0, d_map);
+  fwd::launch_cross_attn(replica_stream(m), d_q, d, d_k, d_vt, T, kvp, kmul, d_out, B, H, d_done, kv_div, frag ? 1 : 0, d_map);
   FW_HIP(hipGetLastError());
-  return frag ? download_f16_frag(m->stream, out, d_out, R, d) : download_f16(m->stream, out, d_out, (size_t)R * d);
+  return frag ? download_f16_frag(replica_stream(m), out, d_out, R, d) : download_f16(replica_stream(m), out, d_out, (size_t)R * d);
 }
 
 int32_t fw_test_dec_cross_probs(fw_model* fm, const float* q, const float* k, int32_t B, int32_t T, int32_t H,
@@ -770,9 +788,9 @@
   if ((rc = db.upload_f16(&d_q, q, (size_t)B * blk * d)) || (rc = db.upload_f16(&d_k, kf.data(), kf.size())) ||
       (rc = db.upload(&d_heads, heads, (size_t)n_sel)) || (rc = db.upload(&d_p, probs, n_probs)))
     return rc;
-  fwd::launch_cross_probs(m->stream, d_q, d, d_k, T, kvp, d_heads, n_sel, n_sel, d_p, n_tok, tok_idx, B, blk_n);
+  fwd::launch_cross_probs(replica_stream(m), d_q, d, d_k, T, kvp, d_heads, n_sel, n_sel, d_p, n_tok, tok_idx, B, blk_n);
   FW_HIP(hipGetLastError());
-  FW_HIP(hipStreamSynchronize(m->stream));
+  FW_HIP(hipStreamSynchronize(replica_stream(m)));
   return download(probs, d_p, n_probs);
 }
 
@@ -791,10 +809,10 @@
   int rc;
   if ((rc = db.upload(&d_lg, logits, n_lg)) || (rc = db.alloc(&d_out, (size_t)rows)) || (rc = db.alloc(&d_t, (size_t)rows))) return rc;
   FW_HIP(hipMemcpy(d_t, target, (size_t)(nospeech ? 1 : rows) * sizeof(int), hipMemcpyHostToDevice));
-  if (nospeech) fwd::launch_nospeech(m->stream, d_lg, V, row_mul, target[0], d_out, rows);
-  else fwd::launch_token_prob(m->stream, d_lg, V, d_t, d_out, 1, 0, rows, row_mul);
+  if (nospeech) fwd::launch_nospeech(replica_stream(m), d_lg, V, row_mul, target[0], d_out, rows);
+  else fwd::launch_token_prob(replica_stream(m), d_lg, V, d_t, d_out, 1, 0, rows, row_mul);
   FW_HIP(hipGetLastError());
-  FW_HIP(hipStreamSynchronize(m->stream));
+  FW_HIP(hipStreamSynchronize(replica_stream(m)));
   return download(out, d_out, (size_t)rows);
 }
 
diff --git a/profiles/queue_overlap.py b/profiles/queue_overlap.py
--- /dev/null
+++ b/profiles/queue_overlap.py
@@ -0,0 +1,157 @@
+import argparse
+import bisect
+import csv
+import gzip
+import sys
+from collections import Counter, defaultdict
+
+
+def short(name):
+    n = name.strip().strip('"')
+    if n.startswith("void "):
+        n = n[5:]
+    for stop in "<(":
+        n = n.split(stop)[0]
+    if n.startswith("_Z"):
+        digits = ""
+        for ch in n[2:]:
+            if not ch.isdigit():
+                break
+            digits += ch
+        if digits:
+            n = n[2 + len(digits):2 + len(digits) + int(digits)]
+    return n
+
+
+def read_trace(path):
+    opener = gzip.open if path.endswith(".gz") else open
+    rows = []
+    with opener(path, "rt", newline="") as f:
+        for r in csv.DictReader(f):
+            rows.append((short(r["Kernel_Name"]), r["Queue_Id"], int(r["Start_Timestamp"]), int(r["End_Timestamp"])))
+    rows.sort(key=lambda r: r[2])
+    return rows
+
+
+def merged(intervals):
+    starts, ends = [], []
+    for s, e in sorted(intervals):
+        if ends and s <= ends[-1]:
+            ends[-1] = max(ends[-1], e)
+        else:
+            starts.append(s)
+            ends.append(e)
+    return starts, ends
+
+
+def covered(union, a, b):
+    starts, ends = union
+    tot = 0
+    i = max(0, bisect.bisect_right(ends, a) - 1)
+    while i < len(starts) and starts[i] < b:
+        tot += max(0, min(ends[i], b) - max(starts[i], a))
+        i += 1
+    return tot
+
+
+def is_encoder_only(n):
+    return n.startswith("logmel_") or n in ("attn_enc_kernel", "layernorm_kernel", "features_to_cl_kernel")
+
+
+def lanes_of(rows):
+    by_q = defaultdict(list)
+    for n, q, s, e in rows:
+        if n == "dec_cross_attn_kernel":
+            by_q[q].append((s, e))
+    order = sorted(by_q, key=lambda q: by_q[q][0][0])
+    overlap = {}
+    for i, qa in enumerate(order):
+        ua = merged(by_q[qa])
+        for qb in order[i + 1:]:
+            overlap[(qa, qb)] = sum(covered(ua, s, e) for s, e in by_q[qb])
+    return order, {q: len(v) for q, v in by_q.items()}, overlap
+
+
+def passes_of(rows):
+    marks = [(s, q) for n, q, s, e in rows if n == "logmel_prep_kernel"]
+    out = []
+    starts = [m[0] for m in marks]
+    row_starts = [r[2] for r in rows]
+    for k, (s0, q) in enumerate(marks):
+        s1 = starts[k + 1] if k + 1 < len(marks) else float("inf")
+        end, cnt = s0, 0
+        for i in range(bisect.bisect_left(row_starts, s0), len(rows)):
+            n, qq, s, e = rows[i]
+            if s >= s1:
+                break
+            if qq == q and (is_encoder_only(n) or n == "gemm_f16_kernel"):
+                cnt += 1
+                if is_encoder_only(n):
+                    end = max(end, e)
+        out.append((q, s0, end, cnt))
+    return out
+
+
+def main():
+    ap = argparse.ArgumentParser()
+    ap.add_argument("trace")
+    ap.add_argument("--steady", type=int, default=64)
+    args = ap.parse_args()
+    rows = read_trace(args.trace)
+    t0 = rows[0][2]
+    print(f"# {args.trace.split('/')[-1]}: {len(rows)} dispatches over {(rows[-1][3] - t0) / 1e9:.2f} s")
+
+    lane_q, lane_n, lane_overlap = lanes_of(rows)
+    passes = passes_of(rows)
+    enc_q = Counter(p[0] for p in passes)
+    per_q = defaultdict(Counter)
+    for n, q, s, e in rows:
+        per_q[q]["encoder" if is_encoder_only(n) else "decode" if n.startswith("dec_") else
+                 "gemm_f16" if n == "gemm_f16_kernel" else "other"] += 1
+    print("\n## a) queue ids by role")
+    print(f"encoder passes: {len(passes)} on queues " + ", ".join(f"{q} ({c})" for q, c in sorted(enc_q.items())))
+    for i, q in enumerate(lane_q):
+        print(f"decode lane {i}: queue {q} ({lane_n[q]} dec_cross_attn_kernel launches)")
+    for (qa, qb), ns in lane_overlap.items():
+        print(f"  dec_cross_attn_kernel on queues {qa} and {qb} overlap for {ns / 1e6:.1f} ms")
+    print("dispatches per queue (encoder-only kernels / gemm_f16_kernel / dec_* / other):")
+    for q in sorted(per_q):
+        c = per_q[q]
+        print(f"  queue {q}: {c['encoder']} / {c['gemm_f16']} / {c['decode']} / {c['other']}")
+    roles = set(enc_q) | set(lane_q)
+    print(f"distinct queue ids over the three roles: {len(roles)}; encoder queues that are also a lane's: "
+          f"{sorted(set(enc_q) & set(lane_q)) or 'none'}")
+
+    dec_all = merged([(s, e) for n, q, s, e in rows if n.startswith("dec_")])
+    dec_by_q = {q: merged([(s, e) for n, qq, s, e in rows if qq == q and n.startswith("dec_")]) for q in lane_q}
+    print("\n## b) encoder passes")
+    print("pass  t_ms      queue  shares_lane  kernels  wall_ms  decode_busy  " +
+          "  ".join(f"lane{i}_busy" for i in range(len(lane_q))))
+    stats = []
+    for k, (q, s, e, cnt) in enumerate(passes):
+        wall = max(1, e - s)
+        share = covered(dec_all, s, e) / wall
+        per_lane = [covered(dec_by_q[lq], s, e) / wall for lq in lane_q]
+        shares = lane_q.index(q) if q in lane_q else -1
+        stats.append((shares >= 0, wall / 1e6, share))
+        print(f"{k:4d}  {(s - t0) / 1e6:9.1f}  {q:>5}  {('lane ' + str(shares)) if shares >= 0 else 'no':>11}  {cnt:7d}  "
+              f"{wall / 1e6:7.2f}  {share:11.3f}  " + "  ".join(f"{x:10.3f}" for x in per_lane))
+
+    def summary(title, st):
+        print(f"\n## c) {title}: {len(st)} passes")
+        print("class                 passes  share_of_passes  mean_wall_ms  mean_decode_busy")
+        for name, sel in (("shared a lane's queue", True), ("own queue", False)):
+            g = [x for x in st if x[0] == sel]
+            if not g:
+                print(f"{name:21s} {0:6d}  {0.0:15.3f}  {'-':>12}  {'-':>16}")
+                continue
+            print(f"{name:21s} {len(g):6d}  {len(g) / len(st):15.3f}  {sum(x[1] for x in g) / len(g):12.2f}  "
+                  f"{sum(x[2] for x in g) / len(g):16.3f}")
+
+    summary("all passes", stats)
+    if args.steady and len(stats) > args.steady:
+        summary(f"the last {args.steady} passes (the timed steps)", stats[-args.steady:])
+
+
+if __name__ == "__main__":
+    sys.exit(main())
```

New measurement: 3188, median of 6. Within noise of the previous version (+0.8%).
